# henry-yeh/DeepACO

Hardware: AMD Instinct MI355X
Metric: ant-tours/sec, TSP-500 n_ants=512 (higher is better)
Workload: dtype f32; 1 GPU; TSP-500 random-Euclidean, n_ants=512, 64 instances per GPU, AS update, heuristic 1/d sparsified k=50, sampler=auto -> scan_sparse; nodes=500, n_ants=512, instances_per_gpu=64, sampler=scan_sparse, parallelism=instance-sharded x1

## Files before the change

deepaco_amd/_lib.py:

```python
import ctypes as C
import os

import torch

_HERE = os.path.dirname(os.path.abspath(__file__))
LIB_PATH = os.environ.get("DACO_LIB_PATH") or os.path.join(_HERE, "lib", "libdeepaco_hip.so")

RACE_NOISE, RACE_PHILOX, SCAN, SCAN_WAVE = 0, 1, 2, 3
MAX_NODES = 4096

_lib = None

_vp, _i, _l, _f, _u64, _u32, _sz = (C.c_void_p, C.c_int, C.c_long, C.c_float, C.c_uint64, C.c_uint32,
                                     C.c_size_t)

SIGNATURES = {
    "daco_version": (_i, []),
    "daco_last_error": (C.c_char_p, []),
    "daco_vec_for_n": (_i, [_i]),
    "daco_ld_for_n": (_i, [_i]),
    "daco_tsp_sample_workspace_bytes": (_sz, [_i, _i, _i]),
    "daco_tsp_sample": (_i, [_vp, _i, _i, _i, _vp, _l, _vp, _l, _f, _f, _i, _i, _vp, _i, _vp, _u64, _u64, _vp,
                             _u32, _i, _vp, _vp, _vp, _vp, _vp, _l, _vp, _vp, _vp, _sz, _vp, _vp]),
    "daco_tsp_sparse_workspace_bytes": (_sz, [_i, _i, _i]),
    "daco_tsp_sparse_workspace_bytes_general": (_sz, [_i, _i, _i]),
    "daco_tsp_sparse_tours_offset": (_sz, [_i, _i, _i]),
    "daco_tsp_sparse_resident_per_cu": (_i, [_i, _i, _i]),
    "daco_tsp_sparse_split_tours": (_i, [_i]),
    "daco_tsp_sample_sparse": (_i, [_vp, _i, _i, _i, _vp, _l, _vp, _l, _f, _f, _vp, _i, _vp, _i, _u64, _u64, _vp, _u32, _i, _vp, _vp,
                                    _vp, _l, _vp, _vp, _vp, _vp, _sz, _vp, _vp]),
    "daco_tsp_sample_race_head": (_i, [_vp, _i, _i, _i, _vp, _l, _vp, _l, _f, _f, _vp, _i, _vp, _i, _u64, _u64, _vp, _u32, _i, _vp, _vp,
                                       _vp, _l, _vp, _vp, _vp, _vp, _sz, _vp, _vp]),
    "daco_tsp_sample_heads": (_i, [_vp, _i, _i, _i, _i, _i, _i, _i, _vp, _l, _vp, _l, _f, _f, _vp, _i, _vp, _i, _u64, _u64, _vp, _u32, _i, _vp, _vp,
                                   _vp, _l, _vp, _vp, _vp, _vp, _sz, _vp, _vp]),
    "daco_pheromone_update_heads": (_i, [_vp, _i, _i, _i, _vp, _vp, _vp, _f, _i, _vp, _vp, _f, _vp, _vp, _vp, _sz,
                                         _vp, _l, _f, _f, _vp, _i, _i, _i, _vp, _sz]),
    "daco_allreduce_delta_tau": (_i, [_vp, _vp, _vp, _sz]),
    "daco_tour_costs": (_i, [_vp, _i, _i, _i, _i, _vp, _l, _vp, _i, _vp]),
    "daco_pheromone_update_workspace_bytes": (_sz, [_i, _i, _i, _i]),
    "daco_pheromone_update": (_i, [_vp, _i, _i, _i, _i, _vp, _vp, _vp, _f, _i, _i, _vp, _vp, _f, _vp, _vp, _i, _vp,
                                   _sz]),
    "daco_prob_matrix": (_i, [_vp, _i, _i, _vp, _l, _vp, _l, _f, _f, _i, _vp, _sz]),
    "daco_pick_move": (_i, [_vp, _i, _i, _i, _vp, _sz, _i, _vp, _vp, _vp, _u64, _u64, _u32, _i, _vp, _vp, _vp, _vp]),
    "daco_directed_table_bytes": (_sz, [_i, _i, _i]),
    "daco_track_best": (_i, [_vp, _i, _i, _i, _vp, _vp, _vp, _vp, _vp, _vp, _f]),
    "daco_track_best_tours16": (_i, [_vp, _i, _i, _i, _i, _vp, _vp, _vp, _vp, _vp, _vp, _f]),
    "daco_cvrp_sample": (_i, [_vp, _i, _i, _i, _vp, _l, _vp, _l, _f, _f, _vp, _f, _i, _vp, _i, _u64, _u64, _vp, _u32, _i, _i,
                              _vp, _vp, _vp, _vp, _vp, _vp, _l, _vp, _vp, _vp, _sz, _vp, C.c_double, _vp, _vp]),
    "daco_sample_backward": (_i, [_vp, _i, _i, _i, _i, _vp, _l, _vp, _l, _f, _f, _vp, _vp, _vp, _vp, _vp, _f, _vp, _vp,
                                  C.c_double]),
    "daco_tsp_edge_logp": (_l, [_vp, _i, _i, _i, _i, _vp, _vp, _l, _vp, _f, _f, _vp, _vp, _vp]),
    "daco_tsp_edge_backward": (_l, [_vp, _i, _i, _i, _i, _vp, _vp, _l, _vp, _f, _f, _vp, _vp, _vp, _vp]),
    "daco_gnn_param_floats": (_sz, [_i]),
    "daco_gnn_workspace_bytes": (_sz, [_i, _i]),
    "daco_gnn_forward": (_i, [_vp, _i, _i, _i, _vp, _vp, _vp, _vp, _vp, _vp, _vp, _vp, _vp, _vp, _sz]),
    "daco_gnn_train_workspace_bytes": (_sz, [_i, _i, _i]),
    "daco_gnn_train_forward": (_i, [_vp, _i, _i, _i, _i, _vp, _vp, _vp, _vp, _vp, _vp, _vp, _vp, _vp, _vp, _vp, _sz]),
    "daco_gnn_train_backward": (_i, [_vp, _i, _i, _i, _i, _vp, _vp, _vp, _vp, _vp, _vp, _vp, _vp, _vp, _vp, _vp, _vp, _i, _vp, _sz]),
    "daco_cvrp_local_search": (_i, [_vp, _i, _i, _i, _i, _vp, _l, _vp, _f, _vp, _i, _vp, _vp]),
    "daco_hgs_table_bytes": (_sz, [_i, _i]),
    "daco_hgs_prepare": (_i, [_vp, _i, _i, _vp, _l, _i, _vp]),
    "daco_hgs_workspace_bytes": (_sz, [_i, _i, _i, _i, _i]),
    "daco_hgs_local_search": (_i, [_vp, _i, _i, _i, _i, _i, _vp, _vp, _vp, _vp, _vp, _vp, C.c_double, _i, _vp, _vp, _vp, _vp, _sz]),
    "daco_hgs_workspace_bytes_ss": (_sz, [_i, _i, _i, _i, _i]),
    "daco_hgs_local_search_ss": (_l, [_vp, _i, _i, _i, _i, _i, _vp, _vp, _vp, _vp, _vp, _vp, C.c_double, _i, _vp, _vp, _vp, _vp, _sz,
                                      _vp, _vp]),
    "daco_sibling_workspace_bytes": (_sz, [_i, _i, _i]),
    "daco_sibling_sample": (_i, [_vp, _i, _i, _i, _i, _vp, _l, _vp, _l, _f, _f, _vp, _vp, _l, _f, _vp, _i, _i, _vp, _vp,
                                 _i, _u64, _u64, _u32, _i, _vp, _vp, _vp, _vp, _vp, _vp, _sz]),
    "daco_sibling_backward": (_i, [_vp, _i, _i, _i, _i, _i, _vp, _l, _vp, _l, _f, _f, _vp, _vp, _l, _f, _vp, _i, _vp, _vp,
                                   _vp, _vp, _vp]),
    "daco_sibling_objective": (_l, [_vp, _i, _i, _i, _i, _i, _vp, _vp, _vp, _vp, _vp, _vp, _l, C.c_double, _i, _vp, _vp, _vp, _vp, _vp]),
    "daco_sibling_record": (_l, [_vp, _i, _i, _i, _i, _vp, _vp, _vp, _vp, _i, _vp, _vp, _vp, _vp, _vp, _f, _vp]),
    "daco_tsp_knn_graph": (_i, [_vp, _i, _i, _i, _vp, _f, _vp, _vp, _vp, _vp]),
    "daco_tsp_knn_graph_csr": (_i, [_vp, _i, _i, _i, _vp, _f, _vp, _vp, _vp, _vp, _vp, _vp]),
    "daco_cvrp_knn_graph": (_l, [_vp, _i, _i, _i, _vp, _i, _l, _vp, _vp, _vp, _vp, _vp, _vp]),
    "daco_heu_matrix": (_i, [_vp, _i, _i, _i, _vp, _vp, _f, _f, _vp, _vp]),
    "daco_sparsify": (_l, [_vp, _i, _i, _i, _vp, _l, _vp, _l, _vp]),
    "daco_sparse_head": (_l, [_vp, _i, _i, _i, _vp, _l, _vp]),
    "daco_head_stats": (_l, [_vp, _i, _i, _vp, _l, _i, C.c_double, C.c_double, _vp]),
    "daco_two_opt": (_i, [_vp, _i, _i, _i, _vp, _vp, _l, _vp, _l, _vp]),
    "daco_two_opt_tables_bytes": (_sz, [_i, _i]),
    "daco_two_opt_prepare": (_i, [_vp, _i, _i, _vp, _l, _vp, _sz]),
    "daco_two_opt_nbr": (_i, [_vp, _i, _i, _i, _vp, _l, _vp, _vp, _vp, _l, _vp]),
    "daco_two_opt_auto": (_i, [_vp, _i, _i, _i, _vp, _vp, _l, _vp, _vp, _vp, _l, _vp]),
    "daco_mkpv_sample": (_i, [_vp, _i, _i, _i, _i, _vp, _l, _vp, _l, _f, _f, _vp, _vp, _i, _vp, _i, _u64, _u64, _u32, _i,
                              _vp, _vp, _vp, _vp, _vp, _vp]),
    "daco_mkpv_backward": (_i, [_vp, _i, _i, _i, _i, _i, _vp, _l, _vp, _l, _f, _f, _vp, _vp, _vp, _vp, _vp, _vp]),
    "daco_mkpv_update": (_i, [_vp, _i, _i, _i, _i, _vp, _vp, _vp, _vp, _f, _i, _i, _f, _f, _vp, _vp, _vp]),
    "daco_transformer_param_floats": (_sz, [_i]),
    "daco_transformer_workspace_bytes": (_sz, [_i, _i]),
    "daco_transformer_forward": (_i, [_vp, _i, _i, _i, _vp, _vp, _sz, _vp, _vp, _sz]),
    "daco_transformer_saved_floats": (_sz, [_i, _i]),
    "daco_transformer_train_workspace_bytes": (_sz, [_i, _i]),
    "daco_transformer_forward_train": (_i, [_vp, _i, _i, _i, _vp, _vp, _sz, _vp, _vp, _sz, _vp, _sz]),
    "daco_transformer_backward": (_i, [_vp, _i, _i, _i, _vp, _vp, _sz, _vp, _sz, _vp, _vp, _vp, _sz]),
    "daco_rcpsp_schedule": (_i, [_vp, _i, _i, _i, _i, _i, _i, _vp, _vp, _vp, _vp, _vp, _vp, _vp, _vp, _vp, _vp, _vp]),
    "daco_rcpsp_workspace_bytes": (_sz, [_i, _i]),
    "daco_rcpsp_sample": (_i, [_vp, _i, _i, _i, _i, _i, _i, _vp, _vp, _vp, _vp, _vp, _vp, _vp, _vp, _vp, _vp, _l, _vp, _l, _f, _f,
                               C.c_double, C.c_double, _i, _vp, _u64, _u64, _u32, _vp, _vp, _vp, _vp, _vp, _vp, _vp, _sz]),
    "daco_rcpsp_backward": (_i, [_vp, _i, _i, _i, _vp, _vp, _vp, _l, _vp, _l, _f, _f, C.c_double, C.c_double, _vp, _vp, _vp, _vp]),
    "daco_rcpsp_track": (_i, [_vp, _i, _i, _i, _vp, _vp, _vp, C.c_double, _i, _i, _i, _f, _vp, _vp, _vp, _vp, _vp, _vp, _vp, _vp]),
    "daco_rcpsp_net_param_floats": (_sz, []),
    "daco_rcpsp_net_workspace_bytes": (_sz, [_i, _i]),
    "daco_rcpsp_net_forward": (_l, [_vp, _i, _i, _i, _vp, _vp, _vp, _f, _vp, _vp, _vp, _vp, _sz]),
    "daco_rcpsp_net_train_saved_bytes": (_sz, [_i, _i]),
    "daco_rcpsp_net_train_workspace_bytes": (_sz, [_i, _i]),
    "daco_rcpsp_net_train_forward": (_l, [_vp, _i, _i, _i, _vp, _vp, _vp, _f, _vp, _vp, _vp, _vp, _sz]),
    "daco_rcpsp_net_train_backward": (_l, [_vp, _i, _i, _i, _vp, _vp, _vp, _vp, _sz, _vp, _vp, _vp, _vp, _sz]),
    "daco_tsp_nls": (_i, [_vp, _i, _i, _i, _vp, _l, _vp, _vp, _vp, _l, _vp, _vp, _vp, _l, _i, _l, _vp, _vp, _vp]),
}


ABI_VERSION = 129


class DacoError(RuntimeError):
    pass

# ... 31 lines not shown
```

deepaco_amd/csrc/daco_colony_setup.hip:

```cpp
#include "daco_host.h"

namespace daco {

constexpr int CS_MAX_N = 1024;
constexpr int CS_HEAD_MAX_K = 127;

__device__ inline uint32_t cs_key(float v) {
  const uint32_t b = __float_as_uint(v == 0.0f ? 0.0f : v);
  return (b & 0x80000000u) ? ~b : (b | 0x80000000u);
}
__device__ inline float cs_unkey(uint32_t u) { return __uint_as_float((u & 0x80000000u) ? (u & 0x7fffffffu) : ~u); }

__device__ inline int cs_below(uint64_t mask) {
  return (int)__builtin_amdgcn_mbcnt_hi((uint32_t)(mask >> 32), __builtin_amdgcn_mbcnt_lo((uint32_t)mask, 0u));
}

template <int CPL>
__device__ inline uint32_t cs_kth_largest(const uint32_t (&key)[CPL], int k) {
  uint32_t t = 0;
  for (int bit = 31; bit >= 0; --bit) {
    const uint32_t cand = t | (1u << bit);
    int cnt = 0;
#pragma unroll
    for (int q = 0; q < CPL; ++q) cnt += __popcll(__ballot(key[q] >= cand));
// ... 17 lines not shown
  uint32_t chosen = 0;
#pragma unroll
  for (int q = 0; q < CPL; ++q) {
    const bool eq = key[q] == t;
    const uint64_t eqs = __ballot(eq);
    const bool c = key[q] > t || (eq && eq_before + cs_below(eqs) < room);
    const uint64_t cs = __ballot(c);
    pos[q] = ch_before + cs_below(cs);
    chosen |= (c ? 1u : 0u) << q;
    eq_before += __popcll(eqs);
    ch_before += __popcll(cs);
  }
  return chosen;
}

template <int CPL>
__global__ void __launch_bounds__(256)
sparsify_kernel(int B, int n, int k, const float *dist, long dist_bstride, const float *numer, long numer_bstride, float *out) {
  const int lane = threadIdx.x & 63, wave = threadIdx.x >> 6;
  const long row = (long)blockIdx.x * 4 + wave;
  if (row >= (long)B * n) return;
  const int b = (int)(row / n), i = (int)(row % n);
  const float *d = dist + (size_t)b * dist_bstride + (size_t)i * n;
  float v[CPL];
  uint32_t key[CPL];
#pragma unroll
  for (int q = 0; q < CPL; ++q) {
    const int j = lane + 64 * q;
    v[q] = j < n ? d[j] : 0.0f;
    key[q] = j < n ? ~cs_key(v[q]) : 0u;
  }
  int pos[CPL];
  const uint32_t chosen = cs_choose(key, k, cs_kth_largest(key, k), pos);
  const float *nu = numer ? numer + (size_t)b * numer_bstride : nullptr;
  float *o = out + (size_t)row * n;
#pragma unroll
  for (int q = 0; q < CPL; ++q) {
    const int j = lane + 64 * q;
    if (j < n) o[j] = (nu ? nu[j] : 1.0f) / (((chosen >> q) & 1u) ? v[q] : 1e10f);
  }
}

template <int CPL>
__global__ void __launch_bounds__(256)
sparse_head_kernel(int B, int n, int k, int slots, const float *w, long w_bstride, uint16_t *ids) {
  __shared__ uint16_t tab[4][128];
  const int lane = threadIdx.x & 63, wave = threadIdx.x >> 6;
  const long rows = (w_bstride == 0 ? 1L : (long)B) * n;
  const long row = (long)blockIdx.x * 4 + wave;
  const bool active = row < rows;
  tab[wave][lane] = 0;
  tab[wave][lane + 64] = 0;
  __syncthreads();
  if (active) {
    const float *r = w + (size_t)(row / n) * w_bstride + (size_t)(row % n) * n;
    uint32_t key[CPL];
#pragma unroll
    for (int q = 0; q < CPL; ++q) {
      const int j = lane + 64 * q;
      key[q] = j < n ? cs_key(r[j]) : 0u;
    }
    int pos[CPL];
    const uint32_t chosen = cs_choose(key, k, cs_kth_largest(key, k), pos);
#pragma unroll
    for (int q = 0; q < CPL; ++q) {
      const int j = lane + 64 * q;
      if (((chosen >> q) & 1u) && j < n && pos[q] < k) tab[wave][pos[q]] = (uint16_t)j;
    }
    if (lane == 0) tab[wave][slots - 1] = (uint16_t)k;
  }
  __syncthreads();
  const int words = slots >> 1;
  if (active && lane < words) {
    const uint32_t word = (uint32_t)tab[wave][2 * lane] | ((uint32_t)tab[wave][2 * lane + 1] << 16);
    uint32_t *out = reinterpret_cast<uint32_t *>(ids);
    if (w_bstride == 0) {
      for (int b = 0; b < B; ++b) out[((size_t)b * n + (size_t)row) * words + lane] = word;
    } else {
      out[(size_t)row * words + lane] = word;
    }
  }
}

__device__ inline double cs_wave_sum(double x) {
#pragma unroll
  for (int m = 32; m >= 1; m >>= 1) x += __shfl_xor(x, m, 64);
  return x;
}

struct HeadStatsArgs { int k[3]; double mass[3]; };

template <int CPL>
__global__ void __launch_bounds__(256)
head_stats_kernel(long rows, int n, const float *w, long w_bstride, HeadStatsArgs a, int32_t *counts) {
  __shared__ int passed[4][3];
  const int lane = threadIdx.x & 63, wave = threadIdx.x >> 6;
  int pass[3] = {0, 0, 0};
  for (long row = (long)blockIdx.x * 4 + wave; row < rows; row += (long)gridDim.x * 4) {
    const float *r = w + (size_t)(row / n) * w_bstride + (size_t)(row % n) * n;
    float v[CPL];
    uint32_t key[CPL];
    double part = 0.0;
#pragma unroll
    for (int q = 0; q < CPL; ++q) {
      const int j = lane + 64 * q;
      v[q] = j < n ? r[j] : 0.0f;
      key[q] = j < n ? cs_key(v[q]) : 0u;
      part += (double)v[q];
    }
    const double tot = cs_wave_sum(part);
#pragma unroll
    for (int c = 0; c < 3; ++c) {
      if (a.k[c] < 1) continue;
      const int K = a.k[c] < n ? a.k[c] : n;
      const uint32_t t = cs_kth_largest(key, K);
      const int above = cs_count_above(key, t);
      double s = 0.0;
#pragma unroll
      for (int q = 0; q < CPL; ++q) s += key[q] > t ? (double)v[q] : 0.0;
      s = cs_wave_sum(s) + (double)(K - above) * (double)cs_unkey(t);
      pass[c] += (s / tot >= a.mass[c]) ? 1 : 0;
    }
  }
  if (lane == 0) { passed[wave][0] = pass[0]; passed[wave][1] = pass[1]; passed[wave][2] = pass[2]; }
  __syncthreads();
  if (threadIdx.x < 3) {
    const int c = threadIdx.x, sum = passed[0][c] + passed[1][c] + passed[2][c] + passed[3][c];
    if (sum) atomicAdd(counts + c, sum);
  }
}

}

using namespace daco;

#define DACO_CS_DISPATCH(n, LAUNCH) \
  do {                              \
    const int cpl_ = ((n) + 63) / 64; \
    if (cpl_ <= 1) { LAUNCH(1); }     \
    else if (cpl_ <= 2) { LAUNCH(2); } \
    else if (cpl_ <= 4) { LAUNCH(4); } \
    else if (cpl_ <= 8) { LAUNCH(8); } \
    else { LAUNCH(16); }              \
  } while (0)

static int cs_check_size(const char *what, int B, int n) {
  if (n > CS_MAX_N) { set_error("%s: n=%d exceeds %d (one row per wavefront, in registers)", what, n, CS_MAX_N); return DACO_E_TOOLARGE; }
  if ((long)B * n > 0x7fffffffL) { set_error("%s: B * n = %ld rows do not fit 32 bits", what, (long)B * n); return DACO_E_TOOLARGE; }
  return DACO_OK;
}

extern "C" long daco_sparsify(void *stream, int B, int n, int k, const float *dist, long dist_bstride, const float *numer,
                             long numer_bstride, float *out) {
  if (B <= 0 || n < 2 || k < 1 || k > n || !dist || !out || dist_bstride < 0 || numer_bstride < 0) {
    set_error("daco_sparsify: bad argument (B=%d n=%d k=%d)", B, n, k);
    return DACO_E_BADARG;
  }
  if (const int rc = cs_check_size("daco_sparsify", B, n)) return rc;
  hipStream_t s = (hipStream_t)stream;
  const dim3 grid((unsigned)(((long)B * n + 3) / 4)), block(256);
#define DACO_CS_SPARSIFY(C) hipLaunchKernelGGL(sparsify_kernel<C>, grid, block, 0, s, B, n, k, dist, dist_bstride, numer, numer_bstride, out)
  DACO_CS_DISPATCH(n, DACO_CS_SPARSIFY);
#undef DACO_CS_SPARSIFY
  return launch_status("sparsify_kernel");
}

extern "C" long daco_sparse_head(void *stream, int B, int n, int k, const float *weights, long w_bstride, uint16_t *ids) {
  if (B <= 0 || n < 2 || k < 1 || k > n || k > CS_HEAD_MAX_K || !weights || !ids || w_bstride < 0) {
    set_error("daco_sparse_head: bad argument (B=%d n=%d k=%d, k <= %d)", B, n, k, CS_HEAD_MAX_K);
    return DACO_E_BADARG;
  }
  if (const int rc = cs_check_size("daco_sparse_head", B, n)) return rc;
  hipStream_t s = (hipStream_t)stream;
  const long rows = (w_bstride == 0 ? 1L : (long)B) * n;
  const int slots = k <= 63 ? 64 : 128;
  const dim3 grid((unsigned)((rows + 3) / 4)), block(256);
#define DACO_CS_HEAD(C) hipLaunchKernelGGL(sparse_head_kernel<C>, grid, block, 0, s, B, n, k, slots, weights, w_bstride, ids)
  DACO_CS_DISPATCH(n, DACO_CS_HEAD);
#undef DACO_CS_HEAD
  return launch_status("sparse_head_kernel");
}

extern "C" long daco_head_stats(void *stream, int B, int n, const float *weights, long w_bstride, int k_lds, double mass,
                               double mass_lds, int32_t *counts) {
  if (B <= 0 || n < 2 || !weights || !counts || w_bstride < 0) {
    set_error("daco_head_stats: bad argument (B=%d n=%d)", B, n);
    return DACO_E_BADARG;
  }
  if (const int rc = cs_check_size("daco_head_stats", B, n)) return rc;
  hipStream_t s = (hipStream_t)stream;
  if (const int rc = launch_status(zero_async(counts, 3 * sizeof(int32_t), s), "daco_head_stats (clearing the counters)")) return rc;
  const long rows = (w_bstride == 0 ? 1L : (long)B) * n;
  const HeadStatsArgs a = {{63, 127, k_lds}, {mass, mass, mass_lds}};
  const long want = (rows + 3) / 4;
  const dim3 grid((unsigned)(want < 1024 ? want : 1024)), block(256);
#define DACO_CS_STATS(C) hipLaunchKernelGGL(head_stats_kernel<C>, grid, block, 0, s, rows, n, weights, w_bstride, a, counts)
  DACO_CS_DISPATCH(n, DACO_CS_STATS);
#undef DACO_CS_STATS
  return launch_status("head_stats_kernel");
}
```

deepaco_amd/csrc/daco_costs_update.hip:

```cpp
#include "daco_host.h"
#include <cstdlib>

namespace daco {

__global__ void __launch_bounds__(256)
tour_costs_kernel(int B, int n, int len, int A, const float *dist, long dist_bs, const int64_t *paths,
                  int closed, float *costs) {
  const int idx = blockIdx.x * blockDim.x + threadIdx.x;
  if (idx >= B * A) return;
  const int b = idx / A, a = idx - b * A;
  const int64_t *p = paths + (size_t)b * len * A + a;
  const float *d = dist + b * dist_bs;
  float s = 0.0f;
  if (closed) {
    const long first = p[0];
    long prev = first;
    int k = 1;
    for (; k + 8 <= len; k += 8) {
      long u[8];
      float e[8];
#pragma unroll
      for (int j = 0; j < 8; ++j) u[j] = p[(size_t)(k + j) * A];
#pragma unroll
      for (int j = 0; j < 8; ++j) e[j] = d[u[j] * n + (j ? u[j - 1] : prev)];
// ... 57 lines not shown
    nbr[((size_t)b * n + u) * A + a] = up | (un << 16);
  }
}

__global__ void __launch_bounds__(64) argmin_cost_kernel(int A, const float *costs, int *best) {
  const int b = blockIdx.x, lane = threadIdx.x;
  float bk = __builtin_inff();
  int bi = 0x7fffffff;
  for (int a = lane; a < A; a += 64) {
    const float c = costs[(size_t)b * A + a];
    if (c < bk) { bk = c; bi = a; }
  }
  const KeyIdx r = wave_arg<false>(bk, bi);
  if (lane == 0) best[b] = r.idx == 0x7fffffff ? 0 : r.idx;
}

__global__ void __launch_bounds__(256)
track_best_kernel(int len, int A, const float *costs, const int64_t *paths, float *lowest, int64_t *shortest,
                  int32_t *best_idx, float *mmas_max, float mmas_scale, const uint16_t *tours16 = nullptr, int ld = 0) {
  __shared__ float rk[4];
  __shared__ int ri[4];
  __shared__ int take;
  const int b = blockIdx.x, tid = threadIdx.x, lane = tid & 63, wave = tid >> 6;
  float bk = __builtin_inff();
  int bi = 0x7fffffff;
  for (int a = tid; a < A; a += 256) {
    const float c = costs[(size_t)b * A + a];
    if (c < bk) { bk = c; bi = a; }
  }
  const KeyIdx r = wave_arg<false>(bk, bi);
  if (lane == 0) { rk[wave] = r.key; ri[wave] = r.idx; }
  __syncthreads();
  if (tid == 0) {
    float k = rk[0];
    int i = ri[0];
    for (int w = 1; w < 4; ++w)
      if (rk[w] < k || (rk[w] == k && ri[w] < i)) { k = rk[w]; i = ri[w]; }
    if (i == 0x7fffffff) i = 0;
    if (best_idx) best_idx[b] = i;
    float low = lowest[b];
    const bool improved = k < low;
    if (improved) { low = k; lowest[b] = k; }
    if (mmas_max) mmas_max[b] = (1.0f / low) * mmas_scale;
    take = improved ? i : -1;
  }
  __syncthreads();
  const int t = take;
  if (t >= 0 && shortest) {
    if (tours16) { for (int k = tid; k < len; k += 256) shortest[(size_t)b * len + k] = (int64_t)tours16[((size_t)b * A + t) * ld + k]; }
    else for (int k = tid; k < len; k += 256) shortest[(size_t)b * len + k] = paths[((size_t)b * len + k) * A + t];
  }
}

constexpr int DEP_CHUNK = 64;

template <bool RACE, int CH, bool VEC4>
__device__ __forceinline__ void emit_rows_of_wave(int n, int b, int i0, int Rv, const float *rows, const HeadEmit &he, uint32_t *bm,
                                                  int lane, int wave) {
  constexpr int PF = VEC4 ? 2 : 1;
  const float *eb = he.eta + (size_t)b * he.eta_bs;
  const int ch = he.ch > 0 ? he.ch : -he.ch;
  for (int r0 = wave; r0 < Rv; r0 += 4 * PF) {
    HeadEta<CH> pre[PF];
#pragma unroll
    for (int j = 0; j < PF; ++j) {
      const int rr = r0 + 4 * j;
      if (rr < Rv) {
        const size_t row = (size_t)b * n + i0 + rr;
        head_eta_fetch<CH, VEC4>(pre[j], n, ch, eb + (size_t)(i0 + rr) * n, he.hid + row * (16 * he.spl), he.spl, lane);
      }
    }
#pragma unroll
    for (int j = 0; j < PF; ++j) {
      const int rr = r0 + 4 * j;
      if (rr < Rv) {
        const size_t row = (size_t)b * n + i0 + rr;
        emit_head_row_pre<RACE, CH, VEC4>(n, ch, rows + rr * n, pre[j], bm, he.hrow + row * sp_head_row_bytes(he.spl), he.P + row * (256 * ch),
                                          he.spl, he.dead, lane);
      }
    }
  }
}

template <bool SYM, int HEADS, bool GT = false>
__global__ void __launch_bounds__(256, 4)
deposit_rows_kernel(int n, int A, int R, int hub, float *tau, const uint32_t *nbr, const float *costs, const float *weights,
                    float decay, const int *best, const float *clamp_min, const float *clamp_max, float floor_val, const HeadEmit he) {
  extern __shared__ __attribute__((aligned(16))) float rows[];
  uint32_t *stage = (uint32_t *)(rows + (((size_t)R * n + 3) & ~(size_t)3));
  float *wts = (float *)(stage + 2 * R * DEP_CHUNK);
  const int bpi = (n + R - 1) / R;
  const int b = blockIdx.x / bpi;
  const int i0 = (blockIdx.x - b * bpi) * R;
  const int Rv = min(R, n - i0);
  float *g = tau + ((size_t)b * n + i0) * n;
  const int cnt = Rv * n;
  const int hub_lo = SYM ? -1 : (hub - i0) * n, hub_hi = SYM ? -1 : hub_lo + n;
  int alo = 0, ahi = A;
  if (best) { alo = best[b]; ahi = alo + 1; }
  const uint32_t *tab = GT ? nbr + (size_t)b * ((A + 7) >> 3) * n * 8 + (size_t)i0 * 8
                           : nbr + ((size_t)b * n + i0) * A;
  const float *cs = costs + (size_t)b * A, *wt = weights ? weights + (size_t)b * A : nullptr;
  constexpr int LDU = 6;
  auto load_chunk = [&](int c0, int buf, int t0, int nt) {
    const int m = min(DEP_CHUNK, ahi - c0);
    if constexpr (GT) {
      const int per_g = Rv * 8, total = per_g * (DEP_CHUNK / 8);
      for (int ib = t0; ib < total; ib += nt * LDU) {
        uint32_t v[LDU];
        int dstx[LDU];
#pragma unroll
        for (int u = 0; u < LDU; ++u) {
          const int i = ib + u * nt, ic = i < total ? i : t0;
          const int gq = ic / per_g, rem = ic - gq * per_g;
          const int r = rem >> 3, a8 = rem & 7;
          const int ant = c0 + gq * 8 + a8;
          const int j = ant - c0;
          const int antc = j < m ? ant : c0;
          v[u] = tab[((size_t)(antc >> 3) * n + r) * 8 + (antc & 7)];
          dstx[u] = (i < total && j < DEP_CHUNK) ? ((buf * R + r) * DEP_CHUNK + j) | (j < m ? 0 : (int)0x80000000) : -1;
        }
#pragma unroll
        for (int u = 0; u < LDU; ++u)
          if (dstx[u] != -1) stage[dstx[u] & 0x7fffffff] = dstx[u] < 0 ? 0xFFFFFFFFu : v[u];
      }
    } else {
      const int total = Rv * DEP_CHUNK;
      for (int ib = t0; ib < total; ib += nt * LDU) {
        uint32_t v[LDU];
        int dstx[LDU];
#pragma unroll
        for (int u = 0; u < LDU; ++u) {
          const int i = ib + u * nt, ic = i < total ? i : t0;
          const int r = ic / DEP_CHUNK, j = ic - r * DEP_CHUNK;
          v[u] = tab[(size_t)r * A + c0 + (j < m ? j : 0)];
          dstx[u] = i < total ? ((buf * R + r) * DEP_CHUNK + j) | (j < m ? 0 : (int)0x80000000) : -1;
        }
#pragma unroll
        for (int u = 0; u < LDU; ++u)
          if (dstx[u] != -1) stage[dstx[u] & 0x7fffffff] = dstx[u] < 0 ? 0xFFFFFFFFu : v[u];
      }
    }
    if (t0 < DEP_CHUNK)
      wts[buf * DEP_CHUNK + t0] = t0 < m ? (wt ? wt[c0 + t0] : 1.0f / cs[c0 + t0]) : 0.0f;
  };
  load_chunk(alo, 0, threadIdx.x, 256);
  const bool vec_ok = SYM && (n & 3) == 0 && ((uintptr_t)g & 15) == 0;
  if (vec_ok) {
    const float4 *g4 = (const float4 *)g;
    float4 *r4 = (float4 *)rows;
    for (int i = threadIdx.x; i < cnt / 4; i += blockDim.x) {
      float4 x = g4[i];
      x.x *= decay; x.y *= decay; x.z *= decay; x.w *= decay;
      r4[i] = x;
    }
  } else {
    for (int i = threadIdx.x; i < cnt; i += blockDim.x)
      if (SYM || i < hub_lo || i >= hub_hi) rows[i] = g[i] * decay;
  }
  __syncthreads();
  const int r = SYM ? threadIdx.x >> 1 : threadIdx.x;
  const int sh = SYM ? (threadIdx.x & 1) << 4 : 16;
  const bool chain = r < Rv && (SYM || i0 + r != hub);
  float *row = rows + (chain ? r : 0) * n;
  int buf = 0;
  for (int c0 = alo; c0 < ahi; c0 += DEP_CHUNK, buf ^= 1) {
    if (c0 + DEP_CHUNK < ahi && threadIdx.x >= 64)
      load_chunk(c0 + DEP_CHUNK, buf ^ 1, threadIdx.x - 64, 192);
    if (chain) {
      const int m = min(DEP_CHUNK, ahi - c0);
      const uint32_t *st = stage + (buf * R + r) * DEP_CHUNK;
      const float *w = wts + buf * DEP_CHUNK;
      int j = 0;
      uint4 v = *(const uint4 *)st;
      float4 w4 = *(const float4 *)w;
      for (; j + 4 <= m; j += 4) {
        const int jn = j + 8 <= m ? j + 4 : j;
        const uint4 vn = *(const uint4 *)(st + jn);
        const float4 wn = *(const float4 *)(w + jn);
        const uint32_t c0_ = (v.x >> sh) & 0xFFFFu, c1_ = (v.y >> sh) & 0xFFFFu, c2_ = (v.z >> sh) & 0xFFFFu, c3_ = (v.w >> sh) & 0xFFFFu;
        if (SYM || c0_ != 0xFFFFu) row[c0_] = row[c0_] + w4.x;
        if (SYM || c1_ != 0xFFFFu) row[c1_] = row[c1_] + w4.y;
        if (SYM || c2_ != 0xFFFFu) row[c2_] = row[c2_] + w4.z;
        if (SYM || c3_ != 0xFFFFu) row[c3_] = row[c3_] + w4.w;
        v = vn;
        w4 = wn;
      }
      for (; j < m; ++j) {
        const uint32_t col = (st[j] >> sh) & 0xFFFFu;
        if (SYM || col != 0xFFFFu) row[col] = row[col] + w[j];
      }
    }
    __syncthreads();
  }
  const bool clamp = clamp_max != nullptr;
  const float cmin = clamp ? clamp_min[b] : 0.0f, cmax = clamp ? clamp_max[b] : 0.0f;
  auto finish = [&](float x) {
    if (clamp) { x = x < cmin ? cmin : x; x = x > cmax ? cmax : x; }
    if (floor_val > 0.0f) x = x < floor_val ? floor_val : x;
    return x;
  };
  if (vec_ok) {
    float4 *g4 = (float4 *)g;
    float4 *r4 = (float4 *)rows;
    for (int i = threadIdx.x; i < cnt / 4; i += blockDim.x) {
      float4 x = r4[i];
      x.x = finish(x.x); x.y = finish(x.y); x.z = finish(x.z); x.w = finish(x.w);
      g4[i] = x;
      if constexpr (HEADS != 0) r4[i] = x;
    }
  } else {
    for (int i = threadIdx.x; i < cnt; i += blockDim.x) {
      if (!SYM && i >= hub_lo && i < hub_hi) continue;
      const float x = finish(rows[i]);
      g[i] = x;
      if constexpr (HEADS != 0) rows[i] = x;
    }
  }
  if constexpr (SYM && HEADS != 0) {
    uint32_t (*head_bm)[32] = reinterpret_cast<uint32_t (*)[32]>(stage);
    __syncthreads();
    const int lane = threadIdx.x & 63, wave = threadIdx.x >> 6;
    const bool vec4 = he.ch > 0;
    const int ch = vec4 ? he.ch : -he.ch;
    if (ch <= 2) { if (vec4) emit_rows_of_wave<HEADS == 2, 2, true>(n, b, i0, Rv, rows, he, head_bm[wave], lane, wave);
                   else emit_rows_of_wave<HEADS == 2, 2, false>(n, b, i0, Rv, rows, he, head_bm[wave], lane, wave); }
    else { if (vec4) emit_rows_of_wave<HEADS == 2, 4, true>(n, b, i0, Rv, rows, he, head_bm[wave], lane, wave);
           else emit_rows_of_wave<HEADS == 2, 4, false>(n, b, i0, Rv, rows, he, head_bm[wave], lane, wave); }
  }
}

__global__ void __launch_bounds__(256)
build_next_kernel(int B, int n, int len, int A, int hub, int W, const int64_t *paths, uint32_t *nbr, uint32_t *hubmask) {
  const long total = (long)B * (len - 1) * A;
  for (long i = (long)blockIdx.x * blockDim.x + threadIdx.x; i < total; i += (long)gridDim.x * blockDim.x) {
    const int a = (int)(i % A);
    const long r = i / A;
    const int k = (int)(r % (len - 1)), b = (int)(r / (len - 1));
    const int64_t *p = paths + (size_t)b * len * A + a;
    const uint32_t u = (uint32_t)p[(size_t)k * A], v = (uint32_t)p[(size_t)(k + 1) * A];
    if ((int)u != hub) nbr[((size_t)b * n + u) * A + a] = v << 16;
    else atomicOr(hubmask + ((size_t)b * A + a) * W + (v >> 5), 1u << (v & 31));
  }
}

__device__ inline float ant_weight(const float *weights, const float *costs, size_t idx) {
  return weights ? weights[idx] : 1.0f / costs[idx];
}

constexpr int HUB_CHUNK = 256;

__global__ void __launch_bounds__(256)
deposit_hub_kernel(int n, int A, int W, int hub, float *tau, const uint32_t *hubmask, const int32_t *tab_lens,
                   const float *costs, const float *weights, float decay, const int *best, const float *clamp_min,
                   const float *clamp_max, float floor_val) {
  extern __shared__ __attribute__((aligned(16))) uint32_t hub_lds[];
  uint32_t *mw = hub_lds;
  float *wl = (float *)(hub_lds + (size_t)HUB_CHUNK * W);
  uint32_t *padl = (uint32_t *)(wl + HUB_CHUNK);
  __shared__ int longest_s;
  const int b = blockIdx.x;
  float *g = tau + ((size_t)b * n + hub) * n;
  int alo = 0, ahi = A;
  if (best) { alo = best[b]; ahi = alo + 1; }
  if (threadIdx.x == 0) longest_s = 0;
  __syncthreads();
  if (tab_lens) {
    int mx = 0;
    for (int a = threadIdx.x; a < A; a += blockDim.x) mx = max(mx, tab_lens[(size_t)b * A + a]);
    atomicMax(&longest_s, mx);
  }
  __syncthreads();
  const int longest = longest_s;
  const bool clamp = clamp_max != nullptr;
  const float cmin = clamp ? clamp_min[b] : 0.0f, cmax = clamp ? clamp_max[b] : 0.0f;
  for (int cb = 0; cb < n; cb += blockDim.x) {
    const int c = cb + threadIdx.x;
    const uint32_t *mc = mw + (c >> 5);
    const uint32_t bit = 1u << (c & 31);
    const bool is_hub = c == hub;
    float v = c < n ? g[c] * decay : 0.0f;
    for (int c0 = alo; c0 < ahi; c0 += HUB_CHUNK) {
      const int m = min(HUB_CHUNK, ahi - c0);
      __syncthreads();
      for (int i = threadIdx.x; i < m * W; i += blockDim.x) mw[i] = hubmask[((size_t)b * A + c0) * W + i];
      for (int j = threadIdx.x; j < m; j += blockDim.x) {
        wl[j] = ant_weight(weights, costs, (size_t)b * A + c0 + j);
        padl[j] = (tab_lens && tab_lens[(size_t)b * A + c0 + j] < longest) ? 1u : 0u;
      }
      __syncthreads();
      if (c < n) {
        int j = 0;
        for (; j + 8 <= m; j += 8) {
          uint32_t hit[8];
          float wv[8];
#pragma unroll
          for (int u = 0; u < 8; ++u) {
            hit[u] = (mc[(size_t)(j + u) * W] & bit) | (is_hub ? padl[j + u] : 0u);
            wv[u] = wl[j + u];
          }
#pragma unroll
          for (int u = 0; u < 8; ++u) v = hit[u] ? v + wv[u] : v;
        }
        for (; j < m; ++j)
          if ((mc[(size_t)j * W] & bit) || (is_hub && padl[j])) v = v + wl[j];
      }
    }
// ... 50 lines not shown
extern "C" size_t daco_directed_table_bytes(int B, int n, int A) {
  if (B <= 0 || n <= 0 || A <= 0) return 0;
  return DirectedTable::bytes(B, n, A);
}

extern "C" size_t daco_pheromone_update_workspace_bytes(int B, int n, int len, int A) {
  if (B <= 0 || n <= 0 || A <= 0 || len <= 0) return 0;
  return align256(DirectedTable::next_bytes(B, n, A)) + align256((size_t)B * sizeof(int)) + align256(DirectedTable::hubmask_bytes(B, n, A));
}

static int rows_per_block(int n, bool symmetric, int B = 1 << 20) {
  const int budget_kb = symmetric ? 40 : 24;
  int R = (budget_kb * 1024 - 2 * DEP_CHUNK * 4 - 16) / (4 * n + 2 * DEP_CHUNK * 4);
  const int cap = symmetric ? 32 : 64;
  if (R > cap) R = cap;
  if (R < 1) R = 1;
  while (R > 1 && (long)B * ((n + R - 1) / R) < 512) R = (R + 1) / 2;
  return R;
}
static size_t deposit_lds_bytes(int R, int n) {
  return (((size_t)R * n + 3) & ~(size_t)3) * sizeof(float) + (size_t)2 * R * DEP_CHUNK * sizeof(uint32_t) + 2 * DEP_CHUNK * sizeof(float);
}

static int pheromone_update_impl(void *stream, int B, int n, int len, int A, float *tau,
                                 const int64_t *paths, const float *costs, float decay, int elitist,
                                 int symmetric, const float *clamp_min, const float *clamp_max,
                                 float floor_val, const uint32_t *nbr_in, const float *weights, int hub,
                                 void *workspace, size_t workspace_bytes, const HeadEmit &he) {
  if (B <= 0 || n < 3 || A <= 0 || !tau || (!paths && !nbr_in) || !costs || !workspace) {
    set_error("daco_pheromone_update: bad argument (B=%d n=%d A=%d)", B, n, A);
    return DACO_E_BADARG;
  }
  if ((clamp_min == nullptr) != (clamp_max == nullptr)) { set_error("daco_pheromone_update: clamp_min/clamp_max must both be given"); return DACO_E_BADARG; }
  if (n > DACO_MAX_NODES) { set_error("daco_pheromone_update: n=%d exceeds DACO_MAX_NODES", n); return DACO_E_TOOLARGE; }
  if (symmetric && len != n) { set_error("daco_pheromone_update: symmetric deposit needs len == n"); return DACO_E_BADARG; }
  if (hub >= n) { set_error("daco_pheromone_update: hub %d >= n %d", hub, n); return DACO_E_BADARG; }
  if (!symmetric && len < 2) { set_error("daco_pheromone_update: directed deposit needs len >= 2"); return DACO_E_BADARG; }
  if (!symmetric && nbr_in && hub != 0) { set_error("daco_pheromone_update: a directed next_table implies hub = 0"); return DACO_E_BADARG; }
  const size_t need = daco_pheromone_update_workspace_bytes(B, n, len, A);
  if (workspace_bytes < need) { set_error("daco_pheromone_update: workspace %zu < %zu", workspace_bytes, need); return DACO_E_WORKSPACE; }
  hipStream_t s = (hipStream_t)stream;
  const uint32_t *nbr = nbr_in ? nbr_in : (const uint32_t *)workspace;
  int *best = (int *)((char *)workspace + align256(DirectedTable::next_bytes(B, n, A)));
  if (!symmetric) {
    const int W = (n + 31) / 32;
    const uint32_t *hubmask = (const uint32_t *)((char *)best + align256((size_t)B * sizeof(int)));
    const int32_t *tab_lens = nullptr;
    if (nbr_in) {
      const DirectedTable tab = DirectedTable::carve(nbr_in, B, n, A);
      hubmask = tab.hubmask;
      tab_lens = tab.lens;
    } else {
      if (hipMemsetAsync((void *)hubmask, 0, DirectedTable::hubmask_bytes(B, n, A), s) != hipSuccess) { set_error("hipMemsetAsync failed"); return DACO_E_HIP; }
      if (hipMemsetAsync(workspace, 0xFF, DirectedTable::next_bytes(B, n, A), s) != hipSuccess) { set_error("hipMemsetAsync failed"); return DACO_E_HIP; }
      const long total = (long)B * (len - 1) * A;
      int blocks = (int)((total + 255) / 256);
      if (blocks > 16384) blocks = 16384;
      hipLaunchKernelGGL(build_next_kernel, dim3(blocks), dim3(256), 0, s, B, n, len, A, hub, W, paths, (uint32_t *)workspace, (uint32_t *)hubmask);
    }
    if (elitist) hipLaunchKernelGGL(argmin_cost_kernel, dim3(B), dim3(64), 0, s, A, costs, best);
    const int R = rows_per_block(n, false, B);
    const int bpi = (n + R - 1) / R;
    if (hub >= 0)
      hipLaunchKernelGGL(deposit_hub_kernel, dim3(B), dim3(256), (size_t)HUB_CHUNK * (W + 2) * sizeof(uint32_t), s, n, A, W, hub, tau, hubmask, tab_lens,
                         costs, weights, decay, elitist ? best : nullptr, clamp_min, clamp_max, floor_val);
    hipLaunchKernelGGL((deposit_rows_kernel<false, 0>), dim3(B * bpi), dim3(256), deposit_lds_bytes(R, n), s, n, A, R, hub, tau,
                       nbr, costs, weights, decay, elitist ? best : nullptr, clamp_min, clamp_max,
                       floor_val, he);
    return launch_status("directed pheromone update");
  }
  if (!nbr_in) {
    const long total = (long)B * n * A;
    int blocks = (int)((total + 255) / 256);
    if (blocks > 16384) blocks = 16384;
    hipLaunchKernelGGL(build_nbr_kernel, dim3(blocks), dim3(256), 0, s, B, n, A, paths, (uint32_t *)workspace);
  }
  if (elitist) hipLaunchKernelGGL(argmin_cost_kernel, dim3(B), dim3(64), 0, s, A, costs, best);
  const int R = rows_per_block(n, true, B);
  const int bpi = (n + R - 1) / R;
#define DACO_DEPOSIT_SYM_G(H, G) hipLaunchKernelGGL((deposit_rows_kernel<true, H, G>), dim3(B * bpi), dim3(256), deposit_lds_bytes(R, n), s, n, A, R, 0, tau, \
                                                    nbr, costs, weights, decay, elitist ? best : nullptr, clamp_min, clamp_max, floor_val, he)
#define DACO_DEPOSIT_SYM(H) do { if (grouped) DACO_DEPOSIT_SYM_G(H, true); else DACO_DEPOSIT_SYM_G(H, false); } while (0)
  const bool grouped = nbr_in != nullptr && he.nbr_grouped != 0;
  if (!he.eta) DACO_DEPOSIT_SYM(0);
  else if (!he.race) DACO_DEPOSIT_SYM(1);
  else DACO_DEPOSIT_SYM(2);
#undef DACO_DEPOSIT_SYM
#undef DACO_DEPOSIT_SYM_G
  return launch_status("pheromone update");
}

extern "C" int daco_pheromone_update(void *stream, int B, int n, int len, int A, float *tau,
                                     const int64_t *paths, const float *costs, float decay, int elitist,
                                     int symmetric, const float *clamp_min, const float *clamp_max,
                                     float floor_val, const uint32_t *nbr_in, const float *weights, int hub,
                                     void *workspace, size_t workspace_bytes) {
  return pheromone_update_impl(stream, B, n, len, A, tau, paths, costs, decay, elitist, symmetric, clamp_min, clamp_max, floor_val, nbr_in,
                               weights, hub, workspace, workspace_bytes, HeadEmit{});
}

extern "C" int daco_pheromone_update_heads(void *stream, int B, int n, int A, float *tau, const int64_t *paths, const float *costs,
                                           float decay, int elitist, const float *clamp_min, const float *clamp_max, float floor_val,
                                           const uint32_t *nbr_in, const float *weights, void *workspace, size_t workspace_bytes,
                                           const float *eta, long eta_bstride, float alpha, float beta, const uint16_t *head_id,
                                           int head_slots, int race, int nbr_grouped, void *sparse_workspace, size_t sparse_workspace_bytes) {
  if (!eta || !head_id || !sparse_workspace) { set_error("daco_pheromone_update_heads: bad argument"); return DACO_E_BADARG; }
  if (head_slots != 64 && head_slots != 128) { set_error("daco_pheromone_update_heads: head_slots = %d (64 or 128)", head_slots); return DACO_E_BADARG; }
  if (n <= 128 || n > 1024) { set_error("daco_pheromone_update_heads: n=%d outside 129..1024 (the sizes daco_tsp_sample_heads serves)", n); return DACO_E_TOOLARGE; }
  if (alpha != 1.0f || beta != 1.0f) { set_error("daco_pheromone_update_heads: alpha = beta = 1 only (the rows of tau are formed here; other exponents take the sampler's own pass)"); return DACO_E_BADARG; }
  const size_t need = daco_tsp_sparse_workspace_bytes(B, n, A);
  if (sparse_workspace_bytes < need) { set_error("daco_pheromone_update_heads: sparse workspace %zu < %zu bytes", sparse_workspace_bytes, need); return DACO_E_WORKSPACE; }
  const HeadWs ws = HeadWs::carve(sparse_workspace, B, n, A);
  HeadEmit he;
  he.eta = eta; he.eta_bs = eta_bstride; he.hid = head_id;
  he.P = ws.P; he.hrow = ws.hrow;
  he.spl = head_slots / 16; he.race = race ? 1 : 0; he.nbr_grouped = nbr_grouped ? 1 : 0;
  he.dead = ws.ld;
  const bool vec4 = rows_vec4(n, tau, (long)n * n, eta, eta_bstride);
  he.ch = vec4 ? ws.ld / 256 : -(ws.ld / 256);
  return pheromone_update_impl(stream, B, n, n, A, tau, paths, costs, decay, elitist, 1, clamp_min, clamp_max, floor_val, nbr_in, weights, 0,
                               workspace, workspace_bytes, he);
}
```

deepaco_amd/csrc/daco_head_rows.h:

```cpp
#pragma once
#include "daco_device.h"

namespace daco {

constexpr int SP_KH_MAX = 128;
__host__ __device__ constexpr int sp_lane_bytes(int spl) { return spl * 6; }
__host__ __device__ constexpr size_t sp_head_row_bytes(int spl) { return (size_t)16 * sp_lane_bytes(spl); }

template <bool VEC4>
__device__ __forceinline__ void sp_load4(const float *row, int n, int k0, float4 &out) {
  if constexpr (VEC4) {
    out = *reinterpret_cast<const float4 *>(row + (k0 < n ? k0 : 0));
  } else {
    out.x = row[k0 + 0 < n ? k0 + 0 : 0]; out.y = row[k0 + 1 < n ? k0 + 1 : 0];
    out.z = row[k0 + 2 < n ? k0 + 2 : 0]; out.w = row[k0 + 3 < n ? k0 + 3 : 0];
  }
}
__device__ __forceinline__ float4 sp_mul4_masked(const float4 &t, const float4 &e, int n, int k0) {
  float4 v;
  v.x = k0 + 0 < n ? t.x * e.x : 0.0f; v.y = k0 + 1 < n ? t.y * e.y : 0.0f;
  v.z = k0 + 2 < n ? t.z * e.z : 0.0f; v.w = k0 + 3 < n ? t.w * e.w : 0.0f;
  return v;
}
template <bool VEC4>
// ... 11 lines not shown
  int id[2];
  int cnt;
};
template <int CH, bool VEC4>
__device__ __forceinline__ void head_eta_fetch(HeadEta<CH> &h, int n, int ch, const float *er, const uint16_t *ids, int spl, int lane) {
  const int kh = 16 * spl;
  h.cnt = ids[kh - 1] < kh - 1 ? ids[kh - 1] : kh - 1;
#pragma unroll
  for (int c = 0; c < CH; ++c) sp_load4<VEC4>(er, n, c < ch ? (c * 64 + lane) * 4 : 0, h.e[c]);
#pragma unroll
  for (int j = 0; j < 2; ++j) {
    const int m = lane + 64 * j;
    h.id[j] = m < kh ? (int)ids[m] : n;
    h.eh[j] = er[h.id[j] < n ? h.id[j] : 0];
  }
}

template <bool RACE, int CH, bool VEC4>
__device__ __forceinline__ void emit_head_row_pre(int n, int ch, const float *tr, const HeadEta<CH> &h, uint32_t *bm, char *hl,
                                                  float *pr, int spl, int dead, int lane) {
  const int kh = 16 * spl, ls = sp_lane_bytes(spl);
  const int cnt = h.cnt;
  if (lane < 32) bm[lane] = 0u;
  __builtin_amdgcn_wave_barrier();
#pragma unroll
  for (int j = 0; j < 2; ++j) { const int m = lane + 64 * j, id = h.id[j]; if (m < cnt && id < n) atomicOr(&bm[id >> 5], 1u << (id & 31)); }
  __builtin_amdgcn_wave_barrier();
  float part = RACE ? __builtin_inff() : 0.0f;
#pragma unroll
  for (int c = 0; c < CH; ++c) {
    if (c < ch) {
      const int k0 = (c * 64 + lane) * 4;
      float4 t;
      sp_load4<VEC4>(tr, n, k0, t);
      const float4 v = sp_mul4_masked(t, h.e[c], n, k0);
      *reinterpret_cast<float4 *>(pr + k0) = v;
      const uint32_t w = bm[(k0 >> 5) & 31] >> (k0 & 31);
      if constexpr (RACE) {
        part = fminf(part, (w & 1u) ? __builtin_inff() : 1.0f / v.x);
        part = fminf(part, (w & 2u) ? __builtin_inff() : 1.0f / v.y);
        part = fminf(part, (w & 4u) ? __builtin_inff() : 1.0f / v.z);
        part = fminf(part, (w & 8u) ? __builtin_inff() : 1.0f / v.w);
      } else {
        part = part + ((w & 1u) ? 0.0f : v.x);
        part = part + ((w & 2u) ? 0.0f : v.y);
        part = part + ((w & 4u) ? 0.0f : v.z);
        part = part + ((w & 8u) ? 0.0f : v.w);
      }
    }
  }
  float T;
  if constexpr (RACE) {
    for (int o = 32; o >= 1; o >>= 1) part = fminf(part, __shfl_xor(part, o));
    T = part;
  } else {
    T = readlane_f(wave_scan_add(part), 63);
  }
#pragma unroll
  for (int j = 0; j < 2; ++j) {
    const int m = lane + 64 * j;
    if (m < kh) {
      const int id = h.id[j];
      const bool live = m < cnt && id < n;
      const float pid = live ? tr[id] * h.eh[j] : 0.0f;
      float val;
      if constexpr (RACE) val = m == kh - 1 ? T : (live ? 1.0f / pid : __builtin_inff());
      else val = m == kh - 1 ? T : (live ? pid : 0.0f);
      char *hs = hl + (m / spl) * ls;
      *reinterpret_cast<float *>(hs + (m % spl) * 4) = val;
      *reinterpret_cast<uint16_t *>(hs + spl * 4 + (m % spl) * 2) = (uint16_t)(live && m != kh - 1 ? id : dead);
    }
  }
  __builtin_amdgcn_wave_barrier();
}

template <bool RACE, int CH, bool VEC4>
__device__ __forceinline__ void emit_head_row(int n, int ch, const float *tr, const float *er,
                                              const uint16_t *ids, uint32_t *bm, char *hl, float *pr, int spl, int dead, int lane) {
  HeadEta<CH> h;
  head_eta_fetch<CH, VEC4>(h, n, ch, er, ids, spl, lane);
  emit_head_row_pre<RACE, CH, VEC4>(n, ch, tr, h, bm, hl, pr, spl, dead, lane);
}

struct HeadEmit {
  const float *eta = nullptr;
  long eta_bs = 0;
  const uint16_t *hid = nullptr;
  char *hrow = nullptr;
  float *P = nullptr;
  int spl = 4, ch = 2, dead = 512, race = 0;
  int nbr_grouped = 0;
};

}
```

deepaco_amd/csrc/daco_sample_kernel.h:

```cpp
#pragma once
#include <cstdlib>
#include <type_traits>
#include <utility>

#include "daco_host.h"
#include "daco_rcpsp.h"

namespace daco {

struct SampleParams {
  int B, n, A, ld, CH;
  const float *P;
  const float *R;
  int norm_passes;
  const int64_t *start;
  int fixed_start;
  const float *noise;
  uint64_t seed, iter;
  int gid_bstride;
  const uint64_t *iter_dev;
  uint32_t ant_gid0;
  int64_t *paths;
  float *logp;
  float *rowsum;
  int32_t *flags;
  const float *dist;
  long dist_bs;
  float *costs;
  uint32_t *nbr;
  uint32_t *hubmask;
  int32_t *tab_lens;
  const float *aux_vec;
  const float *aux_mat;
  float scalar0;
  const float *wts;
  int m;
  const float *mask;
  int step;
  const float *demand;
  float capacity;
  const double *demand64;
  double capacity64;
  int Lmax;
  int noise_steps;
  int32_t *lens;
  const float *hval = nullptr;
  const uint16_t *hid = nullptr;
  unsigned long long *stats = nullptr;
  uint16_t *tours16 = nullptr;
  const float *tau = nullptr, *eta = nullptr;
  long tau_bs = 0, eta_bs = 0;
  float alpha = 1.0f, beta = 1.0f;
  int row_vec = 0;
  int nbr_grouped = 0;
  int lh_kl = 0, lh_kmax = 0;
  RcpspDev rc;
};

inline SampleParams sample_params(int B, int n, int A, int ld, int CH, const float *P, const float *R, const float *noise, uint64_t seed,
                                  uint64_t iter, uint32_t ant_gid0, int64_t *paths, float *logp, float *rowsum, int32_t *flags) {
  SampleParams sp{};
  sp.B = B; sp.n = n; sp.A = A; sp.ld = ld; sp.CH = CH;
  sp.P = P; sp.R = R; sp.noise = noise; sp.seed = seed; sp.iter = iter; sp.ant_gid0 = ant_gid0;
  sp.paths = paths; sp.logp = logp; sp.rowsum = rowsum; sp.flags = flags;
  return sp;
}

template <class F, int... I>
__device__ inline void static_for_impl(F &&f, std::integer_sequence<int, I...>) {
  (f(std::integral_constant<int, I>{}), ...);
}
template <int N, class F>
__device__ inline void static_for(F &&f) { static_for_impl(f, std::make_integer_sequence<int, N>{}); }

template <int VEC>
__device__ inline void load_vec(const float *p, float (&out)[VEC]) {
  if constexpr (VEC == 4) {
    const float4 t = *reinterpret_cast<const float4 *>(p);
    out[0] = t.x; out[1] = t.y; out[2] = t.z; out[3] = t.w;
  } else if constexpr (VEC == 2) {
    const float2 t = *reinterpret_cast<const float2 *>(p);
    out[0] = t.x; out[1] = t.y;
  } else {
    out[0] = *p;
  }
}

void launch_prob_matrix(int B, int n, int ld, const float *tau, long tau_bs, const float *eta, long eta_bs, float alpha,
                        float beta, float *P, float *R, hipStream_t s);
void launch_pad_matrix(int B, int n, int ld, const float *src, long src_bs, float *dst, float fill, hipStream_t s);

struct Visited {
  uint32_t lo = 0, hi = 0;
  template <int BIT> __device__ inline bool test() const {
    if constexpr (BIT < 32) return (lo >> BIT) & 1u; else return (hi >> (BIT - 32)) & 1u;
  }
  __device__ inline void set(int bit) {
    if (bit < 32) lo |= 1u << bit; else hi |= 1u << (bit - 32);
  }
  template <int BIT> __device__ inline float open_only(float x) const {
    int m;
    float r;
    asm("v_bfe_i32 %0, %1, %2, 1" : "=v"(m) : "v"(BIT < 32 ? lo : hi), "n"(BIT & 31));
    asm("v_bfi_b32 %0, %1, 0, %2" : "=v"(r) : "v"(m), "v"(x));
    return r;
  }
  template <int BIT> __device__ inline void set_if(bool c) {
    if constexpr (BIT < 32) lo |= (c ? 1u : 0u) << BIT; else hi |= (c ? 1u : 0u) << (BIT - 32);
  }
};

enum { PROB_TSP = 0, PROB_CVRP = 1, PROB_STEP = 2, PROB_SOP = 3, PROB_PCTSP = 4, PROB_OP = 5, PROB_MKP = 6, PROB_CVRP64 = 7, PROB_RCPSP = 8 };

template <int VEC, int CH, int MODE, bool LOGP, int PROB>
__global__ void __launch_bounds__(256)
tsp_sample_kernel(const SampleParams p) {
  constexpr bool CVRP = PROB == PROB_CVRP || PROB == PROB_CVRP64, DEM64 = PROB == PROB_CVRP64, STEP = PROB == PROB_STEP, RCPSP = PROB == PROB_RCPSP, SOP = PROB == PROB_SOP || RCPSP,
                 PCTSP = PROB == PROB_PCTSP, OP = PROB == PROB_OP, MKP = PROB == PROB_MKP;
  constexpr bool VARLEN = CVRP || PCTSP || OP || MKP;
  constexpr bool DUMMY = OP || MKP;
  constexpr int NJ = CH * VEC;
  const int lane = threadIdx.x & 63;
  const int wave = threadIdx.x >> 6;
  const int w = xcd_remap(blockIdx.x, gridDim.x);
  const int bpi = (p.A + 3) >> 2;
  const int b = w / bpi;
  const int a_raw = (w - b * bpi) * 4 + wave;
  constexpr bool EPI = PROB == PROB_TSP;
  const bool dup = EPI && a_raw >= p.A;
  if (a_raw >= p.A && !dup) return;
  const int a = dup ? p.A - 1 : a_raw;
  extern __shared__ __attribute__((aligned(16))) uint16_t epi_lds[];
  const int TL = (p.n + 7) & ~7;
  uint16_t *tour = epi_lds + (size_t)wave * TL;
  const int n = p.n, A = p.A, ld = p.ld;
  const uint64_t iter_now = p.iter + (p.iter_dev ? *p.iter_dev : 0ull);
// ... 561 lines not shown
```

deepaco_amd/csrc/daco_scan_sparse.hip:

```cpp
#include "daco_sample_kernel.h"
#include "daco_head_rows.h"

namespace daco {

constexpr int SP_FCMP_OGT = 2, SP_FCMP_OGE = 3, SP_FCMP_OLT = 4;

enum : uint32_t { STREAM_SPARSE = 4, STREAM_SPARSE_RETRY = 5 };

template <int N> __device__ inline float sp_row_bcast(float x) { return dpp_f<0x150 + N, 0xF, false>(x, x); }
template <int N> __device__ inline int sp_row_ror(int x) { return dpp_i<0x120 + N, 0xF, false>(x, x); }
__device__ inline float sp_row_scan(float x) {
  x = x + dpp_f<DPP_ROW_SHR(1), 0xF, true>(0.0f, x);
  x = x + dpp_f<DPP_ROW_SHR(2), 0xF, true>(0.0f, x);
  x = x + dpp_f<DPP_ROW_SHR(4), 0xF, true>(0.0f, x);
  x = x + dpp_f<DPP_ROW_SHR(8), 0xF, true>(0.0f, x);
  return x;
}
__device__ inline uint64_t sp_row_first(uint64_t m) { return m & ~((m | 0x8000800080008000ull) - 0x0001000100010001ull); }

template <bool RACE, bool VEC4, int CH>
__global__ void __launch_bounds__(256)
sparse_prepass_kernel(int B, int n, int ch, const float *tau, long tau_bs, const float *eta, long eta_bs,
                      const uint16_t *hid, float *P, char *hrow, int spl, int dead) {
  __shared__ uint32_t bm[4][32];
  const int lane = threadIdx.x & 63, wave = threadIdx.x >> 6;
  const long row = (long)blockIdx.x * 4 + wave;
  if (row >= (long)B * n) return;
  const int b = (int)(row / n), r = (int)(row - (long)b * n);
  const float *tr = tau + b * tau_bs + (long)r * n, *er = eta + b * eta_bs + (long)r * n;
  emit_head_row<RACE, CH, VEC4>(n, ch, tr, er, hid + row * (16 * spl), bm[wave], hrow + row * sp_head_row_bytes(spl), P + row * (256 * ch), spl, dead, lane);
}

struct SpRowSrc { const float *p; };
__device__ __forceinline__ float4 sp_row4(const SpRowSrc &r, int k0) { return *reinterpret_cast<const float4 *>(r.p + k0); }

template <int CHD, bool TAIL>
__device__ __forceinline__ int sparse_row_walk(const SpRowSrc &rowp, const uint8_t *flg, const uint32_t *bm, int lane, float ur) {
  constexpr int NJ = CHD * 4;
  float run[16];
  float acc = 0.0f;
  uint32_t pos = 0;
#pragma unroll
  for (int c = 0; c < CHD; ++c) {
    const int k0 = (c * 64 + lane) * 4;
    const float4 rv = sp_row4(rowp, k0);
    float f[4];
    if constexpr (TAIL) {
      const uint32_t w = bm[(k0 >> 5) & 31] >> (k0 & 31);
      f[0] = (w & 1u) ? 0.0f : 1.0f; f[1] = (w & 2u) ? 0.0f : 1.0f; f[2] = (w & 4u) ? 0.0f : 1.0f; f[3] = (w & 8u) ? 0.0f : 1.0f;
    } else {
      const uint32_t ff = *reinterpret_cast<const uint32_t *>(flg + k0);
      f[0] = (float)(ff & 0xFFu); f[1] = (float)((ff >> 8) & 0xFFu); f[2] = (float)((ff >> 16) & 0xFFu); f[3] = (float)(ff >> 24);
    }
    acc = __builtin_fmaf(rv.x, f[0], acc); run[4 * c + 0] = acc;
    acc = __builtin_fmaf(rv.y, f[1], acc); run[4 * c + 1] = acc;
    acc = __builtin_fmaf(rv.z, f[2], acc); run[4 * c + 2] = acc;
    acc = __builtin_fmaf(rv.w, f[3], acc); run[4 * c + 3] = acc;
    pos |= (rv.x * f[0] > 0.0f ? 1u : 0u) << (4 * c) | (rv.y * f[1] > 0.0f ? 2u : 0u) << (4 * c) |
           (rv.z * f[2] > 0.0f ? 4u : 0u) << (4 * c) | (rv.w * f[3] > 0.0f ? 8u : 0u) << (4 * c);
  }
#pragma unroll
  for (int j = NJ; j < 16; ++j) run[j] = __builtin_inff();
  const float part = acc;
  const float incl = wave_scan_add(part);
  float r = ur;
  if constexpr (!TAIL) {
    const float S = readlane_f(incl, 63);
    if (!(S > 0.0f)) return -1;
    r = ur * S;
    r = r > 0.0f ? r : 1.401298464e-45f;
  }
  uint64_t m = __ballot(incl >= r && part > 0.0f);
  int L;
  if (m == 0) {
    if constexpr (!TAIL) return -1;
    m = __ballot(part > 0.0f);
    if (m == 0) return -1;
    L = 63 - __builtin_clzll(m);
  } else {
    L = __builtin_ctzll(m);
  }
  const float excl = L ? readlane_f(incl, L - 1) : 0.0f;
  const float thr = fmaxf(r - excl, 1.401298464e-45f);
  const int cnt = count_below<NJ>(run, thr);
  int jsel = readlane_i(cnt, L);
  if (jsel >= NJ) {
    const uint32_t pl = (uint32_t)readlane_i((int)pos, L);
    jsel = pl ? 31 - __builtin_clz(pl) : 0;
  }
  return ((jsel >> 2) * 64 + L) * 4 + (jsel & 3);
}

typedef uint32_t sp_u32x4 __attribute__((ext_vector_type(4)));
typedef uint32_t sp_u32x2 __attribute__((ext_vector_type(2)));
__device__ inline float sp_at_least_denorm(float x) {
  float y;
  asm("v_max_f32 %0, 1, %1" : "=v"(y) : "v"(x));
  return y;
}

constexpr int SP_W = 352;
constexpr int SP_EW = 160;
constexpr int SP_ST_DEAD = 16 * (512 + 16) + 4 * 128 + 256;
constexpr int SP_ST_LDS = SP_ST_DEAD + 16 * SP_W * 2;
static_assert(SP_ST_LDS <= 160 * 1024 / 8 && SP_ST_DEAD % 16 == 0, "ST: eight workgroups per CU");
static_assert(SP_ST_DEAD >= 16 * SP_EW * 2 + 4 * 512 * 2, "ST: early parts and the inverse table of four ants inside the dead bytes");

static_assert(std::is_trivially_copyable<SampleParams>::value, "SampleParams is read back from the kernel-argument segment as plain bytes");
template <int CHD, bool RACE, int SPL, bool LH = false, bool ST = false>
__global__ void __launch_bounds__(256, LH ? 1 : (ST ? 8 : (CHD == 2 ? (RACE ? 4 : 6) : 5)))
scan_sparse_kernel(const SampleParams p) {
  static_assert(!LH || (CHD == 2 && !RACE && SPL == 4), "the LDS-heads variant: n <= 512, scan draw, 64-slot heads");
  static_assert(!ST || (CHD == 2 && !RACE && SPL == 4 && !LH), "the split-tour variant: n <= 512, scan draw, 64-slot heads, not LH");
  constexpr int APW = 4, APB = LH ? 4 : 16;
  constexpr int LS = sp_lane_bytes(SPL);
  constexpr int LAST = SPL - 1;
  constexpr int FL = CHD * 256;
  constexpr int FLP = FL + 16;
  constexpr int FLT = FL + 2;
  constexpr uint32_t ROWB = 16u * LS;
  constexpr bool TG = CHD == 4;
  extern __shared__ __attribute__((aligned(16))) unsigned char sparse_dyn[];
  uint8_t *flag_mem = sparse_dyn;
  uint16_t *tour_mem = reinterpret_cast<uint16_t *>(sparse_dyn + (ST ? SP_ST_DEAD : APB * FLP));
  __shared__ uint32_t bm_static[TG || ST ? 1 : (LH ? 1 : 4)][32];
  uint32_t (*bm_s)[32] = TG ? reinterpret_cast<uint32_t (*)[32]>(sparse_dyn + APB * FLP + APB * 32)
                            : ST ? reinterpret_cast<uint32_t (*)[32]>(sparse_dyn + APB * FLP) : bm_static;
  unsigned char *lh_tab = sparse_dyn + APB * FLP + APB * FLT * 2;
  static_assert(!LH || ((APB * FLP + APB * FLT * 2) % 16 == 0), "LH: table aligned");
  const int lane = threadIdx.x & 63, wave = __builtin_amdgcn_readfirstlane(threadIdx.x >> 6);
  const int q = lane >> 4, s = lane & 15;
  const int w = xcd_remap(blockIdx.x, gridDim.x);
  const int bpi = (p.A + APB - 1) / APB;
  const int b = w / bpi;
  const int abase = (w - b * bpi) * APB;
  const int a0 = abase + wave * APW;
  const int n = p.n, A = p.A;
  const uint64_t iter_now = p.iter + (p.iter_dev ? *p.iter_dev : 0ull);
  const bool active = a0 < A && (!LH || wave == 0);
  const int a = a0 + q < A ? a0 + q : A - 1;
  const uint32_t gid = p.ant_gid0 + (uint32_t)(b * (p.gid_bstride ? p.gid_bstride : A) + a);
  const float *Pb = p.P + (size_t)b * n * p.ld;
  const char *hrb = (const char *)p.hval + (size_t)b * n * ROWB;
  const __amdgpu_buffer_rsrc_t hres = __builtin_amdgcn_make_buffer_rsrc((void *)hrb, 0, (int)((uint32_t)n * ROWB), 0x00020000);
#define SP_ROW_OF(pv) SpRowSrc{Pb + (size_t)(pv) * p.ld}
  uint32_t sls = (uint32_t)s * LS;
  asm volatile("" : "+v"(sls));
  uint8_t *fl = flag_mem + (wave * APW + q) * FLP;
  uint16_t *tour = tour_mem + (wave * APW + q) * (TG ? 16 : ST ? SP_W : FLT);
  uint16_t *t16b = TG || ST ? p.tours16 + ((size_t)b * A + abase) * FL : nullptr;
  const int TE = ST ? (n > SP_W ? (n - SP_W + 15) & ~15 : 0) : 0;
  const uint32_t t16o = (uint32_t)((wave * APW + q) * FL + s);
#define SP_T(t) (TG ? ((t) & 15) : (t))
  bool infeasible = false;
  unsigned long long n_dense = 0, n_tail = 0, n_rej = 0;
  uint32_t lh_rb = 0, lh_rbsel = 0, lh_loff = 0, lh_toff = 0;
  if constexpr (LH) {
    const int kl = p.lh_kl, kmax = p.lh_kmax;
    lh_rb = (uint32_t)kl * LS;
    lh_toff = (uint32_t)(kmax / SPL) * LS + (uint32_t)(kmax % SPL) * 4u;
    lh_rbsel = s < kl ? lh_rb : 0u;
    lh_loff = s < kl ? (uint32_t)s * LS : (uint32_t)n * lh_rb;
    const char *src = hrb;
    const int l16 = threadIdx.x & 15;
    if (l16 < kl)
      for (int row0 = threadIdx.x >> 4; row0 < n; row0 += 16 * 8) {
        uint2 x[8][3];
#pragma unroll
        for (int u = 0; u < 8; ++u) {
          const int row = row0 + 16 * u;
          const uint2 *g = reinterpret_cast<const uint2 *>(src + (size_t)(row < n ? row : row0) * ROWB + l16 * LS);
          x[u][0] = g[0]; x[u][1] = g[1]; x[u][2] = g[2];
        }
#pragma unroll
        for (int u = 0; u < 8; ++u) {
          const int row = row0 + 16 * u;
          if (row < n) {
            uint2 *d = reinterpret_cast<uint2 *>(lh_tab + (uint32_t)row * lh_rb + l16 * LS);
            d[0] = x[u][0]; d[1] = x[u][1]; d[2] = x[u][2];
          }
        }
      }
    if (threadIdx.x < 4) reinterpret_cast<float *>(lh_tab + (uint32_t)n * lh_rb)[threadIdx.x] = 0.0f;
    if (threadIdx.x >= 4 && threadIdx.x < 6) reinterpret_cast<uint32_t *>(lh_tab + (uint32_t)n * lh_rb)[threadIdx.x] = (uint32_t)p.ld * 0x00010001u;
    __syncthreads();
    bool too_many = false;
    for (int row = threadIdx.x; row < n; row += 256) {
      const char *gr = src + (size_t)row * ROWB;
      const uint16_t idk = *reinterpret_cast<const uint16_t *>(gr + (kmax / SPL) * LS + SPL * 4 + (kmax % SPL) * 2);
      too_many |= idk != (uint16_t)p.ld;
      *reinterpret_cast<float *>(lh_tab + (uint32_t)row * lh_rb + lh_toff) = *reinterpret_cast<const float *>(gr + 15 * LS + LAST * 4);
    }
    if (too_many && p.flags) atomicOr(p.flags + b, 4);
    __syncthreads();
  }

  if (active) {
    {
      const uint4 ones = make_uint4(0x01010101u, 0x01010101u, 0x01010101u, 0x01010101u);
#pragma unroll
      for (int g = 0; g < FL / 256; ++g) *(uint4 *)(fl + g * 256 + s * 16) = ones;
      fl[FL + s] = 0;
    }
    int prev;
    if (p.start) prev = (int)p.start[(size_t)b * A + a];
    else if (p.fixed_start >= 0) prev = p.fixed_start;
    else {
      const u32x4 r = rng_block(p.seed, iter_now, STREAM_START, gid, 0);
      prev = (int)__umulhi(r.x, (uint32_t)n);
    }
    __builtin_amdgcn_wave_barrier();
    if (s == 0) { fl[prev] = 0; tour[0] = (uint16_t)prev; }
    asm volatile("" ::: "memory");
    __builtin_amdgcn_wave_barrier();
    u32x4 ublk = {0, 0, 0, 0};
    float ucur = 0.0f;
    for (int t0 = 0; t0 < n; t0 += 16) {
      int t = t0;
      if constexpr (ST) {
        if (t0 == TE && t0 != 0) {
          int lf = lane;
          asm volatile("" : "+v"(lf) :: "memory");
          const int qf = lf >> 4;
          const uint4 *src = reinterpret_cast<const uint4 *>(tour);
          uint4 *dst = reinterpret_cast<uint4 *>(t16b + (size_t)(wave * APW + qf) * FL);
          for (int j = lf & 15; j < (TE >> 3); j += 16) {
            const uint4 v = src[j];
            if (a0 + qf < A) dst[j] = v;
          }
          asm volatile("" ::: "memory");
          tour -= TE;
        }
      }
      if constexpr (!RACE) {
        if ((t0 & 63) == 0) ublk = rng_block(p.seed, iter_now, STREAM_SPARSE, gid, (uint32_t)(((t0 >> 6) << 4) + (15 - s)));
        ucur = u01(comp(ublk, (t0 >> 4) & 3));
        if (t0 == 0) ucur = __int_as_float(sp_row_ror<1>(__float_as_int(ucur)));
      }
      if (t0 == 0) t = 1;
      const int te = t0 + 16 < n ? t0 + 16 : n;
#ifndef DACO_SPARSE_UNROLL
#define DACO_SPARSE_UNROLL 1
#endif
#pragma unroll DACO_SPARSE_UNROLL
      for (; t < te; ++t) {
        const uint32_t off = LH ? __umul24((uint32_t)prev, lh_rbsel) + lh_loff : __umul24((uint32_t)prev, ROWB) + sls;
        float h[SPL];
        uint32_t w0, w1, w2 = 0, w3 = 0;
        if constexpr (LH) {
          const uint2 ra = *reinterpret_cast<const uint2 *>(lh_tab + off), rb_ = *reinterpret_cast<const uint2 *>(lh_tab + off + 8),
                      rc = *reinterpret_cast<const uint2 *>(lh_tab + off + 16);
          const float tv = *reinterpret_cast<const float *>(lh_tab + __umul24((uint32_t)prev, lh_rb) + lh_toff);
          h[0] = __uint_as_float(ra.x); h[1] = __uint_as_float(ra.y); h[2] = __uint_as_float(rb_.x);
          h[3] = s == 15 ? tv : __uint_as_float(rb_.y);
          w0 = rc.x; w1 = rc.y;
        } else if constexpr (SPL == 4) {
          const sp_u32x4 hvr = __builtin_amdgcn_raw_buffer_load_b128(hres, off, 0, 0);
          const sp_u32x2 hi2 = __builtin_amdgcn_raw_buffer_load_b64(hres, off + 16u, 0, 0);
          h[0] = __uint_as_float(hvr.x); h[1] = __uint_as_float(hvr.y); h[2] = __uint_as_float(hvr.z); h[3] = __uint_as_float(hvr.w);
          w0 = hi2.x; w1 = hi2.y;
        } else {
          const sp_u32x4 hva = __builtin_amdgcn_raw_buffer_load_b128(hres, off, 0, 0);
          const sp_u32x4 hvb = __builtin_amdgcn_raw_buffer_load_b128(hres, off + 16u, 0, 0);
          const sp_u32x4 hi4 = __builtin_amdgcn_raw_buffer_load_b128(hres, off + 32u, 0, 0);
          h[0] = __uint_as_float(hva.x); h[1] = __uint_as_float(hva.y); h[2] = __uint_as_float(hva.z); h[3] = __uint_as_float(hva.w);
          h[4] = __uint_as_float(hvb.x); h[5] = __uint_as_float(hvb.y); h[6] = __uint_as_float(hvb.z); h[7] = __uint_as_float(hvb.w);
          w0 = hi4.x; w1 = hi4.y; w2 = hi4.z; w3 = hi4.w;
        }
        if constexpr (SPL == 8) asm volatile("" : "+v"(w0), "+v"(w1), "+v"(w2), "+v"(w3));
#define SP_IDW(j) ((j) == 0 ? w0 : (j) == 1 ? w1 : (j) == 2 ? w2 : w3)
#define SP_ID(v) (((v) & 1) ? (int)(SP_IDW((v) >> 1) >> 16) : (int)(SP_IDW((v) >> 1) & 0xFFFFu))
        if constexpr (RACE) {
          const float rtail = sp_row_bcast<15>(h[LAST]);
          float bk = __builtin_inff();
          int bi = 0x7fffffff;
#pragma unroll
          for (int v = 0; v < SPL; ++v) {
            const int k = SP_ID(v);
            const u32x4 r4 = rng_block(p.seed, iter_now, STREAM_RACE, gid, ((uint32_t)t << 12) | (uint32_t)(k >> 2));
            const float Lk = neg_log2_1m(u01(comp(r4, k & 3)));
            const float key = fl[k] != 0 ? Lk * h[v] : __builtin_inff();
            if (prefer<false>(key, k, bk, bi)) { bk = key; bi = k; }
          }
          arg_step<false, DPP_ROW_SHR(1), 0xF>(bk, bi);
          arg_step<false, DPP_ROW_SHR(2), 0xF>(bk, bi);
          arg_step<false, DPP_ROW_SHR(4), 0xF>(bk, bi);
          arg_step<false, DPP_ROW_SHR(8), 0xF>(bk, bi);
          const float best = sp_row_bcast<15>(bk);
          int choice = __float_as_int(sp_row_bcast<15>(__int_as_float(bi)));
          const float lmin = neg_log2_1m(0x1p-24f);
          uint64_t rare = __ballot(!(best < 0.5f * lmin * rtail)) & 0x0001000100010001ull;
          while (rare) {
            const int gl = __builtin_ctzll(rare);
            rare &= rare - 1;
            const int g = gl >> 4;
            const int pv = readlane_i(prev, gl);
            const uint32_t gidg = (uint32_t)readlane_i((int)gid, gl);
            const uint8_t *flg = flag_mem + (wave * APW + g) * FLP;
            const SpRowSrc rowp = SP_ROW_OF(pv);
            n_dense += a0 + g < A ? 1ull : 0ull;
            float dk = __builtin_inff();
            int di = 0x7fffffff;
#pragma unroll
            for (int c = 0; c < CHD; ++c) {
              const int k0 = (c * 64 + lane) * 4;
              const float4 pvv = sp_row4(rowp, k0);
              const uint32_t ff = *reinterpret_cast<const uint32_t *>(flg + k0);
              const u32x4 r4 = rng_block(p.seed, iter_now, STREAM_RACE, gidg, ((uint32_t)t << 12) | (uint32_t)(c * 64 + lane));
              const float pp[4] = {pvv.x, pvv.y, pvv.z, pvv.w};
#pragma unroll
              for (int v = 0; v < 4; ++v) {
                const float Lk = neg_log2_1m(u01(comp(r4, v)));
                const float key = ((ff >> (8 * v)) & 0xFFu) ? Lk * (1.0f / pp[v]) : __builtin_inff();
                if (key < dk) { dk = key; di = k0 + v; }
              }
            }
            const KeyIdx rr = wave_arg<false>(dk, di);
            int cg = rr.idx;
            if (!(rr.key < __builtin_inff())) { infeasible = true; cg = 0; }
            choice = q == g ? cg : choice;
          }
          if (s == 0) { fl[choice] = 0; tour[SP_T(t)] = (uint16_t)choice; }
          asm volatile("" ::: "memory");
          __builtin_amdgcn_wave_barrier();
          prev = choice;
        } else {
          float f[SPL], run[SPL];
#pragma unroll
          for (int v = 0; v < SPL; ++v) f[v] = (float)fl[SP_ID(v)];
          run[0] = __builtin_fmaf(h[0], f[0], 0.0f);
#pragma unroll
          for (int v = 1; v < SPL; ++v) run[v] = __builtin_fmaf(h[v], f[v], run[v - 1]);
          const float incl = sp_row_scan(run[LAST]);
          const float excl = dpp_f<DPP_ROW_SHR(1), 0xF, true>(0.0f, incl);
          const float r = sp_row_bcast<15>(sp_at_least_denorm(ucur * (incl + h[LAST])));
          ucur = __int_as_float(sp_row_ror<1>(__float_as_int(ucur)));

#define SP_LAST_POSITIVE(out)                                                                                     \
          do {                                                                                                    \
            int lp_ = 0;                                                                                          \
            _Pragma("unroll") for (int v = 1; v < SPL; ++v) lp_ = h[v] * f[v] > 0.0f ? v : lp_;                   \
            const uint64_t lo_ = ((uint64_t)w1 << 32) | w0, hi_ = ((uint64_t)w3 << 32) | w2;                      \
            out = (int)(((lp_ >= 4 ? hi_ : lo_) >> (16 * (lp_ & 3))) & 0xFFFFu);                                  \
          } while (0)
#define SP_HEAD_DECIDE(rr, first_out, sel_out)                                                                    \
          do {                                                                                                    \
            const float rr_ = (rr);                                                                               \
            const uint64_t m_ = __builtin_amdgcn_fcmpf(incl, rr_, SP_FCMP_OGE) & __builtin_amdgcn_fcmpf(run[LAST], 0.0f, SP_FCMP_OGT); \
            first_out = sp_row_first(m_);                                                                         \
            const float thr_ = sp_at_least_denorm(rr_ - excl);                                                    \
            bool below_[SPL];                                                                                     \
            _Pragma("unroll") for (int v = 0; v < SPL - 1; ++v) below_[v] = run[v] < thr_;                        \
            uint32_t pair_;                                                                                       \
            if constexpr (SPL == 4) pair_ = below_[1] ? w1 : w0;                                                  \
            else pair_ = below_[3] ? (below_[5] ? w3 : w2) : (below_[1] ? w1 : w0);                               \
            bool odd_ = below_[0];                                                                                \
            _Pragma("unroll") for (int v = 1; v < SPL - 1; ++v) odd_ = odd_ != below_[v];                         \
            sel_out = odd_ ? (int)(pair_ >> 16) : (int)(pair_ & 0xFFFFu);                                         \
            const uint64_t bad_ = first_out & __builtin_amdgcn_fcmpf(run[LAST], thr_, SP_FCMP_OLT);               \
            if (__builtin_expect(bad_ != 0, 0)) {                                                                 \
              int lastp_;                                                                                         \
              SP_LAST_POSITIVE(lastp_);                                                                           \
              sel_out = run[LAST] < thr_ ? lastp_ : sel_out;                                                      \
            }                                                                                                     \
          } while (0)
          int sel;
          uint64_t first;
          SP_HEAD_DECIDE(r, first, sel);


          if (__builtin_expect(__builtin_popcountll(first) != APW, 0)) {
            uint64_t any = first | (first >> 8);
            any |= any >> 4; any |= any >> 2; any |= any >> 1;
            uint64_t rare = ~any & 0x0001000100010001ull;
            while (rare) {
              const int gl = __builtin_ctzll(rare);
              rare &= rare - 1;
              const int g = gl >> 4;
              const int pv = readlane_i(prev, gl);
              const float Hg = readlane_f(incl, gl + 15);
              const float ug = readlane_f(ucur, gl), rg = readlane_f(r, gl);
              const uint32_t gidg = (uint32_t)readlane_i((int)gid, gl);
              const uint8_t *flg = flag_mem + (wave * APW + g) * FLP;
              const SpRowSrc rowp = SP_ROW_OF(pv);
              int choice_g = -1;
              const unsigned long long real = a0 + g < A ? 1ull : 0ull;
              if (!(Hg > 0.0f)) {
                n_dense += real;
                choice_g = sparse_row_walk<CHD, false>(rowp, flg, nullptr, lane, ug);
              } else {
                n_tail += real;
                if (lane < 32) bm_s[wave][lane] = 0u;
                asm volatile("" ::: "memory");
                __builtin_amdgcn_wave_barrier();
                if (q == g) {
#pragma unroll
                  for (int v = 0; v < SPL; ++v) {
                    const int idl = SP_ID(v);
                    if (idl < n) atomicOr(&bm_s[wave][idl >> 5], 1u << (idl & 31));
                  }
                }
                asm volatile("" ::: "memory");
                __builtin_amdgcn_wave_barrier();
                float rp = rg - Hg;
                rp = rp > 0.0f ? rp : 1.401298464e-45f;
                const int j = sparse_row_walk<CHD, true>(rowp, flg, bm_s[wave], lane, rp);
                if (j < 0) {
                  const bool live_lane = q == g && run[LAST] > 0.0f;
                  const uint64_t ml = __ballot(live_lane);
                  if (ml != 0) {
                    const int Ll = 63 - __builtin_clzll(ml);
                    int lastp;
                    SP_LAST_POSITIVE(lastp);
                    choice_g = readlane_i(lastp, Ll);
                  }
                } else if (flg[j] != 0) {
                  choice_g = j;
                } else {
                  n_rej += real;
                  n_dense += real;
                  const u32x4 rb = rng_block(p.seed, iter_now, STREAM_SPARSE_RETRY, gidg, (uint32_t)t << 8);
                  choice_g = sparse_row_walk<CHD, false>(rowp, flg, nullptr, lane, u01(rb.x));
                }
              }
              if (choice_g < 0) { infeasible = true; choice_g = 0; }
              if (lane == gl) { fl[choice_g] = 0; tour[SP_T(t)] = (uint16_t)choice_g; }
            }
          }
          const bool winner = __builtin_amdgcn_inverse_ballot_w64(first);
          if (winner) { fl[sel] = 0; tour[SP_T(t)] = (uint16_t)sel; }
          asm volatile("" ::: "memory");
          prev = tour[SP_T(t)];
          asm volatile("" ::: "memory");
        }
      }
      if constexpr (TG) {
        asm volatile("" ::: "memory");
        const uint16_t wv = tour[s];
        if (a0 + q < A) t16b[t16o + (uint32_t)t0] = wv;
        asm volatile("" ::: "memory");
      }
    }
  }
#undef SP_T
#undef SP_ROW_OF
#undef SP_HEAD_DECIDE
#undef SP_LAST_POSITIVE
#undef SP_ID
#undef SP_IDW
  typedef const __attribute__((address_space(4))) SampleParams *sp_args_t;
  sp_args_t pe = (sp_args_t)__builtin_amdgcn_kernarg_segment_ptr();
  if constexpr (ST) asm volatile("" : "+s"(pe));
#define SP_E(x) (ST ? pe->x : p.x)
  if (infeasible && SP_E(flags) && lane == 0) atomicOr(SP_E(flags) + b, 1);
  if (SP_E(stats) && lane == 0 && (n_dense | n_tail | n_rej)) {
    atomicAdd(SP_E(stats) + 0, n_dense); atomicAdd(SP_E(stats) + 1, n_tail); atomicAdd(SP_E(stats) + 2, n_rej);
  }

  const int nant = A - abase < APB ? A - abase : APB;
  if constexpr (!TG) {
    uint16_t (*tour_s)[FLT] = reinterpret_cast<uint16_t (*)[FLT]>(tour_mem);
    __syncthreads();
    uint16_t (*early_s)[SP_EW] = reinterpret_cast<uint16_t (*)[SP_EW]>(sparse_dyn);
    uint16_t (*late_s)[SP_W] = reinterpret_cast<uint16_t (*)[SP_W]>(tour_mem);
#define SP_TOUR(k, t) (ST ? ((t) < TE ? early_s[k][t] : late_s[k][(t) - TE]) : tour_s[k][t])
    if constexpr (ST) {
      if (TE > 0) {
        const int V = TE >> 3;
        for (int e = threadIdx.x; e < APB * V; e += 256) {
          const int k = e / V, j = e - k * V;
          reinterpret_cast<uint4 *>(early_s[k])[j] = reinterpret_cast<const uint4 *>(t16b + (size_t)(k < nant ? k : nant - 1) * FL)[j];
        }
        __syncthreads();
      }
    }
    const int k16 = threadIdx.x & (APB - 1);
    constexpr int TSTEP = 256 / APB;
    if (SP_E(paths) && k16 < nant) {
      int64_t *pb = SP_E(paths) + (size_t)b * n * A + abase;
      for (int t = threadIdx.x / APB; t < n; t += TSTEP) pb[(size_t)t * A + k16] = (int64_t)SP_TOUR(k16, t);
    }
    if constexpr (ST) {
      if (!SP_E(paths) && SP_E(tours16)) {
        uint32_t *tb = reinterpret_cast<uint32_t *>(SP_E(tours16) + ((size_t)b * A + abase) * FL + TE);
        const int wl = (TE + SP_W < FL ? SP_W : FL - TE) / 2;
        for (int e = threadIdx.x; e < nant * (SP_W / 2); e += 256) {
          const int k = e / (SP_W / 2), j = e - k * (SP_W / 2);
          if (j < wl) tb[(size_t)k * (FL / 2) + j] = reinterpret_cast<const uint32_t *>(late_s[k])[j];
        }
      }
    } else if (!SP_E(paths) && SP_E(tours16)) {
      uint32_t *tb = reinterpret_cast<uint32_t *>(SP_E(tours16) + ((size_t)b * A + abase) * FL);
      for (int e = threadIdx.x; e < nant * (FL / 2); e += 256) {
        const int k = e / (FL / 2), j = e - k * (FL / 2);
        tb[(size_t)k * (FL / 2) + j] = reinterpret_cast<const uint32_t *>(tour_s[k])[j];
      }
    }
    if (SP_E(costs)) {
      __syncthreads();
      const float *dist_b = SP_E(dist) + (size_t)b * SP_E(dist_bs);
      constexpr int DSW = ST ? 32 : 64;
      float (*dstage)[APW][DSW] = reinterpret_cast<float (*)[APW][DSW]>(LH ? lh_tab : ST ? sparse_dyn + APB * SP_EW * 2 : flag_mem);
      if (active) {
        float cost = 0.0f;
        const float *mine_d = dstage[wave][q];
        for (int base = 1; base < n; base += DSW) {
          const int t = base + (lane & (DSW - 1));
#pragma unroll
          for (int r4 = 0; r4 < APW; r4 += 64 / DSW) {
            const int kr = wave * APW + r4 + lane / DSW;
            dstage[wave][r4 + lane / DSW][lane & (DSW - 1)] = t < n ? dist_b[(uint32_t)SP_TOUR(kr, t) * (uint32_t)n + SP_TOUR(kr, t - 1)] : 0.0f;
          }
          __builtin_amdgcn_wave_barrier();
          if (s == 0) {
#pragma unroll
            for (int v4 = 0; v4 < DSW / 4; ++v4) {
              const float4 v = *(const float4 *)(mine_d + 4 * v4);
              cost = cost + v.x; cost = cost + v.y; cost = cost + v.z; cost = cost + v.w;
            }
          }
          __builtin_amdgcn_wave_barrier();
        }
        if (s == 0 && a0 + q < A) {
          const int km = wave * APW + q;
          cost = cost + dist_b[(uint32_t)SP_TOUR(km, 0) * (uint32_t)n + SP_TOUR(km, n - 1)];
          SP_E(costs)[(size_t)b * A + a0 + q] = cost;
        }
      }
    }
    if (SP_E(nbr)) {
      constexpr int NI = ST ? 4 : 8;
      uint16_t (*inv)[FL] = reinterpret_cast<uint16_t (*)[FL]>(LH ? lh_tab + 4096 : ST ? sparse_dyn + APB * SP_EW * 2 : flag_mem);
      static_assert(LH || ST || APB * FLP >= 8 * FL * (int)sizeof(uint16_t), "inverse table of eight ants inside the flag array");
// ... 44 lines not shown
      if (p.costs) {
        const float *dist_b = p.dist + (size_t)b * p.dist_bs;
        float (*dstage)[2][64] = reinterpret_cast<float (*)[2][64]>(&inv[0][0]);
        const int hh = lane >> 5;
        const int mine = wave * 2 + hh;
        float cost = 0.0f;
        for (int base = 1; base < n; base += 64) {
          const int t = base + lane;
#pragma unroll
          for (int r2 = 0; r2 < 2; ++r2) {
            const uint16_t *tr = tl[wave * 2 + r2];
            dstage[wave][r2][lane] = t < n && wave * 2 + r2 < nh ? dist_b[(uint32_t)tr[t] * (uint32_t)n + tr[t - 1]] : 0.0f;
          }
          __builtin_amdgcn_wave_barrier();
          if ((lane & 31) == 0) {
            const float *md = dstage[wave][hh];
#pragma unroll
            for (int v4 = 0; v4 < 16; ++v4) {
              const float4 v = *(const float4 *)(md + 4 * v4);
              cost = cost + v.x; cost = cost + v.y; cost = cost + v.z; cost = cost + v.w;
            }
          }
          __builtin_amdgcn_wave_barrier();
        }
        if ((lane & 31) == 0 && mine < nh) {
          const uint16_t *tm = tl[mine];
          cost = cost + dist_b[(uint32_t)tm[0] * (uint32_t)n + tm[n - 1]];
          p.costs[(size_t)b * A + abase + half * 8 + mine] = cost;
        }
      }
      if (p.nbr) {
        __syncthreads();
        for (int e = threadIdx.x; e < 8 * FL / 8; e += 256) ((uint4 *)&inv[0][0])[e] = make_uint4(0, 0, 0, 0);
        __syncthreads();
        const uint16_t *tk = tl[k8 < nh ? k8 : 0];
        if (k8 < nh)
          for (int t = threadIdx.x >> 3; t < n; t += 32) inv[k8][tk[t]] = (uint16_t)t;
        __syncthreads();
        const int a8 = abase + half * 8;
        uint32_t *nb = p.nbr_grouped ? p.nbr + (((size_t)b * ((A + 7) >> 3) + (a8 >> 3)) * n) * 8 + (a8 & 7) : p.nbr + (size_t)b * n * A + a8;
        const size_t nstride = p.nbr_grouped ? 8 : (size_t)A;
        if (k8 < nh)
          for (int node = threadIdx.x >> 3; node < n; node += 32) {
            const int t = inv[k8][node];
            const uint32_t pv = tk[t == 0 ? n - 1 : t - 1], nx = tk[t == n - 1 ? 0 : t + 1];
            nb[(size_t)node * nstride + k8] = pv | (nx << 16);
          }
      }
    }
  }
}

}

using namespace daco;

__global__ void __launch_bounds__(256)
pow_pair_kernel(long count_t, const float *tau, float alpha, float *tau_out, long count_e, const float *eta, float beta, float *eta_out) {
  const long i = (long)blockIdx.x * 256 + threadIdx.x;
  if (i < count_t) tau_out[i] = pw(tau[i], alpha);
  if (i < count_e) eta_out[i] = pw(eta[i], beta);
}

static bool sparse_sizes_ok(int B, int n, int A) { return B > 0 && A > 0 && n > 128 && n <= 1024; }
extern "C" size_t daco_tsp_sparse_tours_offset(int B, int n, int A) { return sparse_sizes_ok(B, n, A) ? HeadWs::tours_offset(B, n) : 0; }
extern "C" size_t daco_tsp_sparse_workspace_bytes(int B, int n, int A) { return sparse_sizes_ok(B, n, A) ? HeadWs::bytes(B, n, A) : 0; }
extern "C" size_t daco_tsp_sparse_workspace_bytes_general(int B, int n, int A) { return sparse_sizes_ok(B, n, A) ? HeadWs::bytes_general(B, n, A) : 0; }

constexpr int SP_WHOLE_TOUR_PER_CU = 6, SP_SPLIT_TOUR_PER_CU = 8;
static int sparse_split_mode = -1;
extern "C" int daco_tsp_sparse_split_tours(int mode) {
  const int old = sparse_split_mode;
  if (mode >= -1 && mode <= 1) sparse_split_mode = mode;
  return old;
}
static bool sparse_many_workgroups(long workgroups) {
  if (sparse_split_mode >= 0) return sparse_split_mode == 1;
  int dev = 0, cus = 0;
  if (hipGetDevice(&dev) != hipSuccess || hipDeviceGetAttribute(&cus, hipDeviceAttributeMultiprocessorCount, dev) != hipSuccess) { (void)hipGetLastError(); return true; }
  return workgroups > (long)SP_WHOLE_TOUR_PER_CU * cus && workgroups <= (long)SP_SPLIT_TOUR_PER_CU * cus;
}

struct SparseVariant { const void *fn; size_t lds; };
static SparseVariant sparse_variant(int ld, bool race, int spl, bool many) {
#define DACO_SPARSE_LDS(C) ((C) == 2 ? 16 * ((C) * 256 + 16) + 16 * ((C) * 256 + 2) * 2 : 2 * 8 * (C) * 256 * 2)
#define DACO_SPARSE_V(C, R, S) SparseVariant{reinterpret_cast<const void *>(&scan_sparse_kernel<C, R, S>), (size_t)DACO_SPARSE_LDS(C)}
  if (ld <= 512 && !race && spl == 4 && many) return SparseVariant{reinterpret_cast<const void *>(&scan_sparse_kernel<2, false, 4, false, true>), (size_t)SP_ST_LDS};
  if (ld <= 512) return race ? (spl == 4 ? DACO_SPARSE_V(2, true, 4) : DACO_SPARSE_V(2, true, 8)) : (spl == 4 ? DACO_SPARSE_V(2, false, 4) : DACO_SPARSE_V(2, false, 8));
  return race ? (spl == 4 ? DACO_SPARSE_V(4, true, 4) : DACO_SPARSE_V(4, true, 8)) : (spl == 4 ? DACO_SPARSE_V(4, false, 4) : DACO_SPARSE_V(4, false, 8));
#undef DACO_SPARSE_V
#undef DACO_SPARSE_LDS
}

extern "C" int daco_tsp_sparse_resident_per_cu(int n, int head_slots, int race) {
  if (n <= 128 || n > 1024 || (head_slots != 64 && head_slots != 128)) return 0;
  const SparseVariant v = sparse_variant(HeadWs::ld_for(n), race != 0, head_slots / 16, true);
  int nb = 0;
  if (hipOccupancyMaxActiveBlocksPerMultiprocessor(&nb, v.fn, 256, v.lds) != hipSuccess) { (void)hipGetLastError(); return 0; }
  return nb;
}

static int sample_sparse_impl(bool race, bool heads_ready, int head_live_max, int nbr_grouped, const char *what, void *stream, int B, int n, int A, const float *tau, long tau_bstride, const float *eta,
                                      long eta_bstride, float alpha, float beta, const uint16_t *head_id, int head_slots, const int64_t *start,
                                      int fixed_start, uint64_t seed, uint64_t iter, const uint64_t *iter_offset,
                                      uint32_t ant_gid0, int ant_gid_bstride, int64_t *paths, int32_t *flags, const float *dist,
                                      long dist_bstride, float *costs, uint32_t *nbr, unsigned long long *stats, void *workspace,
                                      size_t workspace_bytes, void *ev_begin, void *ev_end) {
  if (B <= 0 || A <= 0 || !tau || !eta || !head_id || !workspace || (!paths && !nbr)) {
    set_error("%s: bad argument (B=%d n=%d A=%d)", what, B, n, A);
    return DACO_E_BADARG;
  }
  if (head_slots != 64 && head_slots != 128) { set_error("%s: head_slots = %d (64 or 128)", what, head_slots); return DACO_E_BADARG; }
  if (n <= 128 || n > 1024) { set_error("%s: n=%d outside 129..1024 (the dense samplers serve the other sizes)", what, n); return DACO_E_TOOLARGE; }
  if ((size_t)n * A * 8 >= ((size_t)1 << 32)) { set_error("%s: n * A too large for 32-bit offsets", what); return DACO_E_TOOLARGE; }
  if (fixed_start >= n) { set_error("%s: fixed_start %d >= n %d", what, fixed_start, n); return DACO_E_BADARG; }
  if (costs && !dist) { set_error("%s: fused costs need the distance matrix", what); return DACO_E_BADARG; }
  const size_t need = daco_tsp_sparse_workspace_bytes(B, n, A);
  if (workspace_bytes < need) { set_error("%s: workspace %zu < %zu bytes", what, workspace_bytes, need); return DACO_E_WORKSPACE; }
  hipStream_t s = (hipStream_t)stream;
  const HeadWs ws = HeadWs::carve(workspace, B, n, A);
  const int ld = ws.ld;
  const int spl = head_slots / 16;
  if (alpha != 1.0f || beta != 1.0f) {
    const size_t need_g = daco_tsp_sparse_workspace_bytes_general(B, n, A);
    if (workspace_bytes < need_g) {
      set_error("%s: alpha = %g, beta = %g need daco_tsp_sparse_workspace_bytes_general() = %zu bytes of workspace (got %zu)", what, alpha, beta, need_g, workspace_bytes);
      return DACO_E_WORKSPACE;
    }
    if (heads_ready) { set_error("%s: heads_ready needs alpha = beta = 1 (daco_pheromone_update_heads forms the rows of tau itself)", what); return DACO_E_BADARG; }
    if ((tau_bstride != 0 && tau_bstride != (long)n * n) || (eta_bstride != 0 && eta_bstride != (long)n * n)) {
      set_error("%s: exponents other than 1 need dense matrices (stride n * n between instances, or 0 for a shared one)", what);
      return DACO_E_BADARG;
    }
    const long ct = (tau_bstride ? (long)B : 1L) * n * n, ce = (eta_bstride ? (long)B : 1L) * n * n;
    const long cm = ct > ce ? ct : ce;
    hipLaunchKernelGGL(pow_pair_kernel, dim3((unsigned)((cm + 255) / 256)), dim3(256), 0, s, ct, tau, alpha, ws.tau_pow, ce, eta, beta, ws.eta_pow);
    tau = ws.tau_pow; eta = ws.eta_pow;
    alpha = beta = 1.0f;
  }
  const bool vec4 = rows_vec4(n, tau, tau_bstride, eta, eta_bstride);
  if (!heads_ready) {
    const dim3 pg((unsigned)(((long)B * n + 3) / 4));
#define DACO_PREPASS_C(R, V, C) hipLaunchKernelGGL((sparse_prepass_kernel<R, V, C>), pg, dim3(256), 0, s, B, n, ld / 256, tau, tau_bstride, eta, eta_bstride, \
                                                   head_id, ws.P, ws.hrow, spl, ld)
#define DACO_PREPASS(R, V) do { if (ld <= 512) DACO_PREPASS_C(R, V, 2); else DACO_PREPASS_C(R, V, 4); } while (0)
    if (race) { if (vec4) DACO_PREPASS(true, true); else DACO_PREPASS(true, false); }
    else { if (vec4) DACO_PREPASS(false, true); else DACO_PREPASS(false, false); }
#undef DACO_PREPASS
#undef DACO_PREPASS_C
  }
  if (const int rc = launch_status("sparse_prepass_kernel")) return rc;
  SampleParams sp = sample_params(B, n, A, ld, ld / 256, ws.P, nullptr, nullptr, seed, iter, ant_gid0, paths, nullptr, nullptr, flags);
  sp.start = start; sp.fixed_start = fixed_start;
  sp.tau = tau; sp.tau_bs = tau_bstride; sp.eta = eta; sp.eta_bs = eta_bstride; sp.alpha = alpha; sp.beta = beta; sp.row_vec = vec4 ? 1 : 0;
  sp.iter_dev = iter_offset; sp.gid_bstride = ant_gid_bstride;
  sp.dist = dist; sp.dist_bs = dist_bstride; sp.costs = costs; sp.nbr = nbr; sp.nbr_grouped = nbr_grouped ? 1 : 0;
  sp.hval = (const float *)ws.hrow; sp.hid = head_id; sp.stats = stats; sp.tours16 = ws.tours16;
  if (const int rc = record_event(ev_begin, s, "ev_begin")) return rc;
  bool lh = false;
  size_t lh_lds = 0;
  if (!race && spl == 4 && ld == 512 && head_live_max > 0 && head_live_max <= 62 && (long)B * ((A + 3) / 4) <= 256) {
    const int kl = (head_live_max + 1 + 3) / 4;
    const size_t table = (size_t)n * kl * sp_lane_bytes(4) + 32;
    lh_lds = (size_t)4 * (512 + 16) + (size_t)4 * (512 + 2) * 2 + (table > 12288 + 1024 ? table : 12288 + 1024);
    lh = lh_lds + 128 <= 160 * 1024;
    sp.lh_kl = kl; sp.lh_kmax = head_live_max;
  }
  const int bpi = lh ? (A + 3) / 4 : (A + 15) / 16;
  const dim3 grid((unsigned)(B * bpi));
  if (lh) {
    if (hipFuncSetAttribute(reinterpret_cast<const void *>(&scan_sparse_kernel<2, false, 4, true>), hipFuncAttributeMaxDynamicSharedMemorySize,
                            160 * 1024 - 128) != hipSuccess) { set_error("%s: hipFuncSetAttribute(dynamic LDS) failed", what); return DACO_E_HIP; }
    hipLaunchKernelGGL((scan_sparse_kernel<2, false, 4, true>), grid, dim3(256), lh_lds, s, sp);
  } else {
    const SparseVariant v = sparse_variant(ld, race, spl, sparse_many_workgroups((long)B * bpi));
    void *args[] = {&sp};
    if (hipLaunchKernel(v.fn, grid, dim3(256), args, v.lds, s) != hipSuccess) { set_error("%s: scan_sparse_kernel launch failed", what); return DACO_E_HIP; }
  }
  if (const int rc = launch_status("scan_sparse_kernel")) return rc;
  return record_event(ev_end, s, "ev_end");
}

#define DACO_SPARSE_ARGS stream, B, n, A, tau, tau_bstride, eta, eta_bstride, alpha, beta, head_id, head_slots, start, fixed_start, seed, iter, \
                         iter_offset, ant_gid0, ant_gid_bstride, paths, flags, dist, dist_bstride, costs, nbr, stats, workspace, \
                         workspace_bytes, ev_begin, ev_end
extern "C" int daco_tsp_sample_sparse(void *stream, int B, int n, int A, const float *tau, long tau_bstride, const float *eta,
                                      long eta_bstride, float alpha, float beta, const uint16_t *head_id, int head_slots, const int64_t *start,
                                      int fixed_start, uint64_t seed, uint64_t iter, const uint64_t *iter_offset,
                                      uint32_t ant_gid0, int ant_gid_bstride, int64_t *paths, int32_t *flags, const float *dist,
                                      long dist_bstride, float *costs, uint32_t *nbr, unsigned long long *stats, void *workspace,
                                      size_t workspace_bytes, void *ev_begin, void *ev_end) {
  return sample_sparse_impl(false, false, 0, 0, "daco_tsp_sample_sparse", DACO_SPARSE_ARGS);
}
extern "C" int daco_tsp_sample_race_head(void *stream, int B, int n, int A, const float *tau, long tau_bstride, const float *eta,
                                         long eta_bstride, float alpha, float beta, const uint16_t *head_id, int head_slots, const int64_t *start,
                                         int fixed_start, uint64_t seed, uint64_t iter, const uint64_t *iter_offset,
                                         uint32_t ant_gid0, int ant_gid_bstride, int64_t *paths, int32_t *flags, const float *dist,
                                         long dist_bstride, float *costs, uint32_t *nbr, unsigned long long *stats, void *workspace,
                                         size_t workspace_bytes, void *ev_begin, void *ev_end) {
  return sample_sparse_impl(true, false, 0, 0, "daco_tsp_sample_race_head", DACO_SPARSE_ARGS);
}
extern "C" int daco_tsp_sample_heads(void *stream, int race, int heads_ready, int head_live_max, int nbr_grouped, int B, int n, int A, const float *tau, long tau_bstride, const float *eta,
                                     long eta_bstride, float alpha, float beta, const uint16_t *head_id, int head_slots, const int64_t *start,
                                     int fixed_start, uint64_t seed, uint64_t iter, const uint64_t *iter_offset,
                                     uint32_t ant_gid0, int ant_gid_bstride, int64_t *paths, int32_t *flags, const float *dist,
                                     long dist_bstride, float *costs, uint32_t *nbr, unsigned long long *stats, void *workspace,
                                     size_t workspace_bytes, void *ev_begin, void *ev_end) {
  return sample_sparse_impl(race != 0, heads_ready != 0, head_live_max, nbr_grouped, "daco_tsp_sample_heads", DACO_SPARSE_ARGS);
}
```

deepaco_amd/engine/__init__.py:

```python
from .. import _lib
from .colonies import (BatchedCVRP, BatchedTSP, StreamedTSP, ant_sharded_cvrp, ant_sharded_tsp, run_kept_colony,
                       same_state)
from .common import MODES, RACE_NOISE, RACE_PHILOX, SCAN, SCAN_WAVE, _f32c, _stream, _workspace, stage_to_hip
from .cvrp_ops import cvrp_knn_graph, cvrp_sample, sample_backward
from .local_search import (HgsTables, TspLocalSearch, TwoOptTables, cvrp_local_search_, heuristic_dist, hgs_local_search_,
                           hgs_polar_angles, nls_, transposed_for_two_opt, two_opt_, two_opt_tables)
from .mkp_ops import (BatchedMKPVec, mkpv_backward, mkpv_check_flags, mkpv_sample, mkpv_update_, transformer_backward,
                      transformer_forward, transformer_forward_train)
from .rcpsp_ops import (RCPSP_FLAG_ORDER, RCPSP_FLAG_RESOURCE, RCPSP_MAX_HORIZON, RCPSP_MAX_N, RCPSP_MAX_R, RCPSP_NET_MAX_N,
                        BatchedRCPSP, rcpsp_backward, rcpsp_check_flags, rcpsp_net_backward, rcpsp_net_forward,
                        rcpsp_net_forward_train, rcpsp_sample, rcpsp_schedule)
from .sibling_colonies import (BATCHED_SIBLINGS, OBJ_KINDS, BatchedBPP, BatchedMKP, BatchedOP, BatchedPCTSP, BatchedSMTWTP,
                               BatchedSOP, sibling_objective, sibling_record_)
from .sibling_ops import SIB_KINDS, PickService, sibling_backward, sibling_sample
from .tsp_ops import (SPARSE_MAX_N, SPARSE_MIN_N, auto_head_k, head_table, heu_matrix, resolve_sampler, sparse_head,
                      sparse_tours16, sparse_workspace, sparsify_heuristic, take_auto_top, tsp_edge_backward, tsp_edge_logp, tsp_knn_graph,
                      tsp_sample, tsp_sample_sparse)
from .update import pheromone_update_, tour_costs, track_best_
```

deepaco_amd/engine/colonies.py:

```python
import torch

from .common import _f32c, _raise_flags, _require_gpu, _rows
from .cvrp_ops import cvrp_sample
from .local_search import HgsTables, TspLocalSearch, heuristic_dist, hgs_local_search_, hgs_polar_angles
from .tsp_ops import head_table, resolve_sampler, sparse_tours16, sparse_workspace, sparsify_heuristic, tsp_sample, tsp_sample_sparse
from .update import pheromone_update_, tour_costs, track_best_


def same_state(kept, now):
    return kept is not None and len(kept) == len(now) and all(
        (a is b) if torch.is_tensor(a) else (a == b) for a, b in zip(kept, now))


def _mmas_bounds(col, new_max):
    if not col.min_max:
        return None, None
    if col.max is None:
        col.pheromone *= (new_max / col.pheromone.amax(dim=(1, 2))).view(col.B, 1, 1)
    col.max = new_max
    if col._cmin is None:
        col._cmin = torch.full_like(new_max, col.min)
    return col._cmin, new_max


def _init_pheromone(col, pheromone, min_max, min):
    if min_max:
        col.min = 0.1 if min is None else min
        col.max = None
    col._cmin = None
    col.pheromone = torch.ones_like(col.distances) if pheromone is None else _f32c(pheromone).clone()
    if min_max and pheromone is None:
        col.pheromone = col.pheromone * col.min


def run_kept_colony(aco, col, n_iterations, shortest):
    dev = col.distances.device
    col.pheromone = aco.pheromone.detach().to(torch.float32).clone().contiguous().unsqueeze(0)
    col.lowest_cost = torch.as_tensor(aco.lowest_cost, dtype=torch.float32, device=dev).reshape(1).clone()
    col.shortest_path = shortest
    col.iteration = aco._calls
    if aco.min_max:
        col.min, col._cmin = aco.min, None
        col.max = None if aco.max is None else torch.as_tensor(aco.max, dtype=torch.float32, device=dev).reshape(1).clone()
    col._flags.zero_()
    col.run(n_iterations)
    aco._calls = col.iteration
    if aco.min_max and col.max is not None:
        aco.max = col.max[0]
    aco.pheromone = col.pheromone[0]
    aco.lowest_cost = col.lowest_cost[0]


class BatchedTSP:

    setup_path = None

    def __init__(self, distances, n_ants=20, decay=0.9, alpha=1, beta=1, elitist=False, min_max=False,
                 pheromone=None, heuristic=None, min=None, sampler="auto", seed=None, ant_gid0=0,
                 fixed_start=-1, local_search=None, inference=False, norm_passes=1):
        _require_gpu(distances)
        assert distances.dim() == 3
        self.distances = _f32c(distances)
        self.B, self.n = distances.shape[0], distances.shape[1]
        self.n_ants, self.decay, self.alpha, self.beta = n_ants, decay, alpha, beta
        self.elitist, self.min_max = elitist, min_max
        dev = distances.device
        _init_pheromone(self, pheromone, min_max, min)
        assert not min_max or self.min > 1e-9
        self.heuristic = (1 / self.distances) if heuristic is None else heuristic
        self.lowest_cost = torch.full((self.B,), float("inf"), device=dev)
        self.shortest_path = torch.zeros((self.B, self.n), dtype=torch.int64, device=dev)
        self.sampler = sampler
        self.seed = torch.initial_seed() if seed is None else seed
        self.iteration = 0
        self.ant_gid0 = ant_gid0
        self.fixed_start = fixed_start
        self.norm_passes = norm_passes
        assert local_search in (None, "2opt", "nls")
        self.local_search = local_search
        self.inference = inference
        self._ls = TspLocalSearch(self.distances)
        self.nls_counters = None
        self.head_k = None
        self._head = None
        self._sparse_ws = None
        self._heads_for = None
        self._flags = torch.zeros((self.B,), dtype=torch.int32, device=dev)
        self.fuse_head_rows = True

    def check_feasible(self):
        _raise_flags(self._flags, ((1, ValueError, "BatchedTSP: a transition row had no feasible candidate"),
                                   (4, RuntimeError, "BatchedTSP: the head table has more live entries per row than head_live_max")))

    def _heads_state(self, head, race):
        return (self.pheromone, self.pheromone._version, self.heuristic, head, bool(race), float(self.alpha), float(self.beta))

    def _heuristic_dist(self):
        return self._ls.heuristic_dist(self.heuristic)

    @torch.no_grad()
    def sparsify(self, k_sparse):
        self.heuristic = sparsify_heuristic(self.distances, k_sparse, path=self.setup_path)
        self.head_k = min(int(k_sparse), 127)
        self._head = None

    def resolved_sampler(self):
        if getattr(self, "_auto", None) is None:
            self._auto = {}
        return resolve_sampler(self.sampler, self.n, self.head_k, self.heuristic, self._auto, path=self.setup_path)

    def _head_table(self, k=None):
        if self._head is None or self._head[0] is not self.heuristic or (k is not None and self._head[2] != k):
            k = k if k is not None else (self.head_k if self.head_k is not None else max(1, min(127, self.n // 10)))
            self._head = (self.heuristic, head_table(self.heuristic, k, self.B, getattr(self, "_auto", None), path=self.setup_path), k)
        return self._head[1]

    @torch.no_grad()
    def step(self, events=None, _iter_dev=None, ls_events=None, want_paths=True):
        return self._step(events, _iter_dev, ls_events, want_paths)

    def _step(self, events=None, _iter_dev=None, ls_events=None, want_paths=True, resolved=None):
        sampler, hk = resolved or self.resolved_sampler()
        race_head = sampler == "race" and self.head_k is not None and 128 < self.n <= 1024
        heads = None
        if sampler == "scan_sparse" or race_head:
            head = self._head_table(hk)
            unit = float(self.alpha) == 1.0 and float(self.beta) == 1.0
            if self._sparse_ws is None:
                self._sparse_ws = sparse_workspace(self.distances.device, self.B, self.n, self.n_ants, unit_exponents=unit)
            fused = self.fuse_head_rows and unit
            grouped = fused and self.n_ants % 8 == 0 and self.local_search is None
            ready = same_state(self._heads_for, self._heads_state(head, race_head))
            compact = not want_paths and self.local_search is None
            paths, _, costs, nbr = tsp_sample_sparse(self.pheromone, self.heuristic, self.n_ants, head, self.alpha,
                                                     self.beta, seed=self.seed, it=self.iteration, ant_gid0=self.ant_gid0,
                                                     fixed_start=self.fixed_start, batch=self.B, events=events,
                                                     dist=self.distances, want_nbr=True, iter_dev=_iter_dev, race=race_head,
                                                     workspace=self._sparse_ws, heads_ready=ready, head_live_max=self._head[2],
                                                     nbr_grouped=grouped, flags=self._flags, want_paths=not compact)
            tours16 = sparse_tours16(self._sparse_ws, self.B, self.n, self.n_ants) if compact else None
            if fused:
                heads = {"eta": self.heuristic, "alpha": self.alpha, "beta": self.beta, "head": head, "race": race_head,
                         "workspace": self._sparse_ws, "nbr_grouped": grouped}
        else:
            tours16 = None
            paths, _, _, _, costs, nbr = tsp_sample(self.pheromone, self.heuristic, self.n_ants, self.alpha,
                                                    self.beta, mode=sampler, seed=self.seed, it=self.iteration,
                                                    ant_gid0=self.ant_gid0, fixed_start=self.fixed_start,
                                                    batch=self.B, events=events, dist=self.distances, want_nbr=True,
                                                    iter_dev=_iter_dev, norm_passes=self.norm_passes, flags=self._flags)
        if _iter_dev is None:
            self.iteration += 1
        if self.local_search is not None:
            paths, ls_costs = self._ls.improve(paths, self.local_search, self.inference, self.heuristic,
                                               counters=self.nls_counters, events=ls_events)
            costs, nbr = (tour_costs(self.distances, paths) if ls_costs is None else ls_costs), None
        new_max = track_best_(costs, paths, self.lowest_cost, self.shortest_path,
                              mmas_scale=self.n if self.min_max else None, tours16=tours16)
        cmin, cmax = _mmas_bounds(self, new_max)
        pheromone_update_(self.pheromone, paths, costs, self.decay, self.elitist, True, cmin, cmax, nbr=nbr, heads=heads)
        self._heads_for = self._heads_state(heads["head"], heads["race"]) if heads is not None else None
        return paths, costs

    @torch.no_grad()
    def run(self, n_iterations, graph=False):
        if not graph or n_iterations < 3:
            resolved = self.resolved_sampler()
            for _ in range(n_iterations):
                self._step(want_paths=False, resolved=resolved)
            return self.lowest_cost
        self._step(want_paths=False)
        dev = self.distances.device
        it_dev = torch.zeros(1, dtype=torch.int64, device=dev)
        torch.cuda.synchronize(dev)
        side = torch.cuda.Stream(device=dev)
        side.wait_stream(torch.cuda.current_stream(dev))
        with torch.cuda.stream(side):
            self._step(_iter_dev=it_dev, want_paths=False)
            it_dev += 1
        torch.cuda.current_stream(dev).wait_stream(side)
        g = torch.cuda.CUDAGraph()
        with torch.cuda.graph(g, stream=side):
            self._step(_iter_dev=it_dev, want_paths=False)
            it_dev += 1
        for _ in range(n_iterations - 2):
            g.replay()
        self.iteration += n_iterations - 1
        self._graph = g
        return self.lowest_cost


def _gathered(name):
    return property(lambda self: self._gather(name))


class StreamedTSP:

    def __init__(self, distances, parts=4, ant_gid0=0, pheromone=None, heuristic=None, **kw):
        _require_gpu(distances)
        B = distances.shape[0]
        parts = max(1, min(int(parts), B))
        dev = distances.device
        n_ants = kw.get("n_ants", 20)
        bounds = [(p * B) // parts for p in range(parts + 1)]
        self.B, self.n, self.n_ants = B, distances.shape[1], n_ants
        self.cols, self.streams, self.bounds = [], [], bounds
        cur = torch.cuda.current_stream(dev)
        for p in range(parts):
            lo, hi = bounds[p], bounds[p + 1]

            def part(t):
                return None if t is None else (t[lo:hi] if t.dim() == 3 else t)
            self.cols.append(BatchedTSP(distances[lo:hi], ant_gid0=ant_gid0 + lo * n_ants, pheromone=part(pheromone),
                                        heuristic=part(heuristic), **kw))
            st = torch.cuda.Stream(device=dev)
            st.wait_stream(cur)
            self.streams.append(st)
        self._dev = dev

    def _fork(self):
        cur = torch.cuda.current_stream(self._dev)
        for st in self.streams:
            st.wait_stream(cur)

    def sparsify(self, k_sparse):
        self._fork()
        for col, st in zip(self.cols, self.streams):
            with torch.cuda.stream(st):
                col.sparsify(k_sparse)
                col.heuristic = col.heuristic.contiguous()

    @property
    def iteration(self):
        return self.cols[0].iteration

    def step(self, events=None, want_paths=True):
        self._fork()
        for p, (col, st) in enumerate(zip(self.cols, self.streams)):
            with torch.cuda.stream(st):
                col.step(events=events[p] if events is not None else None, want_paths=want_paths)

    def join(self):
        cur = torch.cuda.current_stream(self._dev)
        for st in self.streams:
# ... 185 lines not shown
```

deepaco_amd/engine/tsp_ops.py:

```python
import numpy as np
import torch

from .. import _lib
from .common import MODES, RACE_NOISE, _bstride, _f32c, _grad_out, _on, _ptr, _require_gpu, _stream, _workspace


def tsp_sample(tau, eta, n_ants, alpha=1.0, beta=1.0, mode="scan", norm_passes=1, start=None,
               fixed_start=-1, noise=None, seed=0, it=0, ant_gid0=0, require_prob=False, batch=None,
               events=None, dist=None, want_nbr=False, iter_dev=None, ant_gid_bstride=0, flags=None):
    _require_gpu(tau, eta, start, noise)
    n = tau.shape[-1]
    B = batch or (tau.shape[0] if tau.dim() == 3 else (eta.shape[0] if eta.dim() == 3 else 1))
    dev = tau.device
    tau, tbs = _bstride(tau, n)
    eta, ebs = _bstride(eta, n)
    m = MODES[mode] if isinstance(mode, str) else int(mode)
    L = _lib.lib()
    with _on(dev):
        paths = torch.empty((B, n, n_ants), dtype=torch.int64, device=dev)
        logp = torch.empty((B, n - 1, n_ants), dtype=torch.float32, device=dev) if require_prob else None
        rowsum = torch.empty((B, n - 1, n_ants), dtype=torch.float32, device=dev) if require_prob else None
        if flags is None:
            flags = torch.zeros((B,), dtype=torch.int32, device=dev)
        if start is not None:
            start = start.to(torch.int64).contiguous().view(B, n_ants)
        if noise is not None:
            noise = _f32c(noise).view(B, n - 1, n_ants, n) if m == RACE_NOISE else _f32c(noise).view(B, n - 1, n_ants)
        costs, dbs = None, 0
        if dist is not None:
            _require_gpu(dist)
            dist, dbs = _bstride(dist, n)
            costs = torch.empty((B, n_ants), dtype=torch.float32, device=dev)
        nbr = torch.empty((B, n, n_ants), dtype=torch.int32, device=dev) if want_nbr else None
        ws = _workspace(dev, L.daco_tsp_sample_workspace_bytes(B, n, m), "sample")
        rc = L.daco_tsp_sample(_stream(dev), B, n, n_ants, tau.data_ptr(), tbs, eta.data_ptr(), ebs,
                               float(alpha), float(beta), m, int(norm_passes),
                               start.data_ptr() if start is not None else None, int(fixed_start),
                               noise.data_ptr() if noise is not None else None,
                               int(seed) & (2 ** 64 - 1), int(it), iter_dev.data_ptr() if iter_dev is not None else None,
                               int(ant_gid0) & 0xFFFFFFFF, int(ant_gid_bstride),
                               paths.data_ptr(), logp.data_ptr() if require_prob else None,
                               rowsum.data_ptr() if require_prob else None, flags.data_ptr(),
                               dist.data_ptr() if dist is not None else None, dbs,
                               costs.data_ptr() if costs is not None else None,
                               nbr.data_ptr() if nbr is not None else None,
                               ws.data_ptr(), ws.numel(),
                               events[0].cuda_event if events else None,
                               events[1].cuda_event if events else None)
    _lib.check(rc, "daco_tsp_sample")
    if dist is not None or want_nbr:
        return paths, logp, rowsum, flags, costs, nbr
    return paths, logp, rowsum, flags


SETUP_MAX_N = 1024


def _setup_path(path, n, *tensors):
    ok = 2 <= n <= SETUP_MAX_N and all(t is None or (t.is_cuda and t.dtype == torch.float32) for t in tensors)
    if path is None:
        return "hip" if ok else "torch"
    if path not in ("hip", "torch"):
        raise ValueError(f"path must be None, 'hip' or 'torch' (got {path!r})")
    if path == "hip" and not ok:
        raise _lib.DacoError(f"path='hip' takes float32 tensors on a HIP device with 2 <= n <= {SETUP_MAX_N} (n = {n})")
    return path


def sparsify_heuristic(dist, k, numer=None, path=None):
    n = dist.shape[-1]
    if _setup_path(path, n, dist, numer) == "torch":
        _, idx = torch.topk(dist, k=k, dim=-1, largest=False)
        sparse = torch.full_like(dist, 1e10)
        sparse.scatter_(-1, idx, torch.gather(dist, -1, idx))
        return (1 if numer is None else numer.unsqueeze(-2)) / sparse
    d = dist.detach()
    B = d.shape[0] if d.dim() == 3 else 1
    d = d if d.is_contiguous() else d.contiguous()
    nbs = 0
    if numer is not None:
        numer = numer.detach().contiguous()
        assert numer.shape[-1] == n and (numer.dim() == 1 or tuple(numer.shape) == (B, n))
# ... 49 lines not shown
    n = h.shape[-1]
    if not (SPARSE_MIN_N <= n <= SPARSE_MAX_N):
        return (None, None) if want_top else None
    if _setup_path(path, n, h) == "hip":
        k = _auto_head_k_hip(h, n, mass)
        return (k, None) if want_top else k
    h = h.to(torch.float32)
    top = torch.topk(h, min(127, n - 1), dim=-1).values
    tot = h.sum(dim=-1)
    ok63 = ((top[..., :63].sum(dim=-1) / tot) >= mass).float().mean()
    ok127 = ((top.sum(dim=-1) / tot) >= mass).float().mean()
    k_lds = _lds_head_k(n, top.shape[-1])
    ok_lds = ((top[..., :k_lds].sum(dim=-1) / tot) >= 1.0 - 1e-4).float().mean() if k_lds >= 8 else torch.zeros((), device=h.device)
    ok63, ok127, ok_lds = (float(x) for x in torch.stack((ok63, ok127, ok_lds)).tolist())
    k = k_lds if ok_lds >= 0.95 else (63 if ok63 >= 0.95 else (127 if ok127 >= 0.95 else None))
    return (k, top if k else None) if want_top else k


def _lds_head_k(n, most):
    lanes = min(16, (160 * 1024 - 128 - 4 * 528 - 4 * 514 * 2 - 32) // (n * 24))
    return min(62, 4 * lanes - 1, most)


def _auto_head_k_hip(h, n, mass):
    h, wbs = _bstride(h, n)
    B = h.shape[0] if h.dim() == 3 else 1
    k_lds = _lds_head_k(n, min(127, n - 1))
    dev = h.device
    with _on(dev):
        counts = torch.empty(3, dtype=torch.int32, device=dev)
        rc = _lib.lib().daco_head_stats(_stream(dev), B, n, h.data_ptr(), wbs, k_lds if k_lds >= 8 else 0, float(mass), 1.0 - 1e-4,
                                        counts.data_ptr())
    _lib.check(rc, "daco_head_stats")
    rows = np.float32(B * n)
    ok63, ok127, ok_lds = (float(np.float32(c) / rows) for c in counts.tolist())
    if k_lds < 8:
        ok_lds = 0.0
    return k_lds if ok_lds >= 0.95 else (63 if ok63 >= 0.95 else (127 if ok127 >= 0.95 else None))


_warned_sparse_range = False


def resolve_sampler(sampler, n, head_k, heuristic, cache, path=None):
    global _warned_sparse_range
    in_range = SPARSE_MIN_N <= n <= SPARSE_MAX_N
    if sampler == "scan_sparse" and not in_range:
        if not _warned_sparse_range:
            _warned_sparse_range = True
            import warnings
            warnings.warn(f"sampler='scan_sparse' covers {SPARSE_MIN_N} <= n <= {SPARSE_MAX_N}; n = {n} runs the dense scan "
                          f"(the same distribution)", RuntimeWarning, stacklevel=3)
        return "scan", None
    if sampler != "auto":
        return sampler, head_k
    if not in_range:
        return "scan", None
    if head_k is not None:
        return "scan_sparse", head_k
    hit = cache.get("auto_head")
    if hit is None or hit[0] is not heuristic:
        k, top = auto_head_k(heuristic, want_top=True, path=path)
        hit = cache["auto_head"] = (heuristic, k)
        cache.pop("auto_top", None)
        if top is not None:
            cache["auto_top"] = (heuristic, top)
    return ("scan_sparse", hit[1]) if hit[1] else ("scan", None)


def take_auto_top(cache, heuristic):
    hit = cache.pop("auto_top", None) if cache else None
    return hit[1] if hit is not None and hit[0] is heuristic else None


def head_table(heuristic, k, B, cache=None, path=None):
    h = heuristic.detach()
    top = take_auto_top(cache, heuristic)
    if _setup_path(path, h.shape[-1], h) == "hip":
        return sparse_head(h, k, path="hip", batch=B)
    h = h if h.dim() == 3 else h.unsqueeze(0).expand(B, *h.shape)
    return sparse_head(_f32c(h), k, top=top, path="torch")


def sparse_workspace(device, B, n, n_ants, unit_exponents=True):
    L = _lib.lib()
    nbytes = (L.daco_tsp_sparse_workspace_bytes if unit_exponents else L.daco_tsp_sparse_workspace_bytes_general)(B, n, n_ants)
    if nbytes == 0:
        raise ValueError(f"scan_sparse serves 129 <= n <= 1024 (n = {n})")
    return torch.empty(int(nbytes), dtype=torch.uint8, device=device)


def sparse_tours16(workspace, B, n, n_ants):
    off = int(_lib.lib().daco_tsp_sparse_tours_offset(B, n, n_ants))
    ld = 512 if n <= 512 else 1024
    return workspace[off:off + B * n_ants * ld * 2].view(torch.int16).view(B, n_ants, ld)


def tsp_sample_sparse(tau, eta, n_ants, head, alpha=1.0, beta=1.0, start=None, fixed_start=-1, seed=0, it=0, ant_gid0=0,
                      batch=None, events=None, dist=None, want_nbr=False, iter_dev=None, ant_gid_bstride=0, want_stats=False,
                      want_paths=True, race=False, workspace=None, heads_ready=False, head_live_max=0, nbr_grouped=False, flags=None):
    _require_gpu(tau, eta, start, head, workspace)
    assert not heads_ready or workspace is not None
    n = tau.shape[-1]
    B = batch or (tau.shape[0] if tau.dim() == 3 else (eta.shape[0] if eta.dim() == 3 else 1))
    dev = tau.device
    tau, tbs = _bstride(tau, n)
    eta, ebs = _bstride(eta, n)
    assert head.dtype == torch.int16 and head.is_contiguous() and tuple(head.shape) in ((B, n, 64), (B, n, 128))
    L = _lib.lib()
    with _on(dev):
        paths = torch.empty((B, n, n_ants), dtype=torch.int64, device=dev) if want_paths else None
        if flags is None:
            flags = torch.zeros((B,), dtype=torch.int32, device=dev)
        if start is not None:
            start = start.to(torch.int64).contiguous().view(B, n_ants)
        costs, dbs = None, 0
        if dist is not None:
            _require_gpu(dist)
            dist, dbs = _bstride(dist, n)
            costs = torch.empty((B, n_ants), dtype=torch.float32, device=dev)
        assert not (want_nbr and nbr_grouped) or n_ants % 8 == 0, "the grouped table wants a multiple of eight ants"
        nbr = torch.empty((B, n, n_ants), dtype=torch.int32, device=dev) if want_nbr else None
        stats = torch.zeros(3, dtype=torch.int64, device=dev) if want_stats else None
        unit = float(alpha) == 1.0 and float(beta) == 1.0
        nbytes = (L.daco_tsp_sparse_workspace_bytes if unit else L.daco_tsp_sparse_workspace_bytes_general)(B, n, n_ants)
        if nbytes == 0:
            raise ValueError(f"scan_sparse serves 129 <= n <= 1024 (n = {n})")
        ws = workspace if workspace is not None else _workspace(dev, nbytes, "sample_sparse")
        assert ws.numel() >= nbytes
        rc = L.daco_tsp_sample_heads(_stream(dev), int(bool(race)), int(bool(heads_ready)), int(head_live_max), int(bool(nbr_grouped)), B, n, n_ants, tau.data_ptr(), tbs, eta.data_ptr(), ebs, float(alpha),
                                      float(beta), head.data_ptr(), int(head.shape[2]), start.data_ptr() if start is not None else None,
                                      int(fixed_start), int(seed) & (2 ** 64 - 1), int(it),
                                      iter_dev.data_ptr() if iter_dev is not None else None, int(ant_gid0) & 0xFFFFFFFF,
                                      int(ant_gid_bstride), paths.data_ptr() if paths is not None else None, flags.data_ptr(),
                                      dist.data_ptr() if dist is not None else None, dbs,
                                      costs.data_ptr() if costs is not None else None,
                                      nbr.data_ptr() if nbr is not None else None,
                                      stats.data_ptr() if stats is not None else None, ws.data_ptr(), ws.numel(),
                                      events[0].cuda_event if events else None, events[1].cuda_event if events else None)
    _lib.check(rc, "daco_tsp_sample_heads")
    out = (paths, flags, costs, nbr)
    return out + (stats,) if want_stats else out


def tsp_knn_graph(coords, k_sparse, diag=1e9, want_dist=True):
    _require_gpu(coords)
    coords = _f32c(coords)
    B, n, _ = coords.shape
    dev = coords.device
    E = n * int(k_sparse)
    with _on(dev):
        dist = torch.empty((B, n, n), dtype=torch.float32, device=dev) if want_dist else None
        ei = torch.empty((B, 2, E), dtype=torch.int64, device=dev)
        ea = torch.empty((B, E, 1), dtype=torch.float32, device=dev)
        src32 = torch.empty((B * E,), dtype=torch.int32, device=dev)
        dst32 = torch.empty((B * E,), dtype=torch.int32, device=dev)
        src = ei[:, 0]
        dst = ei[:, 1]
        if B > 1:
            src_c = torch.empty((B, E), dtype=torch.int64, device=dev)
            dst_c = torch.empty((B, E), dtype=torch.int64, device=dev)
        else:
            src_c, dst_c = src, dst
        rc = _lib.lib().daco_tsp_knn_graph_csr(_stream(dev), B, n, int(k_sparse), coords.data_ptr(), float(diag),
                                               _ptr(dist), src_c.data_ptr(), dst_c.data_ptr(),
                                               ea.data_ptr(), src32.data_ptr(), dst32.data_ptr())
        if B > 1:
            ei[:, 0], ei[:, 1] = src_c, dst_c
    _lib.check(rc, "daco_tsp_knn_graph_csr")
    ei._daco_csr = (src32, dst32, n, int(k_sparse), ei._version)
    return dist, ei, ea


def heu_matrix(n, edge_index, heu, fill=0.0, add=0.0, check=False):
    _require_gpu(edge_index, heu)
    B, E = heu.shape
    assert edge_index.shape == (B, 2, E) and edge_index.dtype == torch.int64
    ei = edge_index.contiguous()
    heu = _f32c(heu.detach())
    dev = heu.device
    with _on(dev):
        out = torch.empty((B, n, n), dtype=torch.float32, device=dev)
        bad = torch.zeros((1,), dtype=torch.int32, device=dev) if check else None
        rc = _lib.lib().daco_heu_matrix(_stream(dev), B, n, E, ei.data_ptr(), heu.data_ptr(), float(fill), float(add),
                                        out.data_ptr(), _ptr(bad))
    _lib.check(rc, "daco_heu_matrix")
    if check and int(bad.item()):
        raise IndexError(f"heu_matrix: {int(bad.item())} edge(s) with a node id outside [0, {n})")
    return out


def _edge_destinations(who, edge_index, heu, n, k, pheromone, *others):
    dense = "engine.sample_backward (the dense path) takes such input"
    if pheromone is not None:
        raise _lib.DacoError(f"{who}: the edge-list path replays a fresh colony (pheromone = ones), pheromone must be None; {dense}")
    for t in (heu, edge_index) + others:
        if not t.is_cuda:
            raise _lib.DacoError(f"{who}: runs on a HIP device only (got a CPU tensor), there is no CPU fallback; {dense}")
    B, E = heu.shape
    n, k = int(n), int(k)
    if k < 1 or E != n * k or tuple(edge_index.shape) != (B, 2, E) or edge_index.dtype != torch.int64:
        raise _lib.DacoError(f"{who}: heu [B, n k] and an int64 edge_index [B, 2, n k] expected (n = {n}, k = {k}, heu {tuple(heu.shape)}, "
                             f"edge_index {tuple(edge_index.shape)}); {dense}")
    csr = getattr(edge_index, "_daco_csr", None)
    if (csr is not None and csr[2] == n and csr[3] == k and csr[4] == edge_index._version and csr[1].numel() == B * E
            and csr[1].device == heu.device):
        return None, 0, csr[1].data_ptr(), csr[1]
    if getattr(edge_index, "_daco_regular", None) != (n, k, edge_index._version):
        rows = torch.arange(n, device=edge_index.device).repeat_interleave(k)
        if not bool((edge_index[:, 0] == rows).all()):
            raise _lib.DacoError(f"{who}: edge_index is not in the regular layout (edge j k + t leaves node j, as engine.tsp_knn_graph "
                                 f"writes it); {dense}")
# ... 41 lines not shown
```

deepaco_amd/engine/update.py:

```python
import torch

from .. import _lib
from .common import _bstride, _f32c, _on, _require_gpu, _stream, _workspace


def tour_costs(dist, paths, closed=True):
    _require_gpu(dist, paths)
    n = dist.shape[-1]
    B, length, A = paths.shape
    dist, dbs = _bstride(dist, n)
    paths = paths.contiguous()
    dev = paths.device
    with _on(dev):
        costs = torch.empty((B, A), dtype=torch.float32, device=dev)
        rc = _lib.lib().daco_tour_costs(_stream(dev), B, n, length, A, dist.data_ptr(), dbs, paths.data_ptr(),
                                        int(closed), costs.data_ptr())
    _lib.check(rc, "daco_tour_costs")
    return costs


def track_best_(costs, paths, lowest, shortest=None, mmas_scale=None, tours16=None):
    _require_gpu(costs, paths, lowest, shortest, tours16)
    assert costs.dtype == torch.float32 and costs.is_contiguous()
    B, A = costs.shape
    assert lowest.dtype == torch.float32 and lowest.is_contiguous() and lowest.numel() == B
    dev = costs.device
    with _on(dev):
        mx = torch.empty((B,), dtype=torch.float32, device=dev) if mmas_scale is not None else None
        if paths is None:
            assert tours16 is not None and tours16.dtype == torch.int16 and tours16.is_contiguous() and shortest is not None
            assert tuple(tours16.shape[:2]) == (B, A)
            rc = _lib.lib().daco_track_best_tours16(_stream(dev), B, int(shortest.shape[1]), A, int(tours16.shape[2]), costs.data_ptr(),
                                                    tours16.data_ptr(), lowest.data_ptr(), shortest.data_ptr(), None,
                                                    mx.data_ptr() if mx is not None else None,
                                                    float(mmas_scale) if mmas_scale is not None else 0.0)
            _lib.check(rc, "daco_track_best_tours16")
            return mx
        length = paths.shape[1]
        assert paths.is_contiguous() and tuple(paths.shape) == (B, length, A)
        rc = _lib.lib().daco_track_best(_stream(dev), B, length, A, costs.data_ptr(), paths.data_ptr(), lowest.data_ptr(),
                                        shortest.data_ptr() if shortest is not None else None, None,
                                        mx.data_ptr() if mx is not None else None,
                                        float(mmas_scale) if mmas_scale is not None else 0.0)
    _lib.check(rc, "daco_track_best")
    return mx


def pheromone_update_(tau, paths, costs, decay, elitist=False, symmetric=True, clamp_min=None,
                      clamp_max=None, floor=0.0, nbr=None, weights=None, hub=0, heads=None):
    _require_gpu(tau, paths, costs, clamp_min, clamp_max)
    assert tau.dim() == 3 and tau.dtype == torch.float32 and tau.is_contiguous()
    B, n, _ = tau.shape
    if paths is None:
        assert nbr is not None and symmetric
        length, A = n, costs.shape[-1]
    else:
        _, length, A = paths.shape
        paths = paths.contiguous()
    pptr = paths.data_ptr() if paths is not None else None
    costs = _f32c(costs)
    if weights is not None:
        weights = _f32c(weights)
    dev = tau.device
    L = _lib.lib()
    with _on(dev):
        ws = _workspace(dev, L.daco_pheromone_update_workspace_bytes(B, n, length, A), "update")
        if heads is not None:
            assert symmetric and length == n
            eta, ebs = _bstride(heads["eta"], n)
            head, sws = heads["head"], heads["workspace"]
            _require_gpu(eta, head, sws)
            rc = L.daco_pheromone_update_heads(_stream(dev), B, n, A, tau.data_ptr(), pptr, costs.data_ptr(), float(decay),
                                               int(bool(elitist)), clamp_min.data_ptr() if clamp_min is not None else None,
                                               clamp_max.data_ptr() if clamp_max is not None else None, float(floor),
                                               nbr.data_ptr() if nbr is not None else None,
                                               weights.data_ptr() if weights is not None else None, ws.data_ptr(), ws.numel(),
                                               eta.data_ptr(), ebs, float(heads["alpha"]), float(heads["beta"]), head.data_ptr(),
                                               int(head.shape[2]), int(bool(heads.get("race", False))),
                                               int(bool(heads.get("nbr_grouped", False))) if nbr is not None else 0, sws.data_ptr(), sws.numel())
            _lib.check(rc, "daco_pheromone_update_heads")
            return tau
        rc = L.daco_pheromone_update(_stream(dev), B, n, length, A, tau.data_ptr(), pptr,
                                     costs.data_ptr(), float(decay), int(bool(elitist)), int(bool(symmetric)),
                                     clamp_min.data_ptr() if clamp_min is not None else None,
                                     clamp_max.data_ptr() if clamp_max is not None else None,
                                     float(floor), nbr.data_ptr() if nbr is not None else None,
                                     weights.data_ptr() if weights is not None else None, int(hub),
                                     ws.data_ptr(), ws.numel())
    _lib.check(rc, "daco_pheromone_update")
    return tau
```

deepaco_amd/tsp/aco.py:

```python
import os
import sys

import torch

try:
    from deepaco_amd import engine
except ImportError:
    sys.path.insert(0, os.path.dirname(os.path.dirname(os.path.dirname(os.path.abspath(__file__)))))
    from deepaco_amd import engine


class ACO():

    NORM_PASSES = 1
    setup_path = None
    FIXED_START = -1

    def __init__(self,
                 distances,
                 n_ants=20,
                 decay=0.9,
                 alpha=1,
                 beta=1,
                 elitist=False,
# ... 5 lines not shown
                 *,
                 sampler='auto',
                 seed=None,
                 ):
        distances = engine.stage_to_hip(distances)
        pheromone = engine.stage_to_hip(pheromone, distances)
        heuristic = engine.stage_to_hip(heuristic, distances)
        self.problem_size = len(distances)
        self.distances = distances
        self.n_ants = n_ants
        self.decay = decay
        self.alpha = alpha
        self.beta = beta
        self.elitist = elitist
        self.min_max = min_max

        if min_max:
            if min is not None:
                assert min > 1e-9
            else:
                min = 0.1
            self.min = min
            self.max = None

        if pheromone is None:
            self.pheromone = torch.ones_like(self.distances)
            if min_max:
                self.pheromone = self.pheromone * self.min
        else:
            self.pheromone = pheromone

        self.heuristic = 1 / distances if heuristic is None else heuristic

        self.shortest_path = None
        self.lowest_cost = float('inf')

        self.device = distances.device
        self.sampler = sampler
        self.seed = torch.initial_seed() if seed is None else seed
        self._calls = 0

    @torch.no_grad()
    def sparsify(self, k_sparse):
        self.heuristic = engine.sparsify_heuristic(self.distances, k_sparse, path=self.setup_path)
        self._head_k = min(int(k_sparse), 127)

    def resolved_sampler(self):
        cache = self.__dict__.setdefault("_auto", {})
        return engine.resolve_sampler(self.sampler, self.problem_size, self.__dict__.get("_head_k"), self.heuristic, cache,
                                      path=self.setup_path)

    def _head_table(self, k=None):
        hit = self.__dict__.get("_head")
        if hit is None or hit[0] is not self.heuristic or (k is not None and hit[2] != k):
            k = k or self.__dict__.get("_head_k") or max(1, min(127, self.problem_size // 10))
            hit = (self.heuristic, engine.head_table(self.heuristic, k, 1, self.__dict__.get("_auto"), path=self.setup_path), k)
            self._head = hit
        return hit[1]

    def sample(self):
        paths, log_probs = self.gen_path(require_prob=True)
        costs = self.gen_path_costs(paths)
        return costs, log_probs

    @torch.no_grad()
    def run(self, n_iterations):
        if "gen_path" in self.__dict__ or type(self).gen_path_costs is not ACO.gen_path_costs \
                or getattr(self, "local_search_type", None) is not None:
            return self._run_plain(n_iterations)
        sampler, hk = self.resolved_sampler()
        key = (self.distances, self.heuristic, sampler, hk, self.n_ants, self.decay, self.alpha, self.beta, bool(self.elitist),
               bool(self.min_max), self.seed)
        hit = self.__dict__.get("_colony")
        if hit is None or not engine.same_state(hit[0], key):
            eta = self.heuristic.detach().to(torch.float32).contiguous().unsqueeze(0)
            col = engine.BatchedTSP(self.distances.detach().float().contiguous().unsqueeze(0), n_ants=self.n_ants, decay=self.decay,
                                    alpha=self.alpha, beta=self.beta, elitist=self.elitist, min_max=self.min_max, heuristic=eta,
                                    min=self.min if self.min_max else None, sampler=sampler, seed=self.seed,
                                    fixed_start=self.FIXED_START, norm_passes=self.NORM_PASSES)
            col.setup_path = self.setup_path
            if sampler == "scan_sparse":
                col.head_k = hk
                col._head = (eta, self._head_table(hk), hk)
            hit = self._colony = (key, col)
        col = hit[1]
        shortest = (self.shortest_path.clone() if self.shortest_path is not None else
                    torch.zeros(self.problem_size, dtype=torch.int64, device=self.distances.device)).reshape(1, -1).contiguous()
        engine.run_kept_colony(self, col, n_iterations, shortest)
        self._last_flags = col._flags
        self.shortest_path = col.shortest_path[0]
        return self.lowest_cost

    @torch.no_grad()
    def _run_plain(self, n_iterations):
        for _ in range(n_iterations):
            paths = self.gen_path(require_prob=False)
            costs = self.gen_path_costs(paths)

            best_cost, best_idx = costs.min(dim=0)
            if best_cost < self.lowest_cost:
                self.shortest_path = paths[:, best_idx]
                self.lowest_cost = best_cost
                if self.min_max:
                    max = self.problem_size / self.lowest_cost
                    if self.max is None:
                        self.pheromone *= max / self.pheromone.max()
                    self.max = max

            self.update_pheronome(paths, costs)

        return self.lowest_cost

    @torch.no_grad()
    def update_pheronome(self, paths, costs):
        tau = self.pheromone.detach().to(torch.float32).clone().contiguous().unsqueeze(0)
        cmin = cmax = None
        if self.min_max:
            cmin = torch.full((1,), float(self.min), device=tau.device)
            cmax = torch.as_tensor(self.max, dtype=torch.float32, device=tau.device).reshape(1).contiguous()
        engine.pheromone_update_(tau, paths.unsqueeze(0), costs.unsqueeze(0), self.decay, self.elitist, True,
                                 cmin, cmax)
        self.pheromone = tau[0]

    update_pheromone = update_pheronome

    @torch.no_grad()
    def gen_path_costs(self, paths):
        assert paths.shape == (self.problem_size, self.n_ants)
        return engine.tour_costs(self.distances, paths.unsqueeze(0))[0]

    def gen_path(self, require_prob=False, *, _start=None, _noise=None):
        if _noise is not None:
            mode, start = "race_noise", _start
        else:
            mode, start = self.sampler, _start
        hk = None
        if mode in ("auto", "scan_sparse"):
            mode, hk = self.resolved_sampler()
            if mode == "scan_sparse" and (require_prob or start is not None):
                mode = "scan"
        fixed = self.FIXED_START
        if _noise is not None and start is None and fixed < 0:
            raise ValueError("noise injection needs the start nodes too (_start)")
        start = None if start is None else start.view(1, -1)
        noise = None if _noise is None else _noise.unsqueeze(0)
        it = self._calls
        self._calls += 1
        if require_prob and torch.is_grad_enabled() and self.heuristic.requires_grad:
            from deepaco_amd.autograd import TspSampleFn
            paths, logp, flags = TspSampleFn.apply(self.heuristic, self.pheromone.detach(), self.n_ants, self.alpha,
                                                   self.beta, mode, self.NORM_PASSES, start, fixed, noise,
                                                   self.seed, it)
            self._last_flags = flags
            return paths, logp
        if mode == "scan_sparse":
            paths, flags, _, _ = engine.tsp_sample_sparse(self.pheromone.detach(), self.heuristic.detach(), self.n_ants,
                                                          self._head_table(hk), self.alpha, self.beta, fixed_start=fixed,
                                                          seed=self.seed, it=it, batch=1)
            self._last_flags = flags
            return paths[0]
        paths, logp, rowsum, flags = engine.tsp_sample(
            self.pheromone.detach(), self.heuristic.detach(), self.n_ants, self.alpha, self.beta, mode=mode,
            norm_passes=self.NORM_PASSES, start=start, fixed_start=fixed, noise=noise,
            seed=self.seed, it=it, require_prob=require_prob, batch=1)
        self._last_flags = flags
        if require_prob:
# ... 23 lines not shown
```

include/deepaco_hip.h:

```cpp
#ifndef DEEPACO_HIP_H
#define DEEPACO_HIP_H

#include <stddef.h>
#include <stdint.h>

#ifdef __cplusplus
extern "C" {
#endif

#define DACO_VERSION 129

#define DACO_OK 0
#define DACO_E_BADARG (-1)
#define DACO_E_TOOLARGE (-2)
#define DACO_E_HIP (-3)
#define DACO_E_WORKSPACE (-4)

#define DACO_RACE_NOISE 0
#define DACO_RACE_PHILOX 1
#define DACO_SCAN 2
#define DACO_SCAN_WAVE 3

#define DACO_MAX_NODES 4096

int daco_version(void);
const char *daco_last_error(void);

int daco_vec_for_n(int n);
int daco_ld_for_n(int n);

size_t daco_tsp_sample_workspace_bytes(int B, int n, int mode);
int daco_tsp_sample(void *stream, int B, int n, int A,
                    const float *tau, long tau_bstride, const float *eta, long eta_bstride,
                    float alpha, float beta, int mode, int norm_passes,
                    const int64_t *start, int fixed_start, const float *noise,
                    uint64_t seed, uint64_t iter, const uint64_t *iter_offset, uint32_t ant_gid0,
                    int ant_gid_bstride,
                    int64_t *paths, float *logp, float *rowsum, int32_t *flags,
                    const float *dist, long dist_bstride, float *costs, uint32_t *nbr,
                    void *workspace, size_t workspace_bytes, void *ev_begin, void *ev_end);

size_t daco_tsp_sparse_workspace_bytes(int B, int n, int A);
size_t daco_tsp_sparse_workspace_bytes_general(int B, int n, int A);
size_t daco_tsp_sparse_tours_offset(int B, int n, int A);
int daco_tsp_sparse_resident_per_cu(int n, int head_slots, int race);
int daco_tsp_sparse_split_tours(int mode);
int daco_tsp_sample_sparse(void *stream, int B, int n, int A,
                           const float *tau, long tau_bstride, const float *eta, long eta_bstride,
                           float alpha, float beta, const uint16_t *head_id, int head_slots,
                           const int64_t *start, int fixed_start,
                           uint64_t seed, uint64_t iter, const uint64_t *iter_offset, uint32_t ant_gid0,
                           int ant_gid_bstride,
                           int64_t *paths, int32_t *flags,
                           const float *dist, long dist_bstride, float *costs, uint32_t *nbr,
                           unsigned long long *stats,
                           void *workspace, size_t workspace_bytes, void *ev_begin, void *ev_end);

int daco_tsp_sample_race_head(void *stream, int B, int n, int A,
                              const float *tau, long tau_bstride, const float *eta, long eta_bstride,
                              float alpha, float beta, const uint16_t *head_id, int head_slots,
                              const int64_t *start, int fixed_start,
                              uint64_t seed, uint64_t iter, const uint64_t *iter_offset, uint32_t ant_gid0,
                              int ant_gid_bstride,
                              int64_t *paths, int32_t *flags,
                              const float *dist, long dist_bstride, float *costs, uint32_t *nbr,
                              unsigned long long *stats,
                              void *workspace, size_t workspace_bytes, void *ev_begin, void *ev_end);

int daco_tsp_sample_heads(void *stream, int race, int heads_ready, int head_live_max, int nbr_grouped, int B, int n, int A,
                          const float *tau, long tau_bstride, const float *eta, long eta_bstride,
                          float alpha, float beta, const uint16_t *head_id, int head_slots,
                          const int64_t *start, int fixed_start,
                          uint64_t seed, uint64_t iter, const uint64_t *iter_offset, uint32_t ant_gid0,
                          int ant_gid_bstride,
                          int64_t *paths, int32_t *flags,
                          const float *dist, long dist_bstride, float *costs, uint32_t *nbr,
                          unsigned long long *stats,
                          void *workspace, size_t workspace_bytes, void *ev_begin, void *ev_end);

size_t daco_directed_table_bytes(int B, int n, int A);
int daco_cvrp_sample(void *stream, int B, int n, int A,
                     const float *tau, long tau_bstride, const float *eta, long eta_bstride,
                     float alpha, float beta, const float *demand, float capacity, int mode,
                     const float *noise, int noise_steps, uint64_t seed, uint64_t iter,
                     const uint64_t *iter_offset, uint32_t ant_gid0, int ant_gid_bstride, int Lmax, int64_t *paths, float *logp,
                     float *rowsum,
                     int32_t *lens, int32_t *flags,
                     const float *dist, long dist_bstride, float *costs, void *next_table,
                     void *workspace, size_t workspace_bytes, const double *demand64, double capacity64,
                     void *ev_begin, void *ev_end);

int daco_track_best(void *stream, int B, int len, int A, const float *costs, const int64_t *paths,
                    float *lowest, int64_t *shortest, int32_t *best_idx, float *mmas_max, float mmas_scale);
int daco_track_best_tours16(void *stream, int B, int len, int A, int ld, const float *costs, const uint16_t *tours16,
                            float *lowest, int64_t *shortest, int32_t *best_idx, float *mmas_max, float mmas_scale);

int daco_prob_matrix(void *stream, int B, int n, const float *tau, long tau_bstride,
                     const float *eta, long eta_bstride, float alpha, float beta, int mode,
                     void *workspace, size_t workspace_bytes);
int daco_pick_move(void *stream, int B, int n, int A, const void *prob_workspace,
                   size_t workspace_bytes, int mode, const int64_t *prev, const float *mask,
                   const float *noise, uint64_t seed, uint64_t iter, uint32_t ant_gid0, int step,
                   int64_t *actions, float *logp, float *rowsum, int32_t *flags);

#define DACO_SIB_SOP 3
#define DACO_SIB_PCTSP 4
#define DACO_SIB_OP 5
#define DACO_SIB_MKP 6
size_t daco_sibling_workspace_bytes(int B, int n, int mode);
int daco_sibling_sample(void *stream, int kind, int B, int n, int A,
                        const float *tau, long tau_bstride, const float *eta, long eta_bstride,
                        float alpha, float beta, const float *aux_vec, const float *aux_mat,
                        long aux_mat_bstride, float scalar0, const float *item_weights, int m,
                        int mode, const int64_t *start, const float *noise, int noise_steps,
                        uint64_t seed, uint64_t iter, uint32_t ant_gid0, int Lmax,
                        int64_t *paths, float *logp, float *rowsum, int32_t *lens, int32_t *flags,
                        void *workspace, size_t workspace_bytes);

#define DACO_SIB_SMTWTP 7
#define DACO_SIB_BPP 8
long daco_sibling_objective(void *stream, int kind, int B, int n, int rows, int A, const int64_t *paths,
                            const int32_t *lens, const float *vec0, const float *vec1, const float *vec2,
                           const float *mat, long mat_bstride, double capacity, int elitist, const float *scale,
                           float *obj, double *obj64, float *key, float *weight);
long daco_sibling_record(void *stream, int rule, int B, int len, int A, const float *key, const float *obj,
                         const double *obj64, const int64_t *paths, int row0, float *best_obj, double *best_obj64,
                        int64_t *best_sol, int32_t *best_idx, float *mmas_max, float mmas_n, const float *mmas_scale);

int daco_sibling_backward(void *stream, int kind, int B, int n, int A, int rows,
                          const float *tau, long tau_bstride, const float *eta, long eta_bstride,
                          float alpha, float beta, const float *aux_vec, const float *aux_mat,
                          long aux_mat_bstride, float scalar0, const float *item_weights, int m,
                          const int64_t *paths, const float *rowsum, const float *grad_logp,
                          const int32_t *lens, float *grad_eta);

int daco_sample_backward(void *stream, int B, int n, int A, int rows,
                         const float *tau, long tau_bstride, const float *eta, long eta_bstride,
                         float alpha, float beta, const int64_t *paths, const float *rowsum,
                         const float *grad_logp, const int32_t *lens, const float *demand,
                         float capacity, float *grad_eta, const double *demand64, double capacity64);

long daco_tsp_edge_logp(void *stream, int B, int n, int k, int A, const float *heu, const int64_t *edge_dst,
                        long edge_dst_bstride, const int32_t *edge_dst32, float eps, float beta, const int64_t *paths,
                        float *logp, float *rowsum);
long daco_tsp_edge_backward(void *stream, int B, int n, int k, int A, const float *heu, const int64_t *edge_dst,
                            long edge_dst_bstride, const int32_t *edge_dst32, float eps, float beta, const int64_t *paths,
                            const float *rowsum, const float *grad_logp, float *grad_heu);

int daco_tour_costs(void *stream, int B, int n, int len, int A, const float *dist,
                    long dist_bstride, const int64_t *paths, int closed, float *costs);

size_t daco_pheromone_update_workspace_bytes(int B, int n, int len, int A);
int daco_pheromone_update(void *stream, int B, int n, int len, int A, float *tau,
                          const int64_t *paths, const float *costs, float decay, int elitist,
                          int symmetric, const float *clamp_min, const float *clamp_max,
                          float floor_val, const uint32_t *nbr, const float *weights, int hub,
                          void *workspace, size_t workspace_bytes);

int daco_pheromone_update_heads(void *stream, int B, int n, int A, float *tau,
                                const int64_t *paths, const float *costs, float decay, int elitist,
                                const float *clamp_min, const float *clamp_max, float floor_val,
                                const uint32_t *nbr, const float *weights, void *workspace, size_t workspace_bytes,
                                const float *eta, long eta_bstride, float alpha, float beta,
                                const uint16_t *head_id, int head_slots, int race, int nbr_grouped,
                                void *sparse_workspace, size_t sparse_workspace_bytes);

int daco_allreduce_delta_tau(void *comm, void *stream, float *delta, size_t count);

int daco_two_opt(void *stream, int B, int T, int n, const float *dist, const float *dist_T, long dist_bstride,
                 uint16_t *tours, long max_iterations, int32_t *sweeps);

size_t daco_two_opt_tables_bytes(int B, int n);
int daco_two_opt_prepare(void *stream, int B, int n, const float *dist, long dist_bstride, void *tables, size_t tables_bytes);
int daco_two_opt_nbr(void *stream, int B, int T, int n, const float *dist, long dist_bstride, const void *tables,
                     const void *tables_T, uint16_t *tours, long max_iterations, int32_t *sweeps);
int daco_two_opt_auto(void *stream, int B, int T, int n, const float *dist, const float *dist_T, long dist_bstride,
                      const void *tables, const void *tables_T, uint16_t *tours, long max_iterations, int32_t *sweeps);

int daco_tsp_nls(void *stream, int B, int T, int n, const float *dist, long dist_bstride, const void *tables,
                 const void *tables_T, const float *hdist, long hdist_bstride, const void *htables, const void *htables_T,
                 uint16_t *tours, long max_iterations, int T_nls, long T_p, int32_t *sweeps, float *costs,
                 unsigned long long *counters);

size_t daco_gnn_param_floats(int feats);
size_t daco_gnn_workspace_bytes(int n, int E);
int daco_gnn_forward(void *stream, int n, int E, int feats, const float *x, const int32_t *src,
                     const int32_t *dst, const int32_t *rowptr, const int32_t *perm,
                     const float *edge_attr, const float *params, float *heu, float *emb,
                     void *workspace, size_t workspace_bytes);

size_t daco_gnn_train_workspace_bytes(int n, int E, int G);
int daco_gnn_train_forward(void *stream, int n, int E, int feats, int G, const float *x, const int32_t *src,
                           const int32_t *dst, const int32_t *rowptr, const int32_t *perm, const float *edge_attr,
                           const float *params, float *heu, float *stats_out, const float *fixed_stats, void *workspace,
                           size_t workspace_bytes);
int daco_gnn_train_backward(void *stream, int n, int E, int feats, int G, const float *x, const int32_t *src,
                            const int32_t *dst, const int32_t *rowptr, const int32_t *perm, const int32_t *rowptr_dst,
                            const int32_t *perm_dst, const float *edge_attr, const float *params, const float *heu,
                            const float *grad_heu, float *grad_params, int fixed_stats, void *workspace, size_t workspace_bytes);

int daco_cvrp_local_search(void *stream, int B, int n, int A, int Lmax, const float *dist, long dist_bstride,
                           const float *demand, float capacity, int64_t *paths, int max_moves, int32_t *lens,
                           int32_t *moves);

size_t daco_hgs_table_bytes(int n, int nb_granular);
int daco_hgs_prepare(void *stream, int B, int n, const double *matrix, long bstride, int nb_granular, void *tables);
size_t daco_hgs_workspace_bytes(int B, int n, int A, int Lmax, int nb_granular);
int daco_hgs_local_search(void *stream, int B, int n, int A, int Lmax, int nstages, const double *const *matrices,
                          const double *const *matrices_t, const long *bstrides, const void *const *tables, const int *counts, const double *demand,
                          double capacity, int nb_granular, int64_t *paths, int32_t *status, int32_t *stats,
                          void *workspace, size_t workspace_bytes);

size_t daco_hgs_workspace_bytes_ss(int B, int n, int A, int Lmax, int nb_granular);
long daco_hgs_local_search_ss(void *stream, int B, int n, int A, int Lmax, int nstages, const double *const *matrices,
                              const double *const *matrices_t, const long *bstrides, const void *const *tables, const int *counts, const double *demand,
                              double capacity, int nb_granular, int64_t *paths, int32_t *status, int32_t *stats,
                              void *workspace, size_t workspace_bytes, const double *xy, const int32_t *polar);

int daco_tsp_knn_graph(void *stream, int B, int n, int k, const float *coords, float diag, float *dist,
                       int64_t *edge_src, int64_t *edge_dst, float *edge_attr);
int daco_tsp_knn_graph_csr(void *stream, int B, int n, int k, const float *coords, float diag, float *dist,
                           int64_t *edge_src, int64_t *edge_dst, float *edge_attr, int32_t *src32, int32_t *dst32);

long daco_cvrp_knn_graph(void *stream, int B, int n1, int k, const void *dist, int dist_f64, long dist_bstride,
                         int64_t *edge_index, float *edge_attr, int32_t *src32, int32_t *dst32, int32_t *rowptr, int32_t *perm);

int daco_heu_matrix(void *stream, int B, int n, int E, const int64_t *edge_index, const float *heu, float fill, float add,
                    float *out, int32_t *bad);

long daco_sparsify(void *stream, int B, int n, int k, const float *dist, long dist_bstride, const float *numer,
                  long numer_bstride, float *out);
long daco_sparse_head(void *stream, int B, int n, int k, const float *weights, long w_bstride, uint16_t *ids);
long daco_head_stats(void *stream, int B, int n, const float *weights, long w_bstride, int k_lds, double mass,
                    double mass_lds, int32_t *counts);

int daco_mkpv_sample(void *stream, int B, int n, int A, int m, const float *tau, long tau_bstride,
                     const float *eta, long eta_bstride, float alpha, float beta,
                     const float *item_weights, const float *price, int mode, const float *noise,
                     int noise_steps, uint64_t seed, uint64_t iter, uint32_t ant_gid0, int Lmax,
                     int64_t *sols, int32_t *lens, float *logp, float *rowsum, float *objs, int32_t *flags);

int daco_mkpv_backward(void *stream, int B, int n, int A, int m, int rows, const float *tau, long tau_bstride,
                       const float *eta, long eta_bstride, float alpha, float beta, const float *item_weights,
                       const int64_t *sols, const float *rowsum, const float *grad_logp, const int32_t *lens,
                       float *grad_eta);

int daco_mkpv_update(void *stream, int B, int n, int A, int rows, const int64_t *sols, const int32_t *lens,
                     const float *objs, const float *Q, float decay, int elitist, int min_max, float tmin,
                     float tmax, float *tau, float *best_obj, int64_t *best_sol);

size_t daco_transformer_param_floats(int feats);
size_t daco_transformer_workspace_bytes(int G, int n);
int daco_transformer_forward(void *stream, int G, int n, int feats, const float *src, const float *params,
                             size_t param_floats, float *out, void *workspace, size_t workspace_bytes);

size_t daco_transformer_saved_floats(int G, int n);
size_t daco_transformer_train_workspace_bytes(int G, int n);
int daco_transformer_forward_train(void *stream, int G, int n, int feats, const float *src, const float *params,
                                   size_t param_floats, float *out, float *saved, size_t saved_floats, void *workspace,
                                   size_t workspace_bytes);
int daco_transformer_backward(void *stream, int G, int n, int feats, const float *src, const float *params,
                              size_t param_floats, const float *saved, size_t saved_floats, const float *grad_out,
                              float *grad_params, void *workspace, size_t workspace_bytes);

#define DACO_RCPSP_MAX_N 256
#define DACO_RCPSP_MAX_R 8
#define DACO_RCPSP_MAX_HORIZON 8192
#define DACO_RCPSP_FLAG_ORDER 4
#define DACO_RCPSP_FLAG_RESOURCE 8
int daco_rcpsp_schedule(void *stream, int B, int n, int A, int R, int horizon, int E, const int32_t *duration,
                        const int32_t *resources, const int32_t *capacity, const int32_t *earliest_start,
                        const int32_t *latest_start, const int32_t *succ_ptr, const int32_t *succ_idx,
                        const int64_t *routes, int32_t *starts, int32_t *costs, int32_t *flags);
size_t daco_rcpsp_workspace_bytes(int B, int n);
int daco_rcpsp_sample(void *stream, int B, int n, int A, int R, int horizon, int E, const int32_t *duration,
                      const int32_t *resources, const int32_t *capacity, const int32_t *earliest_start,
                      const int32_t *latest_start, const int32_t *succ_ptr, const int32_t *succ_idx,
                      const float *indegree, const float *adjacency, const float *tau, long tau_bstride,
                      const float *eta, long eta_bstride, float alpha, float beta, double gamma, double c, int mode,
                      const float *noise, uint64_t seed, uint64_t iter, uint32_t ant_gid0, int64_t *routes,
                      float *logp, float *rowsum, int32_t *starts, int32_t *costs, int32_t *flags, void *workspace,
                      size_t workspace_bytes);
int daco_rcpsp_backward(void *stream, int B, int n, int A, const float *indegree, const float *adjacency,
                        const float *tau, long tau_bstride, const float *eta, long eta_bstride, float alpha, float beta,
                        double gamma, double c, const int64_t *routes, const float *rowsum, const float *grad_logp,
                        float *grad_eta);
int daco_rcpsp_track(void *stream, int B, int n, int A, const int64_t *routes, const int32_t *starts, const int32_t *costs,
                     double Q, int elitist, int alias, int min_max, float tmin, int32_t *best_cost, int32_t *best_idx,
                     int64_t *best_route, int32_t *best_schedule, int64_t *upd_routes, float *upd_weights,
                     float *clamp_min, float *clamp_max);

#define DACO_RCPSP_NET_MAX_N 128
size_t daco_rcpsp_net_param_floats(void);
size_t daco_rcpsp_net_workspace_bytes(int B, int n);
long daco_rcpsp_net_forward(void *stream, int B, int n, int feats, const float *x, const uint8_t *relation, const float *params,
                            float eps, float *heu, float *logit, float *emb, void *workspace, size_t workspace_bytes);

size_t daco_rcpsp_net_train_saved_bytes(int B, int n);
size_t daco_rcpsp_net_train_workspace_bytes(int B, int n);
long daco_rcpsp_net_train_forward(void *stream, int B, int n, int feats, const float *x, const uint8_t *relation,
                                  const float *params, float eps, float *heu, float *logit, float *stats, void *saved,
                                  size_t saved_bytes);
long daco_rcpsp_net_train_backward(void *stream, int B, int n, int feats, const float *x, const uint8_t *relation,
                                   const float *params, const void *saved, size_t saved_bytes, const float *grad_heu,
                                   float *grad_params, float *grad_blocks, void *workspace, size_t workspace_bytes);

#ifdef __cplusplus
}
#endif
#endif
```

Baseline: 57.51 million ant-tours/s.

## Add uniform-tail sparse sampling path that reads only tau outside the head

After: 59.26 million ant-tours/s, median of 6. 1.03x the previous value.

```diff
diff --git a/deepaco_amd/_lib.py b/deepaco_amd/_lib.py
--- a/deepaco_amd/_lib.py
+++ b/deepaco_amd/_lib.py
@@ -35,6 +35,11 @@
                                    _vp, _l, _vp, _vp, _vp, _vp, _sz, _vp, _vp]),
     "daco_pheromone_update_heads": (_i, [_vp, _i, _i, _i, _vp, _vp, _vp, _f, _i, _vp, _vp, _f, _vp, _vp, _vp, _sz,
                                          _vp, _l, _f, _f, _vp, _i, _i, _i, _vp, _sz]),
+    "daco_tsp_sample_heads_ut": (_l, [_vp, _i, _i, _i, _i, _i, _i, _vp, _l, _vp, _l, _vp, _i, _vp, _i, _u64, _u64, _vp, _u32, _i, _vp, _vp,
+                                      _vp, _l, _vp, _vp, _vp, _vp, _sz, _vp, _vp, _vp, _f]),
+    "daco_pheromone_update_heads_ut": (_l, [_vp, _i, _i, _i, _vp, _vp, _vp, _f, _i, _vp, _vp, _f, _vp, _vp, _vp, _sz,
+                                            _vp, _i, _i, _vp, _sz, _vp, _f]),
+    "daco_head_eta": (_l, [_vp, _i, _i, _vp, _l, _vp, _i, _vp, _vp]),
     "daco_allreduce_delta_tau": (_i, [_vp, _vp, _vp, _sz]),
     "daco_tour_costs": (_i, [_vp, _i, _i, _i, _i, _vp, _l, _vp, _i, _vp]),
     "daco_pheromone_update_workspace_bytes": (_sz, [_i, _i, _i, _i]),
diff --git a/deepaco_amd/csrc/daco_colony_setup.hip b/deepaco_amd/csrc/daco_colony_setup.hip
--- a/deepaco_amd/csrc/daco_colony_setup.hip
+++ b/deepaco_amd/csrc/daco_colony_setup.hip
@@ -123,6 +123,55 @@
   }
 }
 
+__global__ void __launch_bounds__(256)
+head_eta_kernel(int B, int n, int slots, const float *eta, long eta_bs, const uint16_t *ids, float *head_eta, uint32_t *verdict) {
+  __shared__ uint32_t bm[4][32];
+  const int lane = threadIdx.x & 63, wave = threadIdx.x >> 6;
+  const long row = (long)blockIdx.x * 4 + wave;
+  if (row >= (long)B * n) return;
+  const int b = (int)(row / n), r = (int)(row - (long)b * n);
+  const float *er = eta + (size_t)b * eta_bs + (size_t)r * n;
+  const uint16_t *id = ids + (size_t)row * slots;
+  const int cnt = id[slots - 1] < slots - 1 ? id[slots - 1] : slots - 1;
+  if (lane < 32) bm[wave][lane] = 0u;
+  __builtin_amdgcn_wave_barrier();
+  float eh[2];
+  bool live[2];
+#pragma unroll
+  for (int j = 0; j < 2; ++j) {
+    const int m = lane + 64 * j;
+    const int k = m < slots ? (int)id[m] : n;
+    live[j] = m < cnt && k < n;
+    eh[j] = live[j] ? er[k] : 0.0f;
+    if (live[j]) atomicOr(&bm[wave][k >> 5], 1u << (k & 31));
+    if (m < slots) head_eta[(size_t)row * slots + m] = eh[j];
+  }
+  __builtin_amdgcn_wave_barrier();
+  uint32_t lo = 0xFFFFFFFFu, hi = 0u;
+  for (int k = lane; k < n; k += 64) {
+    if ((bm[wave][k >> 5] >> (k & 31)) & 1u) continue;
+    const uint32_t u = __float_as_uint(er[k]);
+    lo = u < lo ? u : lo;
+    hi = u > hi ? u : hi;
+  }
+#pragma unroll
+  for (int o = 32; o >= 1; o >>= 1) {
+    const uint32_t l2 = (uint32_t)__shfl_xor((int)lo, o, 64), h2 = (uint32_t)__shfl_xor((int)hi, o, 64);
+    lo = l2 < lo ? l2 : lo;
+    hi = h2 > hi ? h2 : hi;
+  }
+  const bool tail = lo <= hi;
+  const float c = __uint_as_float(lo);
+  bool bad = tail && (lo != hi || lo >= 0x7f800000u);
+#pragma unroll
+  for (int j = 0; j < 2; ++j) bad = bad || (tail && live[j] && !(eh[j] >= c));
+  const bool any_bad = __ballot(bad) != 0;
+  if (lane == 0) {
+    if (any_bad) atomicOr(verdict + 0, 1u);
+    if (tail) { atomicMax(verdict + 1, ~lo); atomicMax(verdict + 2, hi); }
+  }
+}
+
 __device__ inline double cs_wave_sum(double x) {
 #pragma unroll
   for (int m = 32; m >= 1; m >>= 1) x += __shfl_xor(x, m, 64);
@@ -240,3 +289,17 @@
 #undef DACO_CS_STATS
   return launch_status("head_stats_kernel");
 }
+
+extern "C" long daco_head_eta(void *stream, int B, int n, const float *eta, long eta_bstride, const uint16_t *head_id, int head_slots,
+                              float *head_eta, uint32_t *verdict) {
+  if (B <= 0 || n < 2 || !eta || !head_id || !head_eta || !verdict || eta_bstride < 0 || (head_slots != 64 && head_slots != 128)) {
+    set_error("daco_head_eta: bad argument (B=%d n=%d head_slots=%d)", B, n, head_slots);
+    return DACO_E_BADARG;
+  }
+  if (const int rc = cs_check_size("daco_head_eta", B, n)) return rc;
+  hipStream_t s = (hipStream_t)stream;
+  if (const int rc = launch_status(zero_async(verdict, 3 * sizeof(uint32_t), s), "daco_head_eta (clearing the verdict)")) return rc;
+  hipLaunchKernelGGL(head_eta_kernel, dim3((unsigned)(((long)B * n + 3) / 4)), dim3(256), 0, s, B, n, head_slots, eta, eta_bstride, head_id,
+                     head_eta, verdict);
+  return launch_status("head_eta_kernel");
+}
diff --git a/deepaco_amd/csrc/daco_costs_update.hip b/deepaco_amd/csrc/daco_costs_update.hip
--- a/deepaco_amd/csrc/daco_costs_update.hip
+++ b/deepaco_amd/csrc/daco_costs_update.hip
@@ -163,6 +163,32 @@
   }
 }
 
+constexpr int UT_PRE = 4;
+__device__ __forceinline__ void ut_prefetch_rows(HeadUt (&pre)[UT_PRE], int n, int b, int i0, int Rv, const HeadEmit &he, int lane, int wave) {
+#pragma unroll
+  for (int j = 0; j < UT_PRE; ++j) {
+    const int rr = wave + 4 * j;
+    const size_t slot0 = ((size_t)b * n + i0 + (rr < Rv ? rr : 0)) * (16 * he.spl);
+    head_ut_fetch(pre[j], n, he.heta + slot0, he.hid + slot0, he.spl, lane);
+  }
+}
+template <int CH>
+__device__ __forceinline__ void emit_rows_of_wave_ut(const HeadUt (&pre)[UT_PRE], int n, int ch, int b, int i0, int Rv, const float *rows,
+                                                     const HeadEmit &he, uint32_t *bm, int lane, int wave) {
+#pragma unroll
+  for (int j = 0; j < UT_PRE; ++j) {
+    const int rr = wave + 4 * j;
+    if (rr < Rv)
+      emit_head_row_ut<CH>(n, ch, rows + rr * n, he.tail_c, pre[j], bm, he.hrow + ((size_t)b * n + i0 + rr) * sp_head_row_bytes(he.spl), he.spl, he.dead, lane);
+  }
+  for (int rr = wave + 4 * UT_PRE; rr < Rv; rr += 4) {
+    const size_t row = (size_t)b * n + i0 + rr;
+    HeadUt h;
+    head_ut_fetch(h, n, he.heta + row * (16 * he.spl), he.hid + row * (16 * he.spl), he.spl, lane);
+    emit_head_row_ut<CH>(n, ch, rows + rr * n, he.tail_c, h, bm, he.hrow + row * sp_head_row_bytes(he.spl), he.spl, he.dead, lane);
+  }
+}
+
 template <bool SYM, int HEADS, bool GT = false>
 __global__ void __launch_bounds__(256, 4)
 deposit_rows_kernel(int n, int A, int R, int hub, float *tau, const uint32_t *nbr, const float *costs, const float *weights,
@@ -182,6 +208,8 @@
   const uint32_t *tab = GT ? nbr + (size_t)b * ((A + 7) >> 3) * n * 8 + (size_t)i0 * 8
                            : nbr + ((size_t)b * n + i0) * A;
   const float *cs = costs + (size_t)b * A, *wt = weights ? weights + (size_t)b * A : nullptr;
+  HeadUt ut_pre[HEADS == 3 ? UT_PRE : 1];
+  if constexpr (SYM && HEADS == 3) ut_prefetch_rows(ut_pre, n, b, i0, Rv, he, threadIdx.x & 63, threadIdx.x >> 6);
   constexpr int LDU = 6;
   auto load_chunk = [&](int c0, int buf, int t0, int nt) {
     const int m = min(DEP_CHUNK, ahi - c0);
@@ -304,6 +332,10 @@
     const int lane = threadIdx.x & 63, wave = threadIdx.x >> 6;
     const bool vec4 = he.ch > 0;
     const int ch = vec4 ? he.ch : -he.ch;
+    if constexpr (HEADS == 3) {
+      if (ch <= 2) emit_rows_of_wave_ut<2>(ut_pre, n, ch, b, i0, Rv, rows, he, head_bm[wave], lane, wave);
+      else emit_rows_of_wave_ut<4>(ut_pre, n, ch, b, i0, Rv, rows, he, head_bm[wave], lane, wave);
+    } else
     if (ch <= 2) { if (vec4) emit_rows_of_wave<HEADS == 2, 2, true>(n, b, i0, Rv, rows, he, head_bm[wave], lane, wave);
                    else emit_rows_of_wave<HEADS == 2, 2, false>(n, b, i0, Rv, rows, he, head_bm[wave], lane, wave); }
     else { if (vec4) emit_rows_of_wave<HEADS == 2, 4, true>(n, b, i0, Rv, rows, he, head_bm[wave], lane, wave);
@@ -520,7 +552,8 @@
                                                     nbr, costs, weights, decay, elitist ? best : nullptr, clamp_min, clamp_max, floor_val, he)
 #define DACO_DEPOSIT_SYM(H) do { if (grouped) DACO_DEPOSIT_SYM_G(H, true); else DACO_DEPOSIT_SYM_G(H, false); } while (0)
   const bool grouped = nbr_in != nullptr && he.nbr_grouped != 0;
-  if (!he.eta) DACO_DEPOSIT_SYM(0);
+  if (he.heta) DACO_DEPOSIT_SYM(3);
+  else if (!he.eta) DACO_DEPOSIT_SYM(0);
   else if (!he.race) DACO_DEPOSIT_SYM(1);
   else DACO_DEPOSIT_SYM(2);
 #undef DACO_DEPOSIT_SYM
@@ -559,3 +592,23 @@
   return pheromone_update_impl(stream, B, n, n, A, tau, paths, costs, decay, elitist, 1, clamp_min, clamp_max, floor_val, nbr_in, weights, 0,
                                workspace, workspace_bytes, he);
 }
+
+extern "C" long daco_pheromone_update_heads_ut(void *stream, int B, int n, int A, float *tau, const int64_t *paths, const float *costs,
+                                              float decay, int elitist, const float *clamp_min, const float *clamp_max, float floor_val,
+                                              const uint32_t *nbr_in, const float *weights, void *workspace, size_t workspace_bytes,
+                                              const uint16_t *head_id, int head_slots, int nbr_grouped, void *sparse_workspace,
+                                              size_t sparse_workspace_bytes, const float *head_eta, float tail_c) {
+  if (!head_eta || !head_id || !sparse_workspace || !(tail_c >= 0.0f)) { set_error("daco_pheromone_update_heads_ut: bad argument"); return DACO_E_BADARG; }
+  if (head_slots != 64 && head_slots != 128) { set_error("daco_pheromone_update_heads_ut: head_slots = %d (64 or 128)", head_slots); return DACO_E_BADARG; }
+  if (n <= 128 || n > 1024) { set_error("daco_pheromone_update_heads_ut: n=%d outside 129..1024 (the sizes daco_tsp_sample_heads serves)", n); return DACO_E_TOOLARGE; }
+  if ((n & 3) != 0 || ((uintptr_t)tau & 15) != 0) { set_error("daco_pheromone_update_heads_ut: the uniform-tail mode needs n %% 4 == 0 and 16-byte-aligned rows of tau (n=%d)", n); return DACO_E_BADARG; }
+  const size_t need = daco_tsp_sparse_workspace_bytes(B, n, A);
+  if (sparse_workspace_bytes < need) { set_error("daco_pheromone_update_heads_ut: sparse workspace %zu < %zu bytes", sparse_workspace_bytes, need); return DACO_E_WORKSPACE; }
+  const HeadWs ws = HeadWs::carve(sparse_workspace, B, n, A);
+  HeadEmit he;
+  he.hid = head_id; he.hrow = ws.hrow; he.heta = head_eta; he.tail_c = tail_c;
+  he.spl = head_slots / 16; he.nbr_grouped = nbr_grouped ? 1 : 0;
+  he.dead = ws.ld; he.ch = ws.ld / 256;
+  return pheromone_update_impl(stream, B, n, n, A, tau, paths, costs, decay, elitist, 1, clamp_min, clamp_max, floor_val, nbr_in, weights, 0,
+                               workspace, workspace_bytes, he);
+}
diff --git a/deepaco_amd/csrc/daco_head_rows.h b/deepaco_amd/csrc/daco_head_rows.h
--- a/deepaco_amd/csrc/daco_head_rows.h
+++ b/deepaco_amd/csrc/daco_head_rows.h
@@ -117,6 +117,65 @@
   emit_head_row_pre<RACE, CH, VEC4>(n, ch, tr, h, bm, hl, pr, spl, dead, lane);
 }
 
+struct HeadUt {
+  float eh[2];
+  uint32_t idp;
+  int cnt;
+};
+__device__ __forceinline__ void head_ut_fetch(HeadUt &h, int n, const float *heta, const uint16_t *ids, int spl, int lane) {
+  const int kh = 16 * spl;
+  h.cnt = ids[kh - 1] < kh - 1 ? ids[kh - 1] : kh - 1;
+  uint32_t idp = 0;
+#pragma unroll
+  for (int j = 0; j < 2; ++j) {
+    const int m = lane + 64 * j;
+    idp |= (uint32_t)(m < kh ? (int)ids[m] : n) << (16 * j);
+    h.eh[j] = m < kh ? heta[m] : 0.0f;
+  }
+  h.idp = idp;
+}
+template <int CH>
+__device__ __forceinline__ void emit_head_row_ut(int n, int ch, const float *tr, float c, const HeadUt &h, uint32_t *bm, char *hl,
+                                                 int spl, int dead, int lane) {
+  const int kh = 16 * spl, ls = sp_lane_bytes(spl);
+  const int cnt = h.cnt;
+  const float4 c4 = make_float4(c, c, c, c);
+  if (lane < 32) bm[lane] = 0u;
+  __builtin_amdgcn_wave_barrier();
+#pragma unroll
+  for (int j = 0; j < 2; ++j) { const int m = lane + 64 * j, id = (int)((h.idp >> (16 * j)) & 0xFFFFu); if (m < cnt && id < n) atomicOr(&bm[id >> 5], 1u << (id & 31)); }
+  __builtin_amdgcn_wave_barrier();
+  float part = 0.0f;
+#pragma unroll
+  for (int q = 0; q < CH; ++q) {
+    if (q < ch) {
+      const int k0 = (q * 64 + lane) * 4;
+      float4 t;
+      sp_load4<true>(tr, n, k0, t);
+      const float4 v = sp_mul4_masked(t, c4, n, k0);
+      const uint32_t w = bm[(k0 >> 5) & 31] >> (k0 & 31);
+      part = part + ((w & 1u) ? 0.0f : v.x);
+      part = part + ((w & 2u) ? 0.0f : v.y);
+      part = part + ((w & 4u) ? 0.0f : v.z);
+      part = part + ((w & 8u) ? 0.0f : v.w);
+    }
+  }
+  const float T = readlane_f(wave_scan_add(part), 63);
+#pragma unroll
+  for (int j = 0; j < 2; ++j) {
+    const int m = lane + 64 * j;
+    if (m < kh) {
+      const int id = (int)((h.idp >> (16 * j)) & 0xFFFFu);
+      const bool live = m < cnt && id < n;
+      const float pid = live ? tr[id] * h.eh[j] : 0.0f;
+      char *hs = hl + (m / spl) * ls;
+      *reinterpret_cast<float *>(hs + (m % spl) * 4) = m == kh - 1 ? T : pid;
+      *reinterpret_cast<uint16_t *>(hs + spl * 4 + (m % spl) * 2) = (uint16_t)(live && m != kh - 1 ? id : dead);
+    }
+  }
+  __builtin_amdgcn_wave_barrier();
+}
+
 struct HeadEmit {
   const float *eta = nullptr;
   long eta_bs = 0;
@@ -125,6 +184,8 @@
   float *P = nullptr;
   int spl = 4, ch = 2, dead = 512, race = 0;
   int nbr_grouped = 0;
+  const float *heta = nullptr;
+  float tail_c = 0.0f;
 };
 
 }
diff --git a/deepaco_amd/csrc/daco_sample_kernel.h b/deepaco_amd/csrc/daco_sample_kernel.h
--- a/deepaco_amd/csrc/daco_sample_kernel.h
+++ b/deepaco_amd/csrc/daco_sample_kernel.h
@@ -50,8 +50,8 @@
   uint16_t *tours16 = nullptr;
   const float *tau = nullptr, *eta = nullptr;
   long tau_bs = 0, eta_bs = 0;
+  float tail_c = 0.0f;
   float alpha = 1.0f, beta = 1.0f;
-  int row_vec = 0;
   int nbr_grouped = 0;
   int lh_kl = 0, lh_kmax = 0;
   RcpspDev rc;
diff --git a/deepaco_amd/csrc/daco_scan_sparse.hip b/deepaco_amd/csrc/daco_scan_sparse.hip
--- a/deepaco_amd/csrc/daco_scan_sparse.hip
+++ b/deepaco_amd/csrc/daco_scan_sparse.hip
@@ -31,19 +31,65 @@
   emit_head_row<RACE, CH, VEC4>(n, ch, tr, er, hid + row * (16 * spl), bm[wave], hrow + row * sp_head_row_bytes(spl), P + row * (256 * ch), spl, dead, lane);
 }
 
+template <int CH>
+__global__ void __launch_bounds__(256)
+sparse_prepass_ut_kernel(int B, int n, int ch, const float *tau, long tau_bs, const float *heta, float tail_c, const uint16_t *hid,
+                         char *hrow, int spl, int dead) {
+  __shared__ uint32_t bm[4][32];
+  const int lane = threadIdx.x & 63, wave = threadIdx.x >> 6;
+  const long row = (long)blockIdx.x * 4 + wave;
+  if (row >= (long)B * n) return;
+  const int b = (int)(row / n), r = (int)(row - (long)b * n);
+  HeadUt h;
+  head_ut_fetch(h, n, heta + row * (16 * spl), hid + row * (16 * spl), spl, lane);
+  emit_head_row_ut<CH>(n, ch, tau + b * tau_bs + (long)r * n, tail_c, h, bm[wave], hrow + row * sp_head_row_bytes(spl), spl, dead, lane);
+}
+
+typedef uint32_t sp_u32x4 __attribute__((ext_vector_type(4)));
+typedef uint32_t sp_u32x2 __attribute__((ext_vector_type(2)));
 struct SpRowSrc { const float *p; };
-__device__ __forceinline__ float4 sp_row4(const SpRowSrc &r, int k0) { return *reinterpret_cast<const float4 *>(r.p + k0); }
-
-template <int CHD, bool TAIL>
-__device__ __forceinline__ int sparse_row_walk(const SpRowSrc &rowp, const uint8_t *flg, const uint32_t *bm, int lane, float ur) {
+struct SpRowUT { __amdgpu_buffer_rsrc_t t; float c; };
+struct SpRowTE { __amdgpu_buffer_rsrc_t t, e; };
+__device__ __forceinline__ __amdgpu_buffer_rsrc_t sp_row_rsrc(const float *row, int n) {
+  return __builtin_amdgcn_make_buffer_rsrc((void *)row, 0, (int)((uint32_t)n * 4u), 0x00020000);
+}
+__device__ __forceinline__ int sp_lane_off(const SpRowSrc &, int lane) { return lane; }
+template <class Src> __device__ __forceinline__ int sp_lane_off(const Src &, int lane) {
+  int lo = lane * 16;
+  asm volatile("" : "+v"(lo));
+  return lo;
+}
+__device__ __forceinline__ float4 sp_row4(const SpRowSrc &r, int c, int lo) { return *reinterpret_cast<const float4 *>(r.p + (c * 64 + lo) * 4); }
+__device__ __forceinline__ float4 sp_row4(const SpRowUT &r, int c, int lo) {
+  const sp_u32x4 t = __builtin_amdgcn_raw_buffer_load_b128(r.t, lo + c * 1024, 0, 0);
+  return make_float4(__uint_as_float(t.x) * r.c, __uint_as_float(t.y) * r.c, __uint_as_float(t.z) * r.c, __uint_as_float(t.w) * r.c);
+}
+__device__ __forceinline__ float4 sp_row4(const SpRowTE &r, int c, int lo) {
+  const sp_u32x4 t = __builtin_amdgcn_raw_buffer_load_b128(r.t, lo + c * 1024, 0, 0), e = __builtin_amdgcn_raw_buffer_load_b128(r.e, lo + c * 1024, 0, 0);
+  return make_float4(__uint_as_float(t.x) * __uint_as_float(e.x), __uint_as_float(t.y) * __uint_as_float(e.y),
+                     __uint_as_float(t.z) * __uint_as_float(e.z), __uint_as_float(t.w) * __uint_as_float(e.w));
+}
+
+typedef const __attribute__((address_space(4))) SampleParams *sp_args_t;
+template <bool UT>
+__device__ __forceinline__ auto sp_row_of(const float *base, sp_args_t pa, int b, int row, int ld, int n) {
+  if constexpr (UT) asm volatile("" : "+s"(pa));
+  if constexpr (UT) return SpRowUT{sp_row_rsrc(pa->tau + (size_t)b * pa->tau_bs + (size_t)row * n, n), pa->tail_c};
+  else return SpRowSrc{base + (size_t)row * ld};
+}
+
+template <int CHD, bool TAIL, class Src>
+__device__ __forceinline__ int sparse_row_walk(const Src &rowp, const uint8_t *flg, const uint32_t *bm, int lane, float ur) {
   constexpr int NJ = CHD * 4;
   float run[16];
   float acc = 0.0f;
   uint32_t pos = 0;
+  const int lo = sp_lane_off(rowp, lane);
 #pragma unroll
   for (int c = 0; c < CHD; ++c) {
     const int k0 = (c * 64 + lane) * 4;
-    const float4 rv = sp_row4(rowp, k0);
+    if constexpr (std::is_same<Src, SpRowTE>::value) __builtin_amdgcn_sched_barrier(0);
+    const float4 rv = sp_row4(rowp, c, lo);
     float f[4];
     if constexpr (TAIL) {
       const uint32_t w = bm[(k0 >> 5) & 31] >> (k0 & 31);
@@ -91,8 +137,6 @@
   return ((jsel >> 2) * 64 + L) * 4 + (jsel & 3);
 }
 
-typedef uint32_t sp_u32x4 __attribute__((ext_vector_type(4)));
-typedef uint32_t sp_u32x2 __attribute__((ext_vector_type(2)));
 __device__ inline float sp_at_least_denorm(float x) {
   float y;
   asm("v_max_f32 %0, 1, %1" : "=v"(y) : "v"(x));
@@ -107,9 +151,10 @@
 static_assert(SP_ST_DEAD >= 16 * SP_EW * 2 + 4 * 512 * 2, "ST: early parts and the inverse table of four ants inside the dead bytes");
 
 static_assert(std::is_trivially_copyable<SampleParams>::value, "SampleParams is read back from the kernel-argument segment as plain bytes");
-template <int CHD, bool RACE, int SPL, bool LH = false, bool ST = false>
+template <int CHD, bool RACE, int SPL, bool LH = false, bool ST = false, bool UT = false>
 __global__ void __launch_bounds__(256, LH ? 1 : (ST ? 8 : (CHD == 2 ? (RACE ? 4 : 6) : 5)))
 scan_sparse_kernel(const SampleParams p) {
+  static_assert(!UT || !RACE, "the uniform-tail mode: scan draw");
   static_assert(!LH || (CHD == 2 && !RACE && SPL == 4), "the LDS-heads variant: n <= 512, scan draw, 64-slot heads");
   static_assert(!ST || (CHD == 2 && !RACE && SPL == 4 && !LH), "the split-tour variant: n <= 512, scan draw, 64-slot heads, not LH");
   constexpr int APW = 4, APB = LH ? 4 : 16;
@@ -140,10 +185,10 @@
   const bool active = a0 < A && (!LH || wave == 0);
   const int a = a0 + q < A ? a0 + q : A - 1;
   const uint32_t gid = p.ant_gid0 + (uint32_t)(b * (p.gid_bstride ? p.gid_bstride : A) + a);
-  const float *Pb = p.P + (size_t)b * n * p.ld;
+  const float *Pb = UT ? nullptr : p.P + (size_t)b * n * p.ld;
   const char *hrb = (const char *)p.hval + (size_t)b * n * ROWB;
   const __amdgpu_buffer_rsrc_t hres = __builtin_amdgcn_make_buffer_rsrc((void *)hrb, 0, (int)((uint32_t)n * ROWB), 0x00020000);
-#define SP_ROW_OF(pv) SpRowSrc{Pb + (size_t)(pv) * p.ld}
+#define SP_ROW_OF(pv) sp_row_of<UT>(Pb, (sp_args_t)__builtin_amdgcn_kernarg_segment_ptr(), b, pv, p.ld, n)
   uint32_t sls = (uint32_t)s * LS;
   asm volatile("" : "+v"(sls));
   uint8_t *fl = flag_mem + (wave * APW + q) * FLP;
@@ -297,14 +342,14 @@
             const int pv = readlane_i(prev, gl);
             const uint32_t gidg = (uint32_t)readlane_i((int)gid, gl);
             const uint8_t *flg = flag_mem + (wave * APW + g) * FLP;
-            const SpRowSrc rowp = SP_ROW_OF(pv);
+            const auto rowp = SP_ROW_OF(pv);
             n_dense += a0 + g < A ? 1ull : 0ull;
             float dk = __builtin_inff();
             int di = 0x7fffffff;
 #pragma unroll
             for (int c = 0; c < CHD; ++c) {
               const int k0 = (c * 64 + lane) * 4;
-              const float4 pvv = sp_row4(rowp, k0);
+              const float4 pvv = sp_row4(rowp, c, sp_lane_off(rowp, lane));
               const uint32_t ff = *reinterpret_cast<const uint32_t *>(flg + k0);
               const u32x4 r4 = rng_block(p.seed, iter_now, STREAM_RACE, gidg, ((uint32_t)t << 12) | (uint32_t)(c * 64 + lane));
               const float pp[4] = {pvv.x, pvv.y, pvv.z, pvv.w};
@@ -382,7 +427,7 @@
               const float ug = readlane_f(ucur, gl), rg = readlane_f(r, gl);
               const uint32_t gidg = (uint32_t)readlane_i((int)gid, gl);
               const uint8_t *flg = flag_mem + (wave * APW + g) * FLP;
-              const SpRowSrc rowp = SP_ROW_OF(pv);
+              const auto rowp = SP_ROW_OF(pv);
               int choice_g = -1;
               const unsigned long long real = a0 + g < A ? 1ull : 0ull;
               if (!(Hg > 0.0f)) {
@@ -420,7 +465,14 @@
                   n_rej += real;
                   n_dense += real;
                   const u32x4 rb = rng_block(p.seed, iter_now, STREAM_SPARSE_RETRY, gidg, (uint32_t)t << 8);
-                  choice_g = sparse_row_walk<CHD, false>(rowp, flg, nullptr, lane, u01(rb.x));
+                  if constexpr (UT) {
+                    sp_args_t pr_ = (sp_args_t)__builtin_amdgcn_kernarg_segment_ptr();
+                    asm volatile("" : "+s"(pr_));
+                    const SpRowTE rowe{rowp.t, sp_row_rsrc(pr_->eta + (size_t)b * pr_->eta_bs + (size_t)pv * n, n)};
+                    choice_g = sparse_row_walk<CHD, false>(rowe, flg, nullptr, lane, u01(rb.x));
+                  } else {
+                    choice_g = sparse_row_walk<CHD, false>(rowp, flg, nullptr, lane, u01(rb.x));
+                  }
                 }
               }
               if (choice_g < 0) { infeasible = true; choice_g = 0; }
@@ -448,7 +500,6 @@
 #undef SP_LAST_POSITIVE
 #undef SP_ID
 #undef SP_IDW
-  typedef const __attribute__((address_space(4))) SampleParams *sp_args_t;
   sp_args_t pe = (sp_args_t)__builtin_amdgcn_kernarg_segment_ptr();
   if constexpr (ST) asm volatile("" : "+s"(pe));
 #define SP_E(x) (ST ? pe->x : p.x)
@@ -659,9 +710,16 @@
 }
 
 struct SparseVariant { const void *fn; size_t lds; };
-static SparseVariant sparse_variant(int ld, bool race, int spl, bool many) {
+static SparseVariant sparse_variant(int ld, bool race, int spl, bool many, bool ut = false) {
 #define DACO_SPARSE_LDS(C) ((C) == 2 ? 16 * ((C) * 256 + 16) + 16 * ((C) * 256 + 2) * 2 : 2 * 8 * (C) * 256 * 2)
 #define DACO_SPARSE_V(C, R, S) SparseVariant{reinterpret_cast<const void *>(&scan_sparse_kernel<C, R, S>), (size_t)DACO_SPARSE_LDS(C)}
+#define DACO_SPARSE_U(C, S) SparseVariant{reinterpret_cast<const void *>(&scan_sparse_kernel<C, false, S, false, false, true>), (size_t)DACO_SPARSE_LDS(C)}
+  if (ut) {
+    if (ld <= 512 && spl == 4 && many) return SparseVariant{reinterpret_cast<const void *>(&scan_sparse_kernel<2, false, 4, false, true, true>), (size_t)SP_ST_LDS};
+    if (ld <= 512) return spl == 4 ? DACO_SPARSE_U(2, 4) : DACO_SPARSE_U(2, 8);
+    return spl == 4 ? DACO_SPARSE_U(4, 4) : DACO_SPARSE_U(4, 8);
+  }
+#undef DACO_SPARSE_U
   if (ld <= 512 && !race && spl == 4 && many) return SparseVariant{reinterpret_cast<const void *>(&scan_sparse_kernel<2, false, 4, false, true>), (size_t)SP_ST_LDS};
   if (ld <= 512) return race ? (spl == 4 ? DACO_SPARSE_V(2, true, 4) : DACO_SPARSE_V(2, true, 8)) : (spl == 4 ? DACO_SPARSE_V(2, false, 4) : DACO_SPARSE_V(2, false, 8));
   return race ? (spl == 4 ? DACO_SPARSE_V(4, true, 4) : DACO_SPARSE_V(4, true, 8)) : (spl == 4 ? DACO_SPARSE_V(4, false, 4) : DACO_SPARSE_V(4, false, 8));
@@ -682,7 +740,7 @@
                                       int fixed_start, uint64_t seed, uint64_t iter, const uint64_t *iter_offset,
                                       uint32_t ant_gid0, int ant_gid_bstride, int64_t *paths, int32_t *flags, const float *dist,
                                       long dist_bstride, float *costs, uint32_t *nbr, unsigned long long *stats, void *workspace,
-                                      size_t workspace_bytes, void *ev_begin, void *ev_end) {
+                                      size_t workspace_bytes, void *ev_begin, void *ev_end, const float *head_eta = nullptr, float tail_c = 0.0f) {
   if (B <= 0 || A <= 0 || !tau || !eta || !head_id || !workspace || (!paths && !nbr)) {
     set_error("%s: bad argument (B=%d n=%d A=%d)", what, B, n, A);
     return DACO_E_BADARG;
@@ -716,7 +774,16 @@
     alpha = beta = 1.0f;
   }
   const bool vec4 = rows_vec4(n, tau, tau_bstride, eta, eta_bstride);
-  if (!heads_ready) {
+  const bool ut = head_eta != nullptr;
+  if (ut && (race || !vec4 || alpha != 1.0f || beta != 1.0f || !(tail_c >= 0.0f))) {
+    set_error("%s: the uniform-tail mode serves the scan draw with alpha = beta = 1, n %% 4 == 0, 16-byte-aligned rows of tau and eta and tail_c >= 0 (n=%d)", what, n);
+    return DACO_E_BADARG;
+  }
+  if (ut && !heads_ready) {
+    const dim3 pg((unsigned)(((long)B * n + 3) / 4));
+    if (ld <= 512) hipLaunchKernelGGL((sparse_prepass_ut_kernel<2>), pg, dim3(256), 0, s, B, n, ld / 256, tau, tau_bstride, head_eta, tail_c, head_id, ws.hrow, spl, ld);
+    else hipLaunchKernelGGL((sparse_prepass_ut_kernel<4>), pg, dim3(256), 0, s, B, n, ld / 256, tau, tau_bstride, head_eta, tail_c, head_id, ws.hrow, spl, ld);
+  } else if (!heads_ready) {
     const dim3 pg((unsigned)(((long)B * n + 3) / 4));
 #define DACO_PREPASS_C(R, V, C) hipLaunchKernelGGL((sparse_prepass_kernel<R, V, C>), pg, dim3(256), 0, s, B, n, ld / 256, tau, tau_bstride, eta, eta_bstride, \
                                                    head_id, ws.P, ws.hrow, spl, ld)
@@ -729,7 +796,7 @@
   if (const int rc = launch_status("sparse_prepass_kernel")) return rc;
   SampleParams sp = sample_params(B, n, A, ld, ld / 256, ws.P, nullptr, nullptr, seed, iter, ant_gid0, paths, nullptr, nullptr, flags);
   sp.start = start; sp.fixed_start = fixed_start;
-  sp.tau = tau; sp.tau_bs = tau_bstride; sp.eta = eta; sp.eta_bs = eta_bstride; sp.alpha = alpha; sp.beta = beta; sp.row_vec = vec4 ? 1 : 0;
+  sp.tau = tau; sp.tau_bs = tau_bstride; sp.eta = eta; sp.eta_bs = eta_bstride; sp.tail_c = tail_c;
   sp.iter_dev = iter_offset; sp.gid_bstride = ant_gid_bstride;
   sp.dist = dist; sp.dist_bs = dist_bstride; sp.costs = costs; sp.nbr = nbr; sp.nbr_grouped = nbr_grouped ? 1 : 0;
   sp.hval = (const float *)ws.hrow; sp.hid = head_id; sp.stats = stats; sp.tours16 = ws.tours16;
@@ -746,11 +813,13 @@
   const int bpi = lh ? (A + 3) / 4 : (A + 15) / 16;
   const dim3 grid((unsigned)(B * bpi));
   if (lh) {
-    if (hipFuncSetAttribute(reinterpret_cast<const void *>(&scan_sparse_kernel<2, false, 4, true>), hipFuncAttributeMaxDynamicSharedMemorySize,
+    const void *lh_fn = ut ? reinterpret_cast<const void *>(&scan_sparse_kernel<2, false, 4, true, false, true>) : reinterpret_cast<const void *>(&scan_sparse_kernel<2, false, 4, true>);
+    if (hipFuncSetAttribute(lh_fn, hipFuncAttributeMaxDynamicSharedMemorySize,
                             160 * 1024 - 128) != hipSuccess) { set_error("%s: hipFuncSetAttribute(dynamic LDS) failed", what); return DACO_E_HIP; }
-    hipLaunchKernelGGL((scan_sparse_kernel<2, false, 4, true>), grid, dim3(256), lh_lds, s, sp);
+    if (ut) hipLaunchKernelGGL((scan_sparse_kernel<2, false, 4, true, false, true>), grid, dim3(256), lh_lds, s, sp);
+    else hipLaunchKernelGGL((scan_sparse_kernel<2, false, 4, true>), grid, dim3(256), lh_lds, s, sp);
   } else {
-    const SparseVariant v = sparse_variant(ld, race, spl, sparse_many_workgroups((long)B * bpi));
+    const SparseVariant v = sparse_variant(ld, race, spl, sparse_many_workgroups((long)B * bpi), ut);
     void *args[] = {&sp};
     if (hipLaunchKernel(v.fn, grid, dim3(256), args, v.lds, s) != hipSuccess) { set_error("%s: scan_sparse_kernel launch failed", what); return DACO_E_HIP; }
   }
@@ -785,3 +854,13 @@
                                      size_t workspace_bytes, void *ev_begin, void *ev_end) {
   return sample_sparse_impl(race != 0, heads_ready != 0, head_live_max, nbr_grouped, "daco_tsp_sample_heads", DACO_SPARSE_ARGS);
 }
+extern "C" long daco_tsp_sample_heads_ut(void *stream, int heads_ready, int head_live_max, int nbr_grouped, int B, int n, int A, const float *tau, long tau_bstride, const float *eta,
+                                        long eta_bstride, const uint16_t *head_id, int head_slots, const int64_t *start,
+                                        int fixed_start, uint64_t seed, uint64_t iter, const uint64_t *iter_offset,
+                                        uint32_t ant_gid0, int ant_gid_bstride, int64_t *paths, int32_t *flags, const float *dist,
+                                        long dist_bstride, float *costs, uint32_t *nbr, unsigned long long *stats, void *workspace,
+                                        size_t workspace_bytes, void *ev_begin, void *ev_end, const float *head_eta, float tail_c) {
+  if (!head_eta) { set_error("daco_tsp_sample_heads_ut: bad argument (head_eta)"); return DACO_E_BADARG; }
+  const float alpha = 1.0f, beta = 1.0f;
+  return sample_sparse_impl(false, heads_ready != 0, head_live_max, nbr_grouped, "daco_tsp_sample_heads_ut", DACO_SPARSE_ARGS, head_eta, tail_c);
+}
diff --git a/deepaco_amd/engine/__init__.py b/deepaco_amd/engine/__init__.py
--- a/deepaco_amd/engine/__init__.py
+++ b/deepaco_amd/engine/__init__.py
@@ -13,7 +13,7 @@
 from .sibling_colonies import (BATCHED_SIBLINGS, OBJ_KINDS, BatchedBPP, BatchedMKP, BatchedOP, BatchedPCTSP, BatchedSMTWTP,
                                BatchedSOP, sibling_objective, sibling_record_)
 from .sibling_ops import SIB_KINDS, PickService, sibling_backward, sibling_sample
-from .tsp_ops import (SPARSE_MAX_N, SPARSE_MIN_N, auto_head_k, head_table, heu_matrix, resolve_sampler, sparse_head,
-                      sparse_tours16, sparse_workspace, sparsify_heuristic, take_auto_top, tsp_edge_backward, tsp_edge_logp, tsp_knn_graph,
-                      tsp_sample, tsp_sample_sparse)
+from .tsp_ops import (SPARSE_MAX_N, SPARSE_MIN_N, auto_head_k, head_eta_table, head_table, heu_matrix, resolve_sampler,
+                      sparse_head, sparse_tours16, sparse_workspace, sparsify_heuristic, take_auto_top, tsp_edge_backward, tsp_edge_logp,
+                      tsp_knn_graph, tsp_sample, tsp_sample_sparse, uniform_tail_applies)
 from .update import pheromone_update_, tour_costs, track_best_
diff --git a/deepaco_amd/engine/colonies.py b/deepaco_amd/engine/colonies.py
--- a/deepaco_amd/engine/colonies.py
+++ b/deepaco_amd/engine/colonies.py
@@ -3,7 +3,7 @@
 from .common import _f32c, _raise_flags, _require_gpu, _rows
 from .cvrp_ops import cvrp_sample
 from .local_search import HgsTables, TspLocalSearch, heuristic_dist, hgs_local_search_, hgs_polar_angles
-from .tsp_ops import head_table, resolve_sampler, sparse_tours16, sparse_workspace, sparsify_heuristic, tsp_sample, tsp_sample_sparse
+from .tsp_ops import head_eta_table, head_table, resolve_sampler, sparse_tours16, sparse_workspace, sparsify_heuristic, tsp_sample, tsp_sample_sparse
 from .update import pheromone_update_, tour_costs, track_best_
 
 
@@ -87,13 +87,17 @@
         self._heads_for = None
         self._flags = torch.zeros((self.B,), dtype=torch.int32, device=dev)
         self.fuse_head_rows = True
+        self.uniform_tail = True
+        self._head_version = None
+        self._head_ut = None
 
     def check_feasible(self):
         _raise_flags(self._flags, ((1, ValueError, "BatchedTSP: a transition row had no feasible candidate"),
                                    (4, RuntimeError, "BatchedTSP: the head table has more live entries per row than head_live_max")))
 
-    def _heads_state(self, head, race):
-        return (self.pheromone, self.pheromone._version, self.heuristic, head, bool(race), float(self.alpha), float(self.beta))
+    def _heads_state(self, head, race, ut=None):
+        return (self.pheromone, self.pheromone._version, self.heuristic, self.heuristic._version, head, bool(race), float(self.alpha),
+                float(self.beta), ut is not None)
 
     def _heuristic_dist(self):
         return self._ls.heuristic_dist(self.heuristic)
@@ -110,10 +114,19 @@
         return resolve_sampler(self.sampler, self.n, self.head_k, self.heuristic, self._auto, path=self.setup_path)
 
     def _head_table(self, k=None):
-        if self._head is None or self._head[0] is not self.heuristic or (k is not None and self._head[2] != k):
+        if self._head is None or self._head[0] is not self.heuristic or (k is not None and self._head[2] != k) \
+                or self._head_version != self.heuristic._version:
             k = k if k is not None else (self.head_k if self.head_k is not None else max(1, min(127, self.n // 10)))
             self._head = (self.heuristic, head_table(self.heuristic, k, self.B, getattr(self, "_auto", None), path=self.setup_path), k)
+            self._head_version = self.heuristic._version
         return self._head[1]
+
+    def _uniform_tail(self, head):
+        if not self.uniform_tail:
+            return None
+        if self._head_ut is None or self._head_ut[0] is not head:
+            self._head_ut = (head, head_eta_table(self.heuristic, head))
+        return self._head_ut[1]
 
     @torch.no_grad()
     def step(self, events=None, _iter_dev=None, ls_events=None, want_paths=True):
@@ -130,18 +143,19 @@
                 self._sparse_ws = sparse_workspace(self.distances.device, self.B, self.n, self.n_ants, unit_exponents=unit)
             fused = self.fuse_head_rows and unit
             grouped = fused and self.n_ants % 8 == 0 and self.local_search is None
-            ready = same_state(self._heads_for, self._heads_state(head, race_head))
+            ut = self._uniform_tail(head) if (unit and not race_head and self.n % 4 == 0) else None
+            ready = same_state(self._heads_for, self._heads_state(head, race_head, ut))
             compact = not want_paths and self.local_search is None
             paths, _, costs, nbr = tsp_sample_sparse(self.pheromone, self.heuristic, self.n_ants, head, self.alpha,
                                                      self.beta, seed=self.seed, it=self.iteration, ant_gid0=self.ant_gid0,
                                                      fixed_start=self.fixed_start, batch=self.B, events=events,
                                                      dist=self.distances, want_nbr=True, iter_dev=_iter_dev, race=race_head,
                                                      workspace=self._sparse_ws, heads_ready=ready, head_live_max=self._head[2],
-                                                     nbr_grouped=grouped, flags=self._flags, want_paths=not compact)
+                                                     nbr_grouped=grouped, flags=self._flags, want_paths=not compact, uniform_tail=ut)
             tours16 = sparse_tours16(self._sparse_ws, self.B, self.n, self.n_ants) if compact else None
             if fused:
                 heads = {"eta": self.heuristic, "alpha": self.alpha, "beta": self.beta, "head": head, "race": race_head,
-                         "workspace": self._sparse_ws, "nbr_grouped": grouped}
+                         "workspace": self._sparse_ws, "nbr_grouped": grouped, "uniform_tail": ut}
         else:
             tours16 = None
             paths, _, _, _, costs, nbr = tsp_sample(self.pheromone, self.heuristic, self.n_ants, self.alpha,
@@ -159,7 +173,7 @@
                               mmas_scale=self.n if self.min_max else None, tours16=tours16)
         cmin, cmax = _mmas_bounds(self, new_max)
         pheromone_update_(self.pheromone, paths, costs, self.decay, self.elitist, True, cmin, cmax, nbr=nbr, heads=heads)
-        self._heads_for = self._heads_state(heads["head"], heads["race"]) if heads is not None else None
+        self._heads_for = self._heads_state(heads["head"], heads["race"], heads["uniform_tail"]) if heads is not None else None
         return paths, costs
 
     @torch.no_grad()
diff --git a/deepaco_amd/engine/tsp_ops.py b/deepaco_amd/engine/tsp_ops.py
--- a/deepaco_amd/engine/tsp_ops.py
+++ b/deepaco_amd/engine/tsp_ops.py
@@ -1,3 +1,5 @@
+import struct
+
 import numpy as np
 import torch
 
@@ -213,12 +215,33 @@
     return sparse_head(_f32c(h), k, top=top, path="torch")
 
 
+def head_eta_table(heuristic, head):
+    _require_gpu(heuristic, head)
+    B, n, slots = head.shape
+    eta, ebs = _bstride(heuristic.detach(), n)
+    dev = head.device
+    with _on(dev):
+        out = torch.empty((B, n, slots), dtype=torch.float32, device=dev)
+        verdict = torch.empty(3, dtype=torch.int32, device=dev)
+        rc = _lib.lib().daco_head_eta(_stream(dev), B, n, eta.data_ptr(), ebs, head.data_ptr(), slots, out.data_ptr(), verdict.data_ptr())
+    _lib.check(rc, "daco_head_eta")
+    bad, nlo, hi = (int(v) & 0xFFFFFFFF for v in verdict.tolist())
+    if bad or (~nlo & 0xFFFFFFFF) != hi:
+        return None
+    return out, struct.unpack("<f", struct.pack("<I", hi))[0]
+
+
+def uniform_tail_applies(n, tau, eta, alpha, beta, race):
+    return (not race and float(alpha) == 1.0 and float(beta) == 1.0 and n % 4 == 0
+            and tau.data_ptr() % 16 == 0 and eta.data_ptr() % 16 == 0)
+
+
 def sparse_workspace(device, B, n, n_ants, unit_exponents=True):
     L = _lib.lib()
     nbytes = (L.daco_tsp_sparse_workspace_bytes if unit_exponents else L.daco_tsp_sparse_workspace_bytes_general)(B, n, n_ants)
     if nbytes == 0:
         raise ValueError(f"scan_sparse serves 129 <= n <= 1024 (n = {n})")
-    return torch.empty(int(nbytes), dtype=torch.uint8, device=device)
+    return torch.zeros(int(nbytes), dtype=torch.uint8, device=device)
 
 
 def sparse_tours16(workspace, B, n, n_ants):
@@ -229,7 +252,8 @@
 
 def tsp_sample_sparse(tau, eta, n_ants, head, alpha=1.0, beta=1.0, start=None, fixed_start=-1, seed=0, it=0, ant_gid0=0,
                       batch=None, events=None, dist=None, want_nbr=False, iter_dev=None, ant_gid_bstride=0, want_stats=False,
-                      want_paths=True, race=False, workspace=None, heads_ready=False, head_live_max=0, nbr_grouped=False, flags=None):
+                      want_paths=True, race=False, workspace=None, heads_ready=False, head_live_max=0, nbr_grouped=False, flags=None,
+                      uniform_tail=None):
     _require_gpu(tau, eta, start, head, workspace)
     assert not heads_ready or workspace is not None
     n = tau.shape[-1]
@@ -259,6 +283,23 @@
             raise ValueError(f"scan_sparse serves 129 <= n <= 1024 (n = {n})")
         ws = workspace if workspace is not None else _workspace(dev, nbytes, "sample_sparse")
         assert ws.numel() >= nbytes
+        if uniform_tail is not None and uniform_tail_applies(n, tau, eta, alpha, beta, race):
+            heta, tail_c = uniform_tail
+            assert heta.dtype == torch.float32 and heta.is_contiguous() and tuple(heta.shape) == tuple(head.shape)
+            rc = L.daco_tsp_sample_heads_ut(_stream(dev), int(bool(heads_ready)), int(head_live_max), int(bool(nbr_grouped)), B, n, n_ants,
+                                            tau.data_ptr(), tbs, eta.data_ptr(), ebs, head.data_ptr(), int(head.shape[2]),
+                                            start.data_ptr() if start is not None else None, int(fixed_start), int(seed) & (2 ** 64 - 1),
+                                            int(it), iter_dev.data_ptr() if iter_dev is not None else None, int(ant_gid0) & 0xFFFFFFFF,
+                                            int(ant_gid_bstride), paths.data_ptr() if paths is not None else None, flags.data_ptr(),
+                                            dist.data_ptr() if dist is not None else None, dbs,
+                                            costs.data_ptr() if costs is not None else None,
+                                            nbr.data_ptr() if nbr is not None else None,
+                                            stats.data_ptr() if stats is not None else None, ws.data_ptr(), ws.numel(),
+                                            events[0].cuda_event if events else None, events[1].cuda_event if events else None,
+                                            heta.data_ptr(), float(tail_c))
+            _lib.check(rc, "daco_tsp_sample_heads_ut")
+            out = (paths, flags, costs, nbr)
+            return out + (stats,) if want_stats else out
         rc = L.daco_tsp_sample_heads(_stream(dev), int(bool(race)), int(bool(heads_ready)), int(head_live_max), int(bool(nbr_grouped)), B, n, n_ants, tau.data_ptr(), tbs, eta.data_ptr(), ebs, float(alpha),
                                       float(beta), head.data_ptr(), int(head.shape[2]), start.data_ptr() if start is not None else None,
                                       int(fixed_start), int(seed) & (2 ** 64 - 1), int(it),
diff --git a/deepaco_amd/engine/update.py b/deepaco_amd/engine/update.py
--- a/deepaco_amd/engine/update.py
+++ b/deepaco_amd/engine/update.py
@@ -2,6 +2,7 @@
 
 from .. import _lib
 from .common import _bstride, _f32c, _on, _require_gpu, _stream, _workspace
+from .tsp_ops import uniform_tail_applies
 
 
 def tour_costs(dist, paths, closed=True):
@@ -70,6 +71,18 @@
             eta, ebs = _bstride(heads["eta"], n)
             head, sws = heads["head"], heads["workspace"]
             _require_gpu(eta, head, sws)
+            ut = heads.get("uniform_tail")
+            if ut is not None and uniform_tail_applies(n, tau, eta, heads["alpha"], heads["beta"], heads.get("race", False)):
+                rc = L.daco_pheromone_update_heads_ut(_stream(dev), B, n, A, tau.data_ptr(), pptr, costs.data_ptr(), float(decay),
+                                                      int(bool(elitist)), clamp_min.data_ptr() if clamp_min is not None else None,
+                                                      clamp_max.data_ptr() if clamp_max is not None else None, float(floor),
+                                                      nbr.data_ptr() if nbr is not None else None,
+                                                      weights.data_ptr() if weights is not None else None, ws.data_ptr(), ws.numel(),
+                                                      head.data_ptr(), int(head.shape[2]),
+                                                      int(bool(heads.get("nbr_grouped", False))) if nbr is not None else 0,
+                                                      sws.data_ptr(), sws.numel(), ut[0].data_ptr(), float(ut[1]))
+                _lib.check(rc, "daco_pheromone_update_heads_ut")
+                return tau
             rc = L.daco_pheromone_update_heads(_stream(dev), B, n, A, tau.data_ptr(), pptr, costs.data_ptr(), float(decay),
                                                int(bool(elitist)), clamp_min.data_ptr() if clamp_min is not None else None,
                                                clamp_max.data_ptr() if clamp_max is not None else None, float(floor),
diff --git a/deepaco_amd/tsp/aco.py b/deepaco_amd/tsp/aco.py
--- a/deepaco_amd/tsp/aco.py
+++ b/deepaco_amd/tsp/aco.py
@@ -111,6 +111,7 @@
             if sampler == "scan_sparse":
                 col.head_k = hk
                 col._head = (eta, self._head_table(hk), hk)
+                col._head_version = eta._version
             hit = self._colony = (key, col)
         col = hit[1]
         shortest = (self.shortest_path.clone() if self.shortest_path is not None else
diff --git a/include/deepaco_hip.h b/include/deepaco_hip.h
--- a/include/deepaco_hip.h
+++ b/include/deepaco_hip.h
@@ -78,6 +78,18 @@
                           unsigned long long *stats,
                           void *workspace, size_t workspace_bytes, void *ev_begin, void *ev_end);
 
+long daco_tsp_sample_heads_ut(void *stream, int heads_ready, int head_live_max, int nbr_grouped, int B, int n, int A,
+                             const float *tau, long tau_bstride, const float *eta, long eta_bstride,
+                             const uint16_t *head_id, int head_slots,
+                             const int64_t *start, int fixed_start,
+                             uint64_t seed, uint64_t iter, const uint64_t *iter_offset, uint32_t ant_gid0,
+                             int ant_gid_bstride,
+                             int64_t *paths, int32_t *flags,
+                             const float *dist, long dist_bstride, float *costs, uint32_t *nbr,
+                             unsigned long long *stats,
+                             void *workspace, size_t workspace_bytes, void *ev_begin, void *ev_end,
+                             const float *head_eta, float tail_c);
+
 size_t daco_directed_table_bytes(int B, int n, int A);
 int daco_cvrp_sample(void *stream, int B, int n, int A,
                      const float *tau, long tau_bstride, const float *eta, long eta_bstride,
@@ -165,6 +177,14 @@
                                 const uint16_t *head_id, int head_slots, int race, int nbr_grouped,
                                 void *sparse_workspace, size_t sparse_workspace_bytes);
 
+long daco_pheromone_update_heads_ut(void *stream, int B, int n, int A, float *tau,
+                                   const int64_t *paths, const float *costs, float decay, int elitist,
+                                   const float *clamp_min, const float *clamp_max, float floor_val,
+                                   const uint32_t *nbr, const float *weights, void *workspace, size_t workspace_bytes,
+                                   const uint16_t *head_id, int head_slots, int nbr_grouped,
+                                   void *sparse_workspace, size_t sparse_workspace_bytes,
+                                   const float *head_eta, float tail_c);
+
 int daco_allreduce_delta_tau(void *comm, void *stream, float *delta, size_t count);
 
 int daco_two_opt(void *stream, int B, int T, int n, const float *dist, const float *dist_T, long dist_bstride,
@@ -233,6 +253,8 @@
 long daco_sparse_head(void *stream, int B, int n, int k, const float *weights, long w_bstride, uint16_t *ids);
 long daco_head_stats(void *stream, int B, int n, const float *weights, long w_bstride, int k_lds, double mass,
                     double mass_lds, int32_t *counts);
+long daco_head_eta(void *stream, int B, int n, const float *eta, long eta_bstride, const uint16_t *head_id, int head_slots,
+                   float *head_eta, uint32_t *verdict);
 
 int daco_mkpv_sample(void *stream, int B, int n, int A, int m, const float *tau, long tau_bstride,
                      const float *eta, long eta_bstride, float alpha, float beta,
```
